# IuvenisSapiens/Qwen3-TTS-Rust

Hardware: AMD Instinct MI355X
Metric: audio-seconds generated per second (aggregate over GPUs) = concurrent real-time streams; RTF and first-chunk latency from the single-utterance leg (higher is better)
Workload: dtype i8

## Files before the change

### include/q3tts.h

```cpp
#ifndef Q3TTS_H
#define Q3TTS_H
#include <stdint.h>
#include <stddef.h>
#include "q3tts_spec.h"
#ifdef __cplusplus
extern "C" {
#endif

#define Q3TTS_OK 0
#define Q3TTS_ERR -1

const char* q3tts_last_error(void);
int q3tts_version(void);
int q3tts_device_count(void);

typedef struct q3tts_sampler_config {
    float temperature;
    int32_t top_k;
    float top_p;
    int32_t has_seed;
    uint64_t seed;
} q3tts_sampler_config;
void q3tts_sampler_config_default(q3tts_sampler_config* c);

// ... 81 lines not shown
int q3tts_submit_resume(q3tts_engine* e, const q3tts_request* r, int32_t want_pcm, const q3tts_gen_options* opts,
                        const int32_t* trail_ids, int32_t n_trail, int32_t open,
                        const int32_t* prefix_codes, int32_t n_prefix, int64_t* req_id);
#define Q3TTS_LOGPROB_COLS 17
#define Q3TTS_LOGPROB_NONE 1.0f
int q3tts_engine_set_logprobs(q3tts_engine* e, int32_t on);
int q3tts_fetch_logprobs(q3tts_engine* e, int64_t req_id, float* out, int32_t frame_off, int32_t max_frames, int32_t* got_frames);
int q3tts_engine_set_output_format(q3tts_engine* e, const q3tts_pcm_format* f);
int q3tts_request_format(q3tts_engine* e, int64_t req_id, q3tts_pcm_format* out);
int q3tts_fetch_pcm16(q3tts_engine* e, int64_t req_id, int16_t* out, int64_t off, int64_t cap, int64_t* got);
int q3tts_engine_pcm_out_stats(q3tts_engine* e, int64_t* chunks_converted, int64_t* samples_out);
int q3tts_engine_set_speech_rate(q3tts_engine* e, int32_t rate_pct);
int q3tts_request_speech_rate(q3tts_engine* e, int64_t req_id, int32_t* rate_pct);
int q3tts_engine_tsm_stats(q3tts_engine* e, int64_t* chunks, int64_t* frames_out, int64_t* flushes);
int q3tts_engine_set_pitch(q3tts_engine* e, int32_t pitch_pct);
int q3tts_request_pitch(q3tts_engine* e, int64_t req_id, int32_t* pitch_pct);
int q3tts_engine_pitch_stats(q3tts_engine* e, int64_t* chunks, int64_t* samples_out, int64_t* flushes, int64_t* table_bytes);
int q3tts_engine_set_volume(q3tts_engine* e, int32_t db10);
int q3tts_request_volume(q3tts_engine* e, int64_t req_id, int32_t* db10);
int q3tts_engine_volume_stats(q3tts_engine* e, int64_t* chunks, int64_t* samples);
typedef struct { double integrated_lufs, momentary_max_lufs, peak_dbfs; int32_t n_blocks, n_gated; } q3tts_loudness;
int q3tts_engine_set_loudness(q3tts_engine* e, int32_t on);
int q3tts_fetch_loudness(q3tts_engine* e, int64_t req_id, double* out , int64_t block_off, int64_t max_blocks, int64_t* got);
int q3tts_request_loudness(q3tts_engine* e, int64_t req_id, q3tts_loudness* out);
int q3tts_request_metered(q3tts_engine* e, int64_t req_id, int32_t* on);
int q3tts_engine_loudness_stats(q3tts_engine* e, int64_t* chunks, int64_t* blocks);
int q3tts_preamble_create(q3tts_engine* e, const int32_t* codes, int32_t n, int32_t* preamble_id);
int q3tts_preamble_poll(q3tts_engine* e, int32_t preamble_id, int32_t* state, int32_t* n_frames);
int q3tts_preamble_wait(q3tts_engine* e, int32_t preamble_id, double timeout_ms);
int q3tts_preamble_release(q3tts_engine* e, int32_t preamble_id);
int q3tts_voice_set_preamble(q3tts_engine* e, int32_t voice_id, int32_t preamble_id);
int q3tts_engine_set_preamble(q3tts_engine* e, int32_t preamble_id);
int q3tts_request_preamble(q3tts_engine* e, int64_t req_id, int32_t* preamble_id);
int q3tts_engine_preamble_stats(q3tts_engine* e, int64_t* built, int64_t* restores, int64_t* bytes_per_snapshot);
typedef struct q3tts_stem_stats { int64_t built, restores, rows_not_prefilled, pages_copied, mismatches, device_bytes; } q3tts_stem_stats;
int q3tts_stem_create(q3tts_engine* e, const float* rows, int32_t n_rows, int32_t* stem_id);
int q3tts_voice_stem_create(q3tts_engine* e, int32_t voice_id, int32_t lang_id, const int32_t* instr_ids, int32_t n_instr, int32_t* stem_id);
int q3tts_stem_poll(q3tts_engine* e, int32_t stem_id, int32_t* state, int32_t* n_rows);
int q3tts_stem_wait(q3tts_engine* e, int32_t stem_id, double timeout_ms);
int q3tts_stem_release(q3tts_engine* e, int32_t stem_id);
int q3tts_voice_set_stem(q3tts_engine* e, int32_t voice_id, int32_t stem_id);
int q3tts_engine_set_stem(q3tts_engine* e, int32_t stem_id);
int q3tts_request_stem(q3tts_engine* e, int64_t req_id, int32_t* stem_id, int32_t* rows_reused);
int q3tts_engine_stem_stats(q3tts_engine* e, q3tts_stem_stats* out);
int q3tts_submit_score(q3tts_engine* e, const float* prompt, int32_t n_prompt, const int32_t* trail_ids, int32_t n_trail,
                       const int32_t* codes, int32_t n, int64_t* req_id);
int32_t q3tts_engine_score_width(q3tts_engine* e);
int q3tts_submit_candidates(q3tts_engine* e, const q3tts_request* r, int32_t want_pcm, const q3tts_gen_options* opts,
                            const int32_t* trail_ids, int32_t n_trail, const uint64_t* seeds, int32_t n, int64_t* req_ids);
int q3tts_engine_candidate_stats(q3tts_engine* e, int64_t* sets, int64_t* prefill_rows_saved, int64_t* pages_copied);
int q3tts_submit_decode(q3tts_engine* e, const int32_t* codes, int32_t n, int64_t* req_id);
int32_t q3tts_engine_decode_width(q3tts_engine* e);
int q3tts_engine_decode_stats(q3tts_engine* e, int64_t* requests, int64_t* chunks, int64_t* chunks_shared);
int32_t q3tts_engine_prefill_width(q3tts_engine* e);
int q3tts_sched_start(q3tts_engine* e);
int q3tts_sched_stop(q3tts_engine* e);
int q3tts_sched_step(q3tts_engine* e, int32_t* busy);
int q3tts_voice_register(q3tts_engine* e, const float* spk_emb2048, const int32_t* ref_codes, int32_t n_ref_codes,
                         const int32_t* ref_text_ids, int32_t n_ref_text, int32_t* voice_id);
int q3tts_submit_text(q3tts_engine* e, int32_t voice_id, const int32_t* text_ids, int32_t n_text, int32_t lang_id,
                      const int32_t* instr_ids, int32_t n_instr, const q3tts_sampler_config* sampler, int32_t max_steps,
                      int32_t mask_eos, int32_t want_pcm, int64_t* req_id);
int q3tts_submit_text_ex(q3tts_engine* e, int32_t voice_id, const int32_t* text_ids, int32_t n_text, int32_t lang_id,
                         const int32_t* instr_ids, int32_t n_instr, const q3tts_sampler_config* sampler, int32_t max_steps,
                         int32_t mask_eos, int32_t want_pcm, const q3tts_gen_options* opts, int64_t* req_id);
int q3tts_submit_text_streaming(q3tts_engine* e, int32_t voice_id, const int32_t* text_ids, int32_t n_text, int32_t lang_id,
                                const int32_t* instr_ids, int32_t n_instr, const q3tts_sampler_config* sampler, int32_t max_steps,
                                int32_t mask_eos, int32_t want_pcm, const q3tts_gen_options* opts, int64_t* req_id);
int q3tts_submit_text_streaming_open(q3tts_engine* e, int32_t voice_id, const int32_t* text_ids, int32_t n_text, int32_t lang_id,
                                     const int32_t* instr_ids, int32_t n_instr, const q3tts_sampler_config* sampler, int32_t max_steps,
                                     int32_t mask_eos, int32_t want_pcm, const q3tts_gen_options* opts, int64_t* req_id);
int q3tts_text_append(q3tts_engine* e, int64_t req_id, const int32_t* text_ids, int32_t n, int32_t is_last);

typedef struct q3tts_group q3tts_group;
int q3tts_group_create(const q3tts_engine_params* p, const int32_t* device_ids, int32_t n_dev, q3tts_group** out);
void q3tts_group_destroy(q3tts_group* g);
int32_t q3tts_group_size(q3tts_group* g);
q3tts_engine* q3tts_group_engine(q3tts_group* g, int32_t i);
int32_t q3tts_group_uses_rccl(q3tts_group* g);
typedef struct q3tts_group_info_t {
    int32_t n_devices, rccl_loaded, rccl_ranks, distinct_devices;
    int64_t registrations_rccl, registrations_peer_copy;
} q3tts_group_info_t;
int q3tts_group_info(q3tts_group* g, q3tts_group_info_t* out);
int q3tts_group_voice_register(q3tts_group* g, const float* spk_emb2048, const int32_t* ref_codes, int32_t n_ref_codes,
                               const int32_t* ref_text_ids, int32_t n_ref_text, int32_t* voice_id);
int q3tts_group_submit(q3tts_group* g, const q3tts_request* r, int32_t want_pcm, int64_t* req_id);
int q3tts_group_submit_text(q3tts_group* g, int32_t voice_id, const int32_t* text_ids, int32_t n_text, int32_t lang_id,
                            const int32_t* instr_ids, int32_t n_instr, const q3tts_sampler_config* sampler, int32_t max_steps,
                            int32_t mask_eos, int32_t want_pcm, int64_t* req_id);
int q3tts_group_submit_ex(q3tts_group* g, const q3tts_request* r, int32_t want_pcm, const q3tts_gen_options* opts, int64_t* req_id);
int q3tts_group_submit_text_ex(q3tts_group* g, int32_t voice_id, const int32_t* text_ids, int32_t n_text, int32_t lang_id,
                               const int32_t* instr_ids, int32_t n_instr, const q3tts_sampler_config* sampler, int32_t max_steps,
                               int32_t mask_eos, int32_t want_pcm, const q3tts_gen_options* opts, int64_t* req_id);
int q3tts_group_submit_text_streaming(q3tts_group* g, int32_t voice_id, const int32_t* text_ids, int32_t n_text, int32_t lang_id,
                                      const int32_t* instr_ids, int32_t n_instr, const q3tts_sampler_config* sampler, int32_t max_steps,
                                      int32_t mask_eos, int32_t want_pcm, const q3tts_gen_options* opts, int64_t* req_id);
int q3tts_group_submit_text_streaming_open(q3tts_group* g, int32_t voice_id, const int32_t* text_ids, int32_t n_text, int32_t lang_id,
                                           const int32_t* instr_ids, int32_t n_instr, const q3tts_sampler_config* sampler,
                                           int32_t max_steps, int32_t mask_eos, int32_t want_pcm, const q3tts_gen_options* opts,
                                           int64_t* req_id);
int q3tts_group_text_append(q3tts_group* g, int64_t req_id, const int32_t* text_ids, int32_t n, int32_t is_last);
int q3tts_group_trail_append(q3tts_group* g, int64_t req_id, const int32_t* ids, int32_t n, int32_t close);
int q3tts_group_trail_progress(q3tts_group* g, int64_t req_id, int32_t* n_appended, int32_t* n_consumed, int32_t* closed);
int32_t q3tts_group_device_of(q3tts_group* g, int64_t req_id);
int q3tts_group_poll(q3tts_group* g, int64_t req_id, q3tts_req_status* out);
// ... 264 lines not shown
    uint64_t* keys; int64_t n_keys; int32_t key_stride; const int32_t* mask_per_tok; int32_t idx_add;
    float* out; int64_t out_floats, out_off; int32_t out_stride;
    int8_t* aq; uint16_t* ad;
    int32_t form_ran, lpr_ran, mt_ran, z_ran;
} q3tts_linear_desc;
int q3tts_op_linear(q3tts_linear_desc* d);
int q3tts_linear_plan(q3tts_linear_desc* d);
uint64_t q3tts_argmax_key(float v, int32_t idx);

enum { Q3TTS_SEL_SAMPLE = 0, Q3TTS_SEL_SAMPLE_PRED = 1, Q3TTS_SEL_ARGMAX = 2, Q3TTS_SEL_ARGMAX_KEYS = 3 };
#define Q3TTS_SELECT_SENTINEL 0xA5C3F00D5A3C0FF1ull
typedef struct q3tts_select_desc {
    int32_t kernel;
    int32_t B, n, stride, row_off;
    const float* logits;
    const float* temperature; const int32_t* top_k; const float* top_p;
    const int32_t* mask_idx;
    const uint64_t* seed;
    const uint32_t* draw0;
    int32_t n_draws;
    const float* penalty; const int32_t* hist; const int32_t* hist_len; int32_t hist_cap; const int32_t* cur_code;
    int32_t out_stride;
    int32_t start, end, add;
    int32_t* tokens;
    uint64_t* out_raw;
    uint32_t* draws_out;
} q3tts_select_desc;
int q3tts_op_select_rows(q3tts_select_desc* d);

enum { Q3TTS_GLUE_PROJECT_MT = 0, Q3TTS_GLUE_PROJECT_TABLE = 1, Q3TTS_GLUE_FEEDBACK_KEYS = 2, Q3TTS_GLUE_GATHER_ROWS_KEYS = 3,
       Q3TTS_GLUE_ADVANCE_KEYS = 4, Q3TTS_GLUE_STALL_SAVE = 5, Q3TTS_GLUE_ADVANCE_KEYS_GATED = 6 };
#define Q3TTS_GLUE_GUARD 64
typedef struct q3tts_guarded { void* p; int64_t n; } q3tts_guarded;
typedef struct q3tts_frame_glue_desc {
    int32_t kernel;
    int32_t ntok;
    int32_t n_in, n_out, x_stride, x_off, out_stride;
    const float* x; int64_t x_floats;
    const float* w; const float* b;
    const float* const* tables; const int64_t* table_rows;
    int32_t row_len, key_stride;
    const float* tts_pad;
    int32_t trail; const int32_t* trail_ids; int32_t ids_stride; const float* text_table; int64_t text_rows;
    const int32_t* n_trail; const int32_t* open; const int32_t* max_frames;
    int32_t hist_stride;
    q3tts_guarded out;
    q3tts_guarded keys, next_key0;
    q3tts_guarded finished, n_frames, t_slot, t_pos, hist;
    q3tts_guarded hidden, save_hidden;
    q3tts_guarded draws, pdraws, save_draws;
} q3tts_frame_glue_desc;
int q3tts_op_frame_glue(q3tts_frame_glue_desc* d);

enum { Q3TTS_GG_LOAD_ROWS = 0, Q3TTS_GG_ADD = 1, Q3TTS_GG_RMSNORM = 2, Q3TTS_GG_QUANT = 3, Q3TTS_GG_MATVEC = 4, Q3TTS_GG_LINEAR = 5,
       Q3TTS_GG_SWIGLU = 6 };
typedef struct q3tts_ggml_desc {
    int32_t op;
    int32_t ntok, k;
    int64_t n;
    const float* x; int64_t x_floats; int32_t x_stride; int32_t x_rows;
    const float* u; float eps;
    const int32_t* idx; const uint64_t* idx_keys; int32_t idx_stride; int64_t idx_n;
    const void* w; int32_t type, rows, row0, nrows, out_stride;
    q3tts_guarded out;
    q3tts_guarded q8, d8, qk, dk, bs;
} q3tts_ggml_desc;
int q3tts_op_ggml(q3tts_ggml_desc* d);

int q3tts_pcm_out_plan(int32_t rate, int32_t* L, int32_t* M, int32_t* n_taps, int32_t* taps_per_phase);
int64_t q3tts_pcm_out_filter(int32_t rate, float* h32, int64_t cap);
int64_t q3tts_pcm_out_samples(int32_t rate, int64_t n_native);
int q3tts_pcm_format_check(const q3tts_pcm_format* f);
int q3tts_op_pcm_convert(const float* in, int32_t G, const int32_t* chunk_samples, int32_t n_chunks, const int32_t* streams, int32_t n_streams,
                         const q3tts_pcm_format* fmt, const int32_t* reset_before, void* const* out, const int64_t* out_bytes, int64_t* n_out,
                         float* hist_store);

int64_t q3tts_tsm_samples(int32_t rate_pct, int64_t n_native, int32_t final);
int q3tts_tsm_windows(float* w, float* w2);
int q3tts_op_tsm(const float* in, int32_t G, const int32_t* chunk_samples, int32_t n_chunks, const int32_t* streams, int32_t n_streams,
                 const int32_t* rate_pct, const int32_t* encoding, const int32_t* reset_before, int32_t flush, void* const* out,
                 const int64_t* out_bytes, int64_t* n_out, int32_t* const* delta_trace, const int64_t* trace_len, float* hist_store);

int64_t q3tts_pitch_samples(int32_t rate_pct, int32_t pitch_pct, int64_t n_native, int32_t final);
int q3tts_pitch_plan(int32_t pitch_pct, int32_t* L, int32_t* M, int32_t* n_taps, int32_t* taps_per_output);
int64_t q3tts_pitch_filter(int32_t pitch_pct, float* h32, int64_t cap);
int q3tts_op_pitch(const float* in, int32_t G, const int32_t* chunk_samples, int32_t n_chunks, const int32_t* streams, int32_t n_streams,
                   const int32_t* rate_pct, const int32_t* pitch_pct, const int32_t* encoding, const int32_t* reset_before, int32_t flush,
                   void* const* out, const int64_t* out_bytes, int64_t* n_out, int32_t* const* delta_trace, const int64_t* trace_len,
                   float* hist_store, float* zhist_store);

float q3tts_volume_gain(int32_t db10);
int q3tts_op_volume(const float* in, int32_t G, const int32_t* chunk_samples, int32_t n_chunks, const int32_t* streams, int32_t n_streams,
                    const int32_t* vol_db10, const int32_t* reset_before, float* const* out, const int64_t* out_bytes, int64_t* n_out,
                    float* const* gain_trace, const int64_t* trace_len, float* hist_store);

int q3tts_loudness_tables(double* coef , double* m );
int q3tts_loudness_gate(const double* rows, int32_t n, q3tts_loudness* out);
int32_t q3tts_loudness_gain_db10(double measured_lufs, double target_lufs);
int q3tts_op_loudness(const float* in, int32_t G, const int32_t* chunk_samples, int32_t n_chunks, const int32_t* streams, int32_t n_streams,
                      const int32_t* metered, const int32_t* reset_before, double* const* rows, const int64_t* rows_bytes, int64_t* n_rows,
                      double* state_store);

int q3tts_intake_plan(int32_t rate, int32_t* L, int32_t* M, int32_t* n_taps, int32_t* taps_per_output);
int64_t q3tts_intake_filter(int32_t rate, float* h32, int64_t cap);
int64_t q3tts_intake_samples(int32_t rate, int64_t n_frames);
int32_t q3tts_intake_tile(int32_t rate);
// ... 10 lines not shown
```

### qwen3-tts-rust_amd/csrc/capi.cpp

```cpp
#include "../../include/q3tts.h"
#include "engine.h"
#include "tfctx.h"
#include <algorithm>

using namespace q3;

struct q3tts_assets { std::unique_ptr<HostAssets> owned; const HostAssets* a = nullptr; };
struct q3tts_engine { std::unique_ptr<Engine> e; q3tts_assets assets_view; };
struct q3tts_sampler { Sampler s; };
struct q3tts_chunker { std::unique_ptr<Chunker> c; };
struct q3tts_decoder { std::unique_ptr<CodecDecoder> d; hipStream_t st = nullptr; float* pinned = nullptr; size_t pinned_cap = 0; };
struct q3tts_tf { std::unique_ptr<TfContext> c; };

#define Q3_API_BEGIN try {
#define Q3_API_END(failval) } catch (const std::exception& ex) { set_last_error(ex.what()); return failval; } catch (...) { set_last_error("unknown error"); return failval; }

static void require_gpu() {
    int n = 0;
    if (hipGetDeviceCount(&n) != hipSuccess || n <= 0) throw Error("no HIP device available: the HIP path is the only compute path (no CPU fallback)");
}

extern "C" {

const char* q3tts_last_error(void) { return last_error(); }
// ... 85 lines not shown
    g.trail = trail_ids; g.n_trail = n_trail;
    *req_id = e->e->submit(g, want_pcm != 0, true);
    return Q3TTS_OK;
    Q3_API_END(Q3TTS_ERR)
}
int q3tts_submit_trailing_open(q3tts_engine* e, const q3tts_request* r, int32_t want_pcm, const q3tts_gen_options* opts,
                               const int32_t* trail_ids, int32_t n_trail, int64_t* req_id) {
    Q3_API_BEGIN
    Q3_CHECK(e && r && req_id, "null argument");
    GenRequest g = to_gen(*r);
    g.opts = to_opts(opts);
    g.trail = trail_ids; g.n_trail = n_trail; g.open = true;
    *req_id = e->e->submit(g, want_pcm != 0, true);
    return Q3TTS_OK;
    Q3_API_END(Q3TTS_ERR)
}
int q3tts_submit_resume(q3tts_engine* e, const q3tts_request* r, int32_t want_pcm, const q3tts_gen_options* opts, const int32_t* trail_ids,
                        int32_t n_trail, int32_t open, const int32_t* prefix_codes, int32_t n_prefix, int64_t* req_id) {
    Q3_API_BEGIN
    Q3_CHECK(e && r && req_id, "null argument");
    GenRequest g = to_gen(*r);
    g.opts = to_opts(opts);
    g.trail = trail_ids; g.n_trail = n_trail; g.open = open != 0;
    g.prefix = prefix_codes; g.n_prefix = n_prefix;
    *req_id = e->e->submit(g, want_pcm != 0, true);
    return Q3TTS_OK;
    Q3_API_END(Q3TTS_ERR)
}
int q3tts_submit_score(q3tts_engine* e, const float* prompt, int32_t n_prompt, const int32_t* trail_ids, int32_t n_trail, const int32_t* codes,
                       int32_t n, int64_t* req_id) {
    Q3_API_BEGIN
    Q3_CHECK(e && req_id, "null argument");
    *req_id = e->e->submit_score(prompt, n_prompt, trail_ids, n_trail, codes, n);
    return Q3TTS_OK;
    Q3_API_END(Q3TTS_ERR)
}
int32_t q3tts_engine_score_width(q3tts_engine* e) { return e ? e->e->score_width() : -1; }
int q3tts_submit_decode(q3tts_engine* e, const int32_t* codes, int32_t n, int64_t* req_id) {
    Q3_API_BEGIN
    Q3_CHECK(e && codes && req_id, "null argument");
    *req_id = e->e->submit_decode(codes, n);
    return Q3TTS_OK;
    Q3_API_END(Q3TTS_ERR)
}
int32_t q3tts_engine_decode_width(q3tts_engine* e) { return e ? e->e->decode_width() : -1; }
int q3tts_engine_decode_stats(q3tts_engine* e, int64_t* requests, int64_t* chunks, int64_t* chunks_shared) {
    Q3_API_BEGIN
    Q3_CHECK(e, "null argument");
    int64_t r = 0, c = 0, s = 0;
    e->e->decode_stats(&r, &c, &s);
    if (requests) *requests = r;
    if (chunks) *chunks = c;
    if (chunks_shared) *chunks_shared = s;
    return Q3TTS_OK;
    Q3_API_END(Q3TTS_ERR)
}
int q3tts_submit_candidates(q3tts_engine* e, const q3tts_request* r, int32_t want_pcm, const q3tts_gen_options* opts, const int32_t* trail_ids,
                            int32_t n_trail, const uint64_t* seeds, int32_t n, int64_t* req_ids) {
    Q3_API_BEGIN
    Q3_CHECK(e && r, "null argument");
    GenRequest g = to_gen(*r);
    g.opts = to_opts(opts);
    g.trail = trail_ids; g.n_trail = n_trail;
    std::vector<int64_t> ids((size_t)std::max(n, 1));
    e->e->submit_candidates(g, want_pcm != 0, seeds, n, req_ids ? ids.data() : nullptr);
    std::copy(ids.begin(), ids.begin() + n, req_ids);
    return Q3TTS_OK;
    Q3_API_END(Q3TTS_ERR)
}
int q3tts_engine_candidate_stats(q3tts_engine* e, int64_t* sets, int64_t* prefill_rows_saved, int64_t* pages_copied) {
    Q3_API_BEGIN
    Q3_CHECK(e, "null argument");
    int64_t s = 0, r = 0, p = 0;
    e->e->candidate_stats(&s, &r, &p);
    if (sets) *sets = s;
    if (prefill_rows_saved) *prefill_rows_saved = r;
    if (pages_copied) *pages_copied = p;
    return Q3TTS_OK;
    Q3_API_END(Q3TTS_ERR)
}
int q3tts_trail_append(q3tts_engine* e, int64_t req_id, const int32_t* ids, int32_t n, int32_t close) {
    Q3_API_BEGIN
    Q3_CHECK(e, "null argument");
    return e->e->append_trail(req_id, ids, n, close != 0);
    Q3_API_END(Q3TTS_ERR)
}
int q3tts_trail_progress(q3tts_engine* e, int64_t req_id, int32_t* n_appended, int32_t* n_consumed, int32_t* closed) {
    Q3_API_BEGIN
    Q3_CHECK(e && n_appended && n_consumed && closed, "null argument");
    int na = 0, nc = 0; bool cl = false;
    e->e->trail_progress(req_id, &na, &nc, &cl);
    *n_appended = na; *n_consumed = nc; *closed = cl ? 1 : 0;
    return Q3TTS_OK;
    Q3_API_END(Q3TTS_ERR)
}
int q3tts_text_append(q3tts_engine* e, int64_t req_id, const int32_t* text_ids, int32_t n, int32_t is_last) {
    Q3_API_BEGIN
    Q3_CHECK(e, "null argument");
    Q3_CHECK(n >= 0 && (n == 0 || text_ids), "bad arguments");
    std::vector<int32_t> ids(text_ids, text_ids + n);
    if (is_last) ids.push_back(Q3_TEXT_EOS);
    return e->e->append_trail(req_id, ids.data(), (int)ids.size(), is_last != 0);
    Q3_API_END(Q3TTS_ERR)
}
int q3tts_poll(q3tts_engine* e, int64_t id, q3tts_req_status* o) {
    Q3_API_BEGIN
// ... 580 lines not shown
```

### qwen3-tts-rust_amd/csrc/capi_ops.cpp

```cpp
#include "../../include/q3tts.h"
#include "transformer.h"
#include "host_logic.h"
#include "kdev.h"
#include "codec.h"
#include "kernels.h"
#include "pcm_out.h"
#include "tsm.h"
#include "pitch.h"
#include "volume.h"
#include "loudness.h"
#include "intake.h"
#include <memory>
#include "mel.h"

using namespace q3;
#define Q3_API_BEGIN try {
#define Q3_API_END(failval) } catch (const std::exception& ex) { set_last_error(ex.what()); return failval; } catch (...) { set_last_error("unknown error"); return failval; }
static void require_gpu() {
    int n = 0;
    if (hipGetDeviceCount(&n) != hipSuccess || n <= 0) throw Error("no HIP device available: the HIP path is the only compute path (no CPU fallback)");
}

static int attention_op_plan(const q3tts_attention_desc& d) {
    AttnPlanIn a;
// ... 1068 lines not shown
        } else {
            Q3_CHECK(d.tts_pad, "tts_pad missing");
            DevBuf<const float*> d_ptrs(16); DevBuf<int64_t> d_rows(16); DevBuf<float> d_pad(Q3_EMBD), d_text; DevBuf<int32_t> d_ntrail, d_ids;
            d_ptrs.upload(ptrs.data(), 16); d_rows.upload(d.table_rows, 16); d_pad.upload(d.tts_pad, Q3_EMBD);
            if (d.trail) {
                Q3_CHECK(d.n_trail && d.trail_ids && d.ids_stride >= 1 && d.text_table && d.text_rows >= 1, "the trail form needs n_trail / trail_ids / text_table");
                n_frames.up(d.n_frames, n, "n_frames");
                for (size_t t = 0; t < n; t++)
                    Q3_CHECK(n_frames.host[Q3TTS_GLUE_GUARD + t] >= 0 && d.n_trail[t] <= d.ids_stride, "n_frames < 0 or n_trail > ids_stride");
                d_ntrail.alloc(n); d_ntrail.upload(d.n_trail, n);
                d_ids.alloc(n * d.ids_stride); d_ids.upload(d.trail_ids, d_ids.n);
                d_text.alloc((size_t)d.text_rows * Q3_EMBD); d_text.upload(d.text_table, d_text.n);
                TextTrail tt; tt.n_frames = n_frames.p(); tt.n_trail = d_ntrail.p; tt.ids = d_ids.p; tt.ids_stride = d.ids_stride; tt.table = d_text.p; tt.rows = d.text_rows;
                launch_feedback_keys(0, d_ptrs.p, d_rows.p, keys.p(), d.key_stride, d_pad.p, out.p(), d.ntok, &tt);
            } else {
                launch_feedback_keys(0, d_ptrs.p, d_rows.p, keys.p(), d.key_stride, d_pad.p, out.p(), d.ntok);
            }
        }
        Q3_LAUNCH_CHECK();
        Q3_HIP(hipDeviceSynchronize());
        out.down(); keys.down(); n_frames.down();
        return Q3TTS_OK;
    }
    const bool gate = d.kernel != Q3TTS_GLUE_ADVANCE_KEYS;
    Q3_CHECK(d.max_frames && d.hist_stride >= 16, "max_frames / hist_stride missing");
    keys.up(d.keys, n * 16, "keys"); next_key0.up(d.next_key0, n, "next_key0");
    finished.up(d.finished, n, "finished"); n_frames.up(d.n_frames, n, "n_frames"); t_slot.up(d.t_slot, n, "t_slot");
    t_pos.up(d.t_pos, 4 * n, "t_pos"); hist.up(d.hist, n * d.hist_stride, "hist");
    for (size_t b = 0; b < n; b++)
        Q3_CHECK(n_frames.host[Q3TTS_GLUE_GUARD + b] >= 0 && d.max_frames[b] >= 0 && (int64_t)d.max_frames[b] * 16 <= d.hist_stride, "history row outside hist_stride");
    DevBuf<int32_t> d_max(n + 1), d_open, d_ntrail;
    d_max.zero(); d_max.upload(d.max_frames, n);
    AdvanceKeysArgs a{d.ntok, finished.p(), n_frames.p(), d_max.p, keys.p(), next_key0.p(), hist.p(), d.hist_stride, t_slot.p(), t_pos.p()};
    if (!gate) {
        launch_advance_keys(0, a);
    } else {
        Q3_CHECK(d.open && d.n_trail, "the gated kernels need open / n_trail");
        hidden.up(d.hidden, n * Q3_EMBD, "hidden"); save_hidden.up(d.save_hidden, n * Q3_EMBD, "save_hidden");
        draws.up(d.draws, n, "draws"); pdraws.up(d.pdraws, n, "pdraws"); save_draws.up(d.save_draws, 2 * n, "save_draws");
        d_open.alloc(n + 1); d_open.zero(); d_open.upload(d.open, n); d_ntrail.alloc(n + 1); d_ntrail.zero(); d_ntrail.upload(d.n_trail, n);
        StallArgs s; s.open = d_open.p; s.n_trail = d_ntrail.p; s.hidden = hidden.p(); s.draws = draws.p(); s.pdraws = pdraws.p();
        s.save_hidden = save_hidden.p(); s.save_draws = save_draws.p();
        if (d.kernel == Q3TTS_GLUE_STALL_SAVE) launch_stall_save(0, a, s);
        else launch_advance_keys_gated(0, a, s);
    }
    Q3_LAUNCH_CHECK();
    Q3_HIP(hipDeviceSynchronize());
    keys.down(); next_key0.down(); finished.down(); n_frames.down(); t_slot.down(); t_pos.down(); hist.down();
    hidden.down(); save_hidden.down(); draws.down(); pdraws.down(); save_draws.down();
    return Q3TTS_OK;
    Q3_API_END(Q3TTS_ERR)
}

int q3tts_op_ggml(q3tts_ggml_desc* dp) {
    Q3_API_BEGIN
    require_gpu();
    Q3_CHECK(dp, "null ggml-mode descriptor");
    const q3tts_ggml_desc& d = *dp;
    Q3_CHECK(d.op >= Q3TTS_GG_LOAD_ROWS && d.op <= Q3TTS_GG_SWIGLU, "unknown ggml-mode op");
    const bool flat = d.op == Q3TTS_GG_ADD || d.op == Q3TTS_GG_SWIGLU;
    const bool mat = d.op == Q3TTS_GG_MATVEC || d.op == Q3TTS_GG_LINEAR, quant = d.op == Q3TTS_GG_QUANT || mat;
    const auto holds = [](const q3tts_guarded& g, size_t core) { return g.p && g.n >= (int64_t)(core + 2 * Q3TTS_GLUE_GUARD); };
    GlueBuf<float> out, dk;
    GlueBuf<int8_t> q8, qk;
    GlueBuf<uint16_t> d8;
    GlueBuf<int16_t> bs;
    DevBuf<float> dx, du;
    if (flat) {
        Q3_CHECK(d.n >= 0 && d.n <= ((int64_t)1 << 31), "n out of [0, 2^31]");
        if (d.n == 0) return Q3TTS_OK;
        const size_t n = (size_t)d.n;
        Q3_CHECK(d.x && d.x_floats >= d.n && holds(d.out, n), "x / out do not hold n elements");
        Q3_CHECK(d.op == Q3TTS_GG_ADD || d.u, "u missing");
        out.up(d.out, n, "out");
        dx.alloc(n); dx.upload(d.x, n);
        if (d.op == Q3TTS_GG_ADD) gg_add(0, out.p(), dx.p, n);
        else { du.alloc(n); du.upload(d.u, n); gg_swiglu(0, dx.p, du.p, out.p(), n); }
        Q3_LAUNCH_CHECK();
        Q3_HIP(hipDeviceSynchronize());
        out.down();
        return Q3TTS_OK;
    }
    Q3_CHECK(d.ntok >= 0 && d.ntok <= 65535 && d.k >= 1, "ntok out of [0, 65535] or k < 1");
    const size_t nt = (size_t)d.ntok, k = (size_t)d.k;
    GgMat w;
    if (mat) {
        w.type = d.type; w.n = d.rows; w.k = d.k;
        Q3_CHECK(w.type == Q3_T_Q8_0 || w.type == Q3_T_Q5_K || w.type == Q3_T_Q6_K, "ggml mode serves Q8_0 / Q5_K / Q6_K matrices");
        Q3_CHECK(d.rows >= 0 && d.row0 >= 0 && d.nrows >= 0 && (int64_t)d.row0 + d.nrows <= d.rows, "ggml-mode matvec row range");
        if (d.nrows == 0) return Q3TTS_OK;
    }
    if (nt == 0) return Q3TTS_OK;
    if (quant) {
        Q3_CHECK(d.k % 256 == 0, "k % 256 != 0");
        Q3_CHECK(holds(d.q8, nt * k) && holds(d.d8, nt * k / 32) && holds(d.qk, nt * k) && holds(d.dk, nt * k / 256) && holds(d.bs, nt * k / 16),
                 "a quantised array does not hold ntok rows");
    }
    if (d.op == Q3TTS_GG_LOAD_ROWS) {
        Q3_CHECK(d.x && d.x_rows >= 1 && d.x_stride >= d.k && d.x_floats >= (int64_t)(d.x_rows - 1) * d.x_stride + d.k, "x does not hold x_rows rows");
        Q3_CHECK(!(d.idx && d.idx_keys) && holds(d.out, nt * k), "both index forms given, or out too small");
        if (d.idx || d.idx_keys) {
            Q3_CHECK(d.idx_stride >= 1 && d.idx_n >= (int64_t)(nt - 1) * d.idx_stride + 1, "idx / idx_keys do not hold ntok entries");
            for (size_t t = 0; t < nt; t++) {
                const int64_t row = d.idx_keys ? (int64_t)key_code(d.idx_keys[t * d.idx_stride]) : (int64_t)d.idx[t * d.idx_stride];
                Q3_CHECK(row >= 0 && row < d.x_rows, "a selected row lies outside x");
            }
// ... 608 lines not shown
```

### qwen3-tts-rust_amd/csrc/codec_worker.cpp

```cpp
#include "codec_worker.h"
#include <chrono>

namespace q3 {

CodecWorker::CodecWorker(CodecDecoder* codec, int dev, int n_lanes, int n_cs, size_t slot_cap) : codec_(codec), dev_(dev), st_(n_lanes), slot_cap_(slot_cap), n_cs_(n_cs) {
    for (auto& s : st_) Q3_HIP(hipStreamCreateWithFlags(&s, hipStreamNonBlocking));
    Q3_HIP(hipHostMalloc((void**)&pcm_pinned_, (size_t)n_cs * slot_cap_ * sizeof(float)));
}

CodecWorker::~CodecWorker() {
    if (started_) {
        { std::lock_guard<std::mutex> lk(mu_); stop_ = true; q_.hold = 0; }
        cv_.notify_all();
        thread_.join();
    }
    for (auto& c : comp_) (void)hipEventDestroy(c.ev);
    for (auto& kv : last_) (void)hipEventDestroy(kv.second.second);
    if (pcm_pinned_) (void)hipHostFree(pcm_pinned_);
    if (loud_pinned_.load()) (void)hipHostFree(loud_pinned_.load());
    for (auto s : st_) (void)hipStreamDestroy(s);
}

void CodecWorker::push(CodecJob* j, TaskKind kind, const int64_t* codes, int n_codes, bool is_final) {
    { std::lock_guard<std::mutex> lk(mu_); q_.push(j, kind, codes, n_codes, is_final); }
    cv_.notify_all();
}
void CodecWorker::purge(CodecJob* j) { std::lock_guard<std::mutex> lk(mu_); q_.purge(j); }
int CodecWorker::pending() { std::lock_guard<std::mutex> lk(mu_); return q_.pending; }

bool CodecWorker::poll_completion(bool block, Completion* out) {
    std::unique_lock<std::mutex> lk(mu_);
    if (!err_.empty()) throw Error("decoder thread: " + err_);
    if (comp_.empty()) {
        if (!block) return false;
        cv_.wait_for(lk, std::chrono::milliseconds(2));
        if (comp_.empty()) return false;
    }
    *out = comp_.front();
    if (!block && hipEventQuery(out->ev) != hipSuccess) return false;
    comp_.pop_front();
    q_.popped();
    lk.unlock();
    Q3_HIP(hipEventSynchronize(out->ev));
    return true;
}

unsigned char* CodecWorker::stage(const CodecJob& j, size_t add) const {
    const size_t at = j.pcm_enq * j.sample_bytes();
    Q3_CHECK(at + add <= slot_bytes(), "pcm staging overflow");
    return reinterpret_cast<unsigned char*>(pcm_pinned_ + (size_t)j.cs * slot_cap_) + at;
}

double* CodecWorker::loud_stage(const CodecJob& j, size_t add) {
    if (!loud_pinned_.load()) {
        std::lock_guard<std::mutex> cap(capture_mutex());
        double* p = nullptr;
        Q3_HIP(hipHostMalloc((void**)&p, (size_t)n_cs_ * loud_cap() * 2 * sizeof(double)));
        loud_pinned_.store(p);
    }
    Q3_CHECK(j.loud_enq + add <= loud_cap(), "loudness staging overflow");
    return loud_pinned_.load() + ((size_t)j.cs * loud_cap() + j.loud_enq) * 2;
}

int CodecWorker::pick_lane(const Step& s) {
    int lane = next_lane_;
    auto own = last_.find(s[0].job);
    if (s.size() == 1 && own != last_.end()) lane = own->second.first;
    else next_lane_ = (next_lane_ + 1) % (int)st_.size();
    for (const Task& t : s) {
        auto it = last_.find(t.job);
        if (it != last_.end() && it->second.first != lane) Q3_HIP(hipStreamWaitEvent(st_[lane], it->second.second, 0));
    }
    return lane;
}

void CodecWorker::start_stream(int lane, const Step& s) {
    CodecJob* j = s[0].job;
    if (j->pre_snap < 0) { codec_->reset_async(st_[lane], j->cs); return; }
    codec_->restore_async(st_[lane], j->pre_snap, j->cs, pcm_format_native(j->out.fmt) ? nullptr : j->pre_tail);
    pre_restores++;
}

void CodecWorker::decode_pass(int lane, const Step& s) {
    const int G = (int)s.size(), nf = (int)s[0].codes.size() / 16, spf = codec_->samples_per_frame();
    int n_low = 0;
    for (const Task& t : s) n_low += t.job->decode;
    dec_chunks += n_low;
    if (n_low < G) dec_shared += n_low;
    std::vector<int> streams(G); std::vector<float*> dst(G); std::vector<int64_t> codes((size_t)G * nf * 16);
    std::vector<OutSpec> out(G); std::vector<int64_t> n_out(G);
    std::vector<LoudDst> loud(G); std::vector<size_t> rows(G, 0);
    for (int g = 0; g < G; g++) {
        CodecJob* j = s[g].job;
        out[g] = j->out;
        const size_t add = j->bytes_due((int64_t)nf * spf, false);
        if (j->out.loud) {
            rows[g] = (size_t)loud_blocks(j->tsm_native, (int64_t)nf * spf);
            loud[g].pos = j->tsm_native; loud[g].rows = loud_stage(*j, rows[g]);
        }
        j->tsm_native += (int64_t)nf * spf;
        streams[g] = j->cs; dst[g] = reinterpret_cast<float*>(stage(*j, add));
        std::copy(s[g].codes.begin(), s[g].codes.end(), codes.begin() + (size_t)g * nf * 16);
    }
    codec_->decode_group_async(st_[lane], G, streams.data(), codes.data(), nf, dst.data(), lane, out.data(), n_out.data(), loud.data());
    for (int g = 0; g < G; g++) { s[g].job->pcm_enq += (size_t)n_out[g]; s[g].job->loud_enq += rows[g]; }
}

void CodecWorker::flush_rate(int lane, const Step& s) {
    CodecJob* j = s[0].job;
    if (!j->stretched() || j->cancel.load() || j->cs < 0) return;
    const size_t add = j->bytes_due(0, true);
    int64_t n = 0;
    codec_->tsm_flush_async(st_[lane], j->cs, stage(*j, add), &n, lane);
    j->pcm_enq += (size_t)n;
}
void CodecWorker::snapshot_build(int lane, const Step& s) {
    CodecJob* j = s[0].job;
    if (j->snapshot && !j->cancel.load()) j->snap = codec_->snapshot_async(st_[lane], j->cs);
}

void CodecWorker::record(int lane, const Step& s) {
    for (const Task& t : s) {
        hipEvent_t ev = nullptr;
        if (t.kind != TASK_RESET) {
            Q3_HIP(hipEventCreate(&ev));
            Q3_HIP(hipEventRecord(ev, st_[lane]));
        }
        auto it = last_.find(t.job);
        if (t.kind == TASK_FENCE) { if (it != last_.end()) { (void)hipEventDestroy(it->second.second); last_.erase(it); } }
        else {
            hipEvent_t ord;
            if (it == last_.end()) { Q3_HIP(hipEventCreateWithFlags(&ord, hipEventDisableTiming)); last_[t.job] = {lane, ord}; }
            else { ord = it->second.second; it->second.first = lane; }
            Q3_HIP(hipEventRecord(ord, st_[lane]));
        }
        if (t.kind == TASK_RESET) continue;
        std::lock_guard<std::mutex> lk(mu_);
        comp_.push_back(Completion{t.job, ev, t.job->pcm_enq, t.kind == TASK_FENCE, t.job->loud_enq});
        if (t.kind == TASK_CHUNK) codec_calls_++;
    }
    cv_.notify_all();
}

void CodecWorker::main() {
    try {
        Q3_HIP(hipSetDevice(dev_));
        const int gmax = codec_->max_group();
        for (;;) {
            Step s;
            {
                std::unique_lock<std::mutex> lk(mu_);
                cv_.wait(lk, [&] { return stop_ || q_.ready(); });
                s = q_.take(gmax);
                if (s.empty()) return;
            }
            const int lane = pick_lane(s);
            if (s[0].kind == TASK_RESET) start_stream(lane, s);
            else if (s[0].kind == TASK_CHUNK) decode_pass(lane, s);
            else { flush_rate(lane, s); snapshot_build(lane, s); }
            record(lane, s);
        }
    } catch (const std::exception& ex) {
        std::lock_guard<std::mutex> lk(mu_);
        err_ = ex.what();
        cv_.notify_all();
    }
}

}
```

### qwen3-tts-rust_amd/csrc/codec_worker.h

```cpp
#pragma once
#include "codec.h"
#include "loudness.h"
#include "sched_logic.h"
#include <atomic>
#include <condition_variable>
#include <mutex>
#include <thread>

namespace q3 {

struct CodecJob {
    int64_t id = 0;
    bool decode = false;
    int cs = -1;
    OutSpec out;
    int pre_snap = -1; const float* pre_tail = nullptr; bool snapshot = false;
    std::atomic<bool> cancel{false};
    int64_t tsm_native = 0;
    size_t pcm_enq = 0;
    size_t loud_enq = 0;
    int snap = -1;
    size_t sample_bytes() const { return out_sample_bytes(out); }
    bool stretched() const { return out_kind(out) >= OUT_RATED; }
    size_t bytes_due(int64_t n_more, bool final) const {
        return (size_t)(out_delivered(out, tsm_native + n_more, final) - out_delivered(out, tsm_native, false)) * sample_bytes();
    }
};

class CodecWorker {
public:
    struct Completion { CodecJob* job; hipEvent_t ev; size_t pcm_after; bool fence; size_t loud_after; };
    CodecWorker(CodecDecoder* codec, int dev, int n_lanes, int n_cs, size_t slot_cap);
    ~CodecWorker();
    void start() { if (!started_) { started_ = true; thread_ = std::thread([this] { main(); }); } }

    void push_reset(CodecJob* j) { push(j, TASK_RESET); }
    void push_chunk(CodecJob* j, const int64_t* codes, int n_codes, bool is_final) { push(j, TASK_CHUNK, codes, n_codes, is_final); }
    void push_fence(CodecJob* j) { push(j, TASK_FENCE); }
    void purge(CodecJob* j);
    struct Handover {
        CodecWorker* w;
        Handover(CodecWorker* w_, bool on) : w(on ? w_ : nullptr) { if (w) { std::lock_guard<std::mutex> lk(w->mu_); w->q_.open(); } }
        ~Handover() { if (w) { { std::lock_guard<std::mutex> lk(w->mu_); w->q_.close(); } w->cv_.notify_all(); } }
        Handover(const Handover&) = delete; Handover& operator=(const Handover&) = delete;
    };
    int pending();
    bool poll_completion(bool block, Completion* out);

    size_t slot_bytes() const { return slot_cap_ * sizeof(float); }
    const float* staging(int cs) const { return pcm_pinned_ + (size_t)cs * slot_cap_; }
    unsigned char* stage(const CodecJob& j, size_t add) const;
    size_t loud_cap() const { return slot_cap_ / Q3_LOUD_BLOCK + 1; }
    const double* loud_staging(int cs) const { return loud_pinned_.load() + (size_t)cs * loud_cap() * 2; }

    std::atomic<int64_t> dec_chunks{0}, dec_shared{0}, pre_restores{0};
    long take_codec_calls() { return (long)codec_calls_.exchange(0); }

private:
    typedef CodecQueue<CodecJob>::Task Task;
    typedef std::vector<Task> Step;
    void push(CodecJob* j, TaskKind kind, const int64_t* codes = nullptr, int n_codes = 0, bool is_final = false);
    void main();
    int pick_lane(const Step& s);
    void start_stream(int lane, const Step& s);
    void decode_pass(int lane, const Step& s);
    void flush_rate(int lane, const Step& s);
    void snapshot_build(int lane, const Step& s);
    void record(int lane, const Step& s);

    CodecDecoder* codec_; int dev_;
    std::vector<hipStream_t> st_;
    float* pcm_pinned_ = nullptr; size_t slot_cap_ = 0;
    std::atomic<double*> loud_pinned_{nullptr}; int n_cs_ = 0;
    double* loud_stage(const CodecJob& j, size_t add);
    std::thread thread_; bool started_ = false, stop_ = false;
    std::mutex mu_; std::condition_variable cv_;
    CodecQueue<CodecJob> q_; std::deque<Completion> comp_; std::string err_;
    std::map<CodecJob*, std::pair<int, hipEvent_t>> last_; int next_lane_ = 0;
    std::atomic<int64_t> codec_calls_{0};
};

}
```

### qwen3-tts-rust_amd/csrc/engine.cpp

```cpp
#include "engine.h"
#include "../../include/q3tts.h"
#include <algorithm>
#include <cmath>
#include <chrono>
#include "kdev.h"
#include <functional>

namespace q3 {

static std::string quant_dir(const std::string& q) {
    if (q == "q5_k_m") return "gguf_q5_k_m";
    if (q == "q8_0") return "gguf_q8_0";
    if (q == "bf16") return "gguf_bf16";
    if (q == "f16") return "gguf_f16";
    return "gguf";
}
static double now_ms() {
    return std::chrono::duration<double, std::milli>(std::chrono::steady_clock::now().time_since_epoch()).count();
}

Engine::Engine(const EngineParams& p) : p_(p) {
    Q3_CHECK(p.max_batch >= 1 && p.max_batch <= 512, "max_batch out of range");
    Q3_HIP(hipGetDevice(&dev_));
    Q3_HIP(hipStreamCreateWithFlags(&st_, hipStreamNonBlocking));
// ... 20 lines not shown
        const std::vector<float> wt = project_wt(assets_->proj_w, Q3_EMBD, dP_), wb = project_wblk(assets_->proj_w, Q3_EMBD, dP_);
        d_proj_wt_.alloc(wt.size()); d_proj_wt_.upload(wt.data(), wt.size());
        d_proj_wblk_.alloc(wb.size()); d_proj_wblk_.upload(wb.data(), wb.size());
    }
    d_proj_b_.alloc(dP_); d_proj_b_.upload(assets_->proj_b, dP_);
    d_tts_pad_.alloc(Q3_EMBD); d_tts_pad_.upload(assets_->tts_pad(), Q3_EMBD);
    std::vector<const float*> ptrs(16);
    std::vector<int64_t> rows(16);
    for (int q = 0; q < 16; q++) {
        const size_t n = (size_t)assets_->codec_rows[q] * Q3_EMBD;
        d_codec_tab_[q].alloc(n); d_codec_tab_[q].upload(assets_->codec[q], n);
        d_proj_tab_[q].alloc((size_t)assets_->codec_rows[q] * dP_);
        launch_project_table(st_, d_codec_tab_[q].p, assets_->codec_rows[q], d_proj_wt_.p, d_proj_b_.p, Q3_EMBD, dP_, d_proj_tab_[q].p);
        ptrs[q] = d_codec_tab_[q].p; rows[q] = assets_->codec_rows[q];
    }
    d_tab_ptrs_.alloc(16); d_tab_ptrs_.upload(ptrs.data(), 16);
    d_tab_rows_.alloc(16); d_tab_rows_.upload(rows.data(), 16);
    pred_l0_table_ = !predictor_->ggml_mode();
    if (const char* e = std::getenv("Q3_PRED_L0_TABLE")) if (e[0] == '0') pred_l0_table_ = false;
    if (pred_l0_table_) {
        const int qs = (predictor_->hp().n_head + 2 * predictor_->hp().n_kv) * 128;
        Transformer wide(*predictor_, 256);
        for (int q = 1; q < 15; q++) {
            d_qkv0_tab_[q].alloc((size_t)assets_->codec_rows[q] * qs);
            wide.build_layer0_qkv(st_, d_proj_tab_[q].p, dP_, assets_->codec_rows[q], d_qkv0_tab_[q].p);
            pred_table_bytes_ += d_qkv0_tab_[q].n * sizeof(float);
        }
        Q3_HIP(hipStreamSynchronize(st_));
    }
    const int pages_per_seq = (p.max_prompt + p.max_steps + 1 + 63) / 64;
    kv_rows_ = (int64_t)pages_per_seq * 64;
    kv_t_.reset(new KvPool(talker_->hp().n_layer, talker_->hp().n_kv, B * pages_per_seq + 1, B + 1, pages_per_seq));
    kv_p_.reset(new KvPool(predictor_->hp().n_layer, predictor_->hp().n_kv, B, B, 1));
    for (int b = 0; b < B; b++) kv_p_->ensure(b, 16);
    pred_identity_pages_ = true;
    for (int b = 0; b < B; b++) if (kv_p_->page(b, 0) != b) pred_identity_pages_ = false;
    if (const char* e = std::getenv("Q3_UNIFORM_META")) if (e[0] == '0') pred_identity_pages_ = false;
    kv_t_->ensure(B, 1);
    {
        const char* e = std::getenv("Q3_ASYNC_PREFILL");
        async_pf_ = B > 1 && !(e && e[0] == '0');
    }
    if (async_pf_) {
        talker_pf_.reset(new Transformer(*talker_, pf_chunk_));
        Q3_HIP(hipStreamCreateWithFlags(&st_pf_, hipStreamNonBlocking));
        Q3_HIP(hipEventCreate(&pf_done_)); Q3_HIP(hipEventCreate(&pf_e0_));
        lane_alloc(pf_, talker_pf_.get(), st_pf_, pf_chunk_, true,(size_t)4096 * (Q3_EMBD * 4 + 24 + 68 + 64) + ((size_t)1 << 16) + (size_t)B * 4 +
                   (size_t)B * 2 * (sizeof(StemJob) + 4) + 256);
    }
    hist_stride_ = p.max_steps * 16;
    tl_stride_ = (Q3_SAMPLE_END + 31) & ~31;
    slots_ = SlotTable(B); d_slots_.alloc(slots_.host.size()); slots_.dev = d_slots_.p;
    d_keys_.alloc(16 * B); d_next_key0_.alloc(B); d_hist_.alloc((size_t)B * hist_stride_);
    d_rngkey_.alloc((size_t)8 * B); d_draws_.alloc(B); d_prngkey_.alloc((size_t)8 * B); d_pdraws_.alloc(B);
    d_rngkey_.zero(); d_draws_.zero(); d_prngkey_.zero(); d_pdraws_.zero(); d_plogits_.alloc((size_t)B * Q3_CODEBOOK_SIZE);
    d_tlogits_.alloc((size_t)B * tl_stride_); d_thidden_.alloc((size_t)B * Q3_EMBD); d_pin_.alloc((size_t)2 * B * dP_);
    d_fb_.alloc((size_t)B * Q3_EMBD);
    d_hist_.zero(); d_tlogits_.zero(); d_thidden_.zero();
    std::vector<int32_t> seq(B), slot((size_t)16 * B), pos((size_t)16 * B * 4);
    for (int b = 0; b < B; b++) {
        seq[b] = b;
        for (int i = 0; i < 16; i++) { slot[(size_t)i * B + b] = i; for (int s = 0; s < 4; s++) pos[((size_t)i * B + b) * 4 + s] = i; }
    }
    d_pseq_.alloc(B); d_pseq_.upload(seq.data(), B);
    d_pslot_.alloc(slot.size()); d_pslot_.upload(slot.data(), slot.size());
    d_ppos_.alloc(pos.size()); d_ppos_.upload(pos.data(), pos.size());
    h_pend_.assign(B, std::vector<int32_t>()); h_pend_off_.assign(B, 0);
    slot_req_.assign(B, nullptr);
    if (const char* e = std::getenv("Q3_SCORE_WIDTH")) score_w_ = std::max(16, std::min(64, atoi(e)));
    if (async_pf_) { d_pf_logits_.alloc((size_t)B * tl_stride_); d_pf_hidden_.alloc((size_t)B * Q3_EMBD); }
    {
        std::vector<q3_u64> k0((size_t)16 * B, pack_key(-INFINITY, 0)), n0(B, pack_key(-INFINITY, 0));
        d_keys_.upload(k0.data(), k0.size()); d_next_key0_.upload(n0.data(), n0.size());
    }
    lane_alloc(ar_, talker_.get(), st_, talker_->max_tok(), false, (size_t)talker_->max_tok() * Q3_EMBD * 4 + (size_t)B * 4096 + ((size_t)1 << 20));
    Q3_HIP(hipDeviceSynchronize());
    upload_slot_state();
    if (p.load_codec) {
        Q3_CHECK(p.max_steps <= Q3TTS_CODEC_MAX_FRAMES, "max_steps above Q3TTS_CODEC_MAX_FRAMES: a request's codec stream could not be decoded to its end");
        static const int group_env = [] { const char* e = std::getenv("Q3_CODEC_GROUP"); return e ? atoi(e) : 0; }();
        const int group_cap = group_env > 0 ? group_env : (B >= 128 ? 32 : 16);
        const int n_cs = B + std::min(B, 16), gmax = std::max(1, std::min(B, group_cap));
        static const int lanes_env = [] { const char* e = std::getenv("Q3_CODEC_LANES"); return e ? atoi(e) : 0; }();
        const int n_lanes = B > 1 ? (lanes_env > 0 ? std::min(lanes_env, 8) : 2) : 1;
        codec_.reset(new CodecDecoder(p.model_dir + "/onnx/q3tts_codec.gguf", n_cs, 4, n_lanes, gmax));
        worker_.reset(new CodecWorker(codec_.get(), dev_, n_lanes, n_cs, (size_t)p.max_steps * codec_->samples_per_frame()));
        Q3_HIP(hipHostMalloc((void**)&pre_tails_, (size_t)Q3TTS_MAX_PREAMBLES * Q3_PCM_HIST * sizeof(float)));
        for (int i = Q3TTS_MAX_PREAMBLES - 1; i >= 0; i--) pre_tail_free_.push_back(i);
        for (int c = n_cs - 1; c >= 0; c--) cs_free_.push_back(c);
        decode_w_ = q3::decode_width(n_cs, B);
    }
    Q3_HIP(hipStreamSynchronize(st_));
    Q3_HIP(hipDeviceSynchronize());
    ar_.cur.reset();
}

void Engine::lane_alloc(PrefillLane& L, Transformer* talker, hipStream_t st, int chunk, bool async, size_t arena_bytes) {
    L.talker = talker; L.st = st; L.chunk = chunk; L.async = async;
    L.d_rows.alloc((size_t)chunk * Q3_EMBD); L.d_seq.alloc(chunk); L.d_slot.alloc(chunk); L.d_pos.alloc(4 * (size_t)chunk);
    L.d_codes.alloc((size_t)chunk * 16); L.d_ids.alloc(chunk); L.d_fork_dst.alloc(B_);
    L.d_stem_jobs.alloc((size_t)2 * B_); L.d_stem_slots.alloc((size_t)2 * B_);
    L.cur.cap = arena_bytes;
    Q3_HIP(hipHostMalloc((void**)&L.arena, arena_bytes));
}
void* Engine::stage_take(PrefillLane& L, size_t bytes) {
    size_t at = L.cur.take(bytes);
    if (at == StageCursor::NONE) {
        Q3_CHECK(!L.async, "prefill staging arena overflow");
        Q3_HIP(hipStreamSynchronize(L.st));
        L.cur.reset();
        at = L.cur.take(bytes);
        Q3_CHECK(at != StageCursor::NONE, "staging request larger than the arena");
    }
    return L.arena + at;
}
void Engine::h2d(void* dst, const void* src, size_t bytes) {
    void* p = stage_alloc(bytes);
    std::memcpy(p, src, bytes);
    Q3_HIP(hipMemcpyAsync(dst, p, bytes, hipMemcpyHostToDevice, st_));
}
void* Engine::d2h_begin(const void* src, size_t bytes) {
    void* p = stage_alloc(bytes);
    Q3_HIP(hipMemcpyAsync(p, src, bytes, hipMemcpyDeviceToHost, st_));
    return p;
}

struct CandSet { std::vector<float> prompt; std::vector<int32_t> trail; };
struct Engine::Req {
    CodecJob job;
    int64_t set = 0; std::shared_ptr<const CandSet> shared;
    const std::vector<int32_t>& trail_ids() const { return shared ? shared->trail : trail_own; }
    GenRequest r; std::vector<float> prompt_own; std::vector<int32_t> trail_own; bool want_pcm = false;
    std::vector<int32_t> prefix_own;
    bool closed = false;
    int state = REQ_QUEUED; int slot = -1; int fed = 0;
    std::vector<int32_t> codes; std::vector<float> pcm;
    int64_t pcm_n = 0;
    bool score = false;
    int pre = -1; bool pre_held = false; int build_pre = -1;
// ... 112 lines not shown
            if (v.lp) {
                LogprobArgs la;
                la.p.logits = d_plp_.p; la.p.stride = Q3_CODEBOOK_SIZE; la.p.head_stride = (size_t)B_ * Q3_CODEBOOK_SIZE; la.p.n = Q3_CODEBOOK_SIZE;
                la.p.key = d_keys_.p + 1; la.p.key_stride = 16; la.p.col = 1; la.n_first = 15;
                la.t.logits = d_tlogits_.p; la.t.stride = tl_stride_; la.t.n = Q3_SAMPLE_END; la.t.key = d_next_key0_.p; la.t.key_stride = 1;
                la.t.extra_idx = Q3_CODEC_EOS; la.t.col = 0; la.t.col_extra = Q3_LOGPROB_COLS - 1; la.t.row_ahead = 1;
                la.out = d_lp_.p; la.out_stride = Q3_LOGPROB_COLS; la.out_rows = lp_rows_;
                la.n_frames = di(SF_NFRAMES); la.finished = di(SF_FINISHED); la.max_frames = di(SF_MAXFRAMES); la.open = di(SF_OPEN);
                la.n_trail = di(SF_NTRAIL); la.record = d_lp_rec_.p;
                launch_logprob_rows(st_, la, B);
            }
        } else {
            ArgmaxEpi am{d_next_key0_.p, 1, di(SF_MASKEOS), 0};
            talker_->head(st_, 0, B, 0, tl_stride_, nullptr, 0, &am, Q3_SAMPLE_END, d_thidden_.p);
        }
    }
    if (v.gate) launch_advance_keys_gated(st_, a, sg);
    else launch_advance_keys(st_, a);
    Q3_LAUNCH_CHECK();
}

std::mutex& capture_mutex() { static std::mutex mu; return mu; }

Engine::FrameGraph& Engine::frame_graph(int width, FrameVariant v, bool capture) {
    std::unique_ptr<FrameGraph>& slot = graphs_[v.key(width)];
    std::unique_lock<std::mutex> build_lock(capture_mutex(), std::defer_lock);
    if (!slot || (capture && !slot->exec)) build_lock.lock();
    if (!slot) {
        slot.reset(new FrameGraph());
        FrameGraph& fg = *slot;
        fg.width = width;
        const int B = width;
        std::vector<int32_t> seqA(2 * B), slotA(2 * B), posA((size_t)2 * B * 4);
        for (int b = 0; b < B; b++) {
            seqA[b] = b; seqA[B + b] = b; slotA[b] = 0; slotA[B + b] = 1;
            for (int s = 0; s < 4; s++) { posA[(size_t)b * 4 + s] = 0; posA[((size_t)B + b) * 4 + s] = 1; }
        }
        fg.seqA.alloc(2 * B); fg.seqA.upload(seqA.data(), 2 * B);
        fg.slotA.alloc(2 * B); fg.slotA.upload(slotA.data(), 2 * B);
        fg.posA.alloc(posA.size()); fg.posA.upload(posA.data(), posA.size());
    }
    FrameGraph& fg = *slot;
    if (capture && !fg.exec) {
        (void)hipGetLastError();
        Q3_HIP(hipStreamBeginCapture(st_, hipStreamCaptureModeThreadLocal));
        try { record_frame(fg, v); }
        catch (...) { hipGraph_t dead = nullptr; (void)hipStreamEndCapture(st_, &dead); if (dead) (void)hipGraphDestroy(dead); throw; }
        Q3_HIP(hipStreamEndCapture(st_, &fg.graph));
        Q3_HIP(hipGraphInstantiate(&fg.exec, fg.graph, nullptr, nullptr, 0));
    }
    return fg;
}

void Engine::upload_slot_state() {
    slots_.route();
    h2d(slots_.dev, slots_.host.data(), slots_.host.size() * 4);
    slot_dirty_ = false;
}

void Engine::prefill_wave(PrefillLane& L, const std::vector<Req*>& wave, bool sampled) {
    size_t total = 0;
    std::vector<PromptRef> refs;
    std::vector<Req*> batch; std::vector<std::vector<Req*>> rest;
    split_sets(wave, batch, rest);
    for (Req* r : batch) {
        total += (size_t)admission_rows(r->r.n_prompt, r->n_skip, r->r.n_prefix);
        refs.push_back({r->r.prompt, r->r.n_prompt, r->slot, r->r.n_prefix, r->n_skip});
    }
    PrefillCursor cur; std::vector<std::pair<int, int>> lasts; std::vector<FbRun> fb;
    std::vector<char> is_score;
    for (Req* r : batch) is_score.push_back(r->score);
    restore_stems(L, batch);
    L.talker->set_same_seq_tokens(true);
    for (size_t done = 0; done < total;) {
        const size_t n_max = std::min<size_t>(total - done, (size_t)L.chunk);
        float* stage = (float*)stage_take(L, n_max * Q3_EMBD * 4);
        int32_t* hc = (int32_t*)stage_take(L, n_max * 68);
        int32_t* hs = (int32_t*)stage_take(L, n_max * 64);
        int32_t* seq = (int32_t*)stage_take(L, n_max * 4); int32_t* slot = (int32_t*)stage_take(L, n_max * 4); int32_t* pos = (int32_t*)stage_take(L, n_max * 16);
        const PrefillCursor before = cur;
        const int n = pack_prefill_chunk(refs, cur, (int)n_max, stage, seq, slot, pos, lasts, &fb);
        for (auto& run : staged_runs(n, fb))
            Q3_HIP(hipMemcpyAsync(L.d_rows.p + (size_t)run.first * Q3_EMBD, stage + (size_t)run.first * Q3_EMBD, (size_t)run.second * Q3_EMBD * 4, hipMemcpyHostToDevice, L.st));
        feedback_rows(L.st, batch, fb, hc, L.d_codes.p, L.d_ids.p, L.d_rows.p);
        Q3_HIP(hipMemcpyAsync(L.d_seq.p, seq, (size_t)n * 4, hipMemcpyHostToDevice, L.st));
        Q3_HIP(hipMemcpyAsync(L.d_slot.p, slot, (size_t)n * 4, hipMemcpyHostToDevice, L.st));
        Q3_HIP(hipMemcpyAsync(L.d_pos.p, pos, (size_t)n * 16, hipMemcpyHostToDevice, L.st));
        TokMeta tm{L.d_seq.p, L.d_slot.p, L.d_pos.p};
        Transformer::Input in; in.x = L.d_rows.p; in.x_stride = Q3_EMBD;
        L.talker->forward(L.st, in, n, tm, kv_t_->view(), nullptr);
        score_chunk(L.st, *L.talker, batch, score_head_runs(refs, is_score, before, n), hs);
        for (auto& lb : lasts) {
            if (batch[lb.first]->offline()) continue;
            if (L.async) head_staged(batch[lb.first], rest[lb.first], lb.second);
            else head_live(batch[lb.first], rest[lb.first], lb.second, sampled);
        }
        done += (size_t)n;
    }
    save_stems(L, batch);
    if (batch.size() < wave.size()) fork_sets(L.st, batch, rest, (int32_t*)stage_take(L, (size_t)B_ * 4), L.d_fork_dst.p);
}
SampleArgs Engine::first_head_args(const float* logits_row, int b) const {
    return SampleArgs{logits_row, tl_stride_, Q3_SAMPLE_END, df(SF_TEMP) + b, di(SF_TOPK) + b, df(SF_TOPP) + b,
                      di(SF_MASKEOS) + b, d_rngkey_.p + (size_t)b * 8, d_draws_.p + b, d_keys_.p + (size_t)b * 16, 16};
}
void Engine::head_live(Req* lead, const std::vector<Req*>& rest, int tok, bool sampled) {
    const bool hist = resumed_penalised(lead->r);
    const bool rec = lead->r.logprobs;
    for (size_t m = 0; m <= rest.size(); m++) {
// ... 427 lines not shown
            case CANCEL_PURGE: worker_->purge(&r->job); break;
            default: break;
            }
        }
    }
    for (Req* r : live) retire(r, false);
}

void Engine::admit(bool stalled) {
    if (async_pf_ && !pf_batch_.empty()) return;
    std::vector<Req*> batch;
    {
        std::lock_guard<std::mutex> lk(mu_);
        int reserved = 0;
        for (int b = 0; b < B_; b++) if (slot_req_[b]) reserved++;
        static const int quantum_div = [] { const char* e = std::getenv("Q3_ADMIT_DIV"); return e ? std::max(1, atoi(e)) : 8; }();
        const int free_slots = B_ - reserved, quantum = std::max(1, B_ / quantum_div);
        if (free_slots < quantum && n_active_ > 0 && free_slots < (int)pending_.size() && !stalled) return;
        std::vector<QueueEntry> q;
        for (Req* r : pending_) {
            if ((int)q.size() >= free_slots && (q.empty() || r->set == 0 || r->set != q.back().set)) break;
            q.push_back({admission_rows(r->r.n_prompt, r->n_skip, r->r.n_prefix), r->want_pcm, r->set});
        }
        for (int take = admission_take(q, free_slots, (int)cs_free_.size(), async_pf_ && n_active_ > 0); take > 0; take--) {
            Req* r = pending_.front();
            int slot = -1;
            for (int b = 0; b < B_; b++) if (!slot_req_[b]) { slot = b; break; }
            pending_.pop_front();
            r->slot = slot;
            if (r->want_pcm) { r->job.cs = cs_free_.back(); cs_free_.pop_back(); }
            r->state = REQ_RUNNING; r->t_admit = now_ms();
            slot_req_[slot] = r;
            batch.push_back(r);
        }
    }
    if (batch.empty()) return;
    alloc_stem_stores(batch);
    for (Req* r : batch) {
        if (r->want_pcm) worker_->push_reset(&r->job);
        r->chunker.reset(new Chunker([this, r](const int64_t* codes, int n_codes, bool is_final) { if (r->want_pcm) worker_->push_chunk(&r->job, codes, n_codes, is_final); }));
        Q3_HIP(hipEventCreate(&r->ev_admit));
    }
    if (async_pf_ && n_active_ > 0) { prefill_async(batch); return; }
    for (Req* r : batch) kv_t_->release(r->slot), kv_t_->ensure(r->slot, kv_positions(r->r, r->score), st_);
    bool sampled = live_variant(slots_).sampled;
    std::vector<Req*> live, scores, builds;
    for (Req* r : batch) {
        if (r->r.sampler.temperature > 0.0f) sampled = true;
        (r->build_stem >= 0 ? builds : r->score ? scores : live).push_back(r);
    }
    hipEvent_t e0, e1;
    Q3_HIP(hipEventCreate(&e0)); Q3_HIP(hipEventCreate(&e1));
    go_live(live);
    { std::lock_guard<std::mutex> lk(mu_); n_active_ += (int)live.size(); }
    Q3_HIP(hipEventRecord(e0, st_));
    for (Req* r : batch) Q3_HIP(hipEventRecord(r->ev_admit, st_));
    prefill_wave(ar_, batch, sampled);
    Q3_HIP(hipEventRecord(e1, st_));
    Q3_HIP(hipStreamSynchronize(st_));
    { float ms = 0; Q3_HIP(hipEventElapsedTime(&ms, e0, e1)); stats.prefill_ms += ms; }
    (void)hipEventDestroy(e0); (void)hipEventDestroy(e1);
    {
        const double t = now_ms();
        std::lock_guard<std::mutex> lk(mu_);
        for (Req* r : batch) r->prefill_ms = t - r->t_submit;
    }
    finish_scores(scores);
    finish_builds(builds);
}

int64_t Engine::submit_decode(const int32_t* codes, int n) {
    if (const char* why = decode_refusal(codes, n, p_.max_steps, codec_ != nullptr)) throw Error(why);
    std::unique_ptr<Req> r(new Req());
    r->job.decode = true; r->want_pcm = true;
    take_out(r.get(), n);
    r->r.max_steps = n; r->r.n_prompt = 0; r->r.sampler.temperature = 0.0f;
    r->codes.assign(codes, codes + (size_t)n * 16); r->fed = n;
    r->t_submit = now_ms();
    std::lock_guard<std::mutex> lk(mu_);
    if (pres_.setting >= 0) pre_attach(r.get(), pres_.setting);
    dec_reqs_++;
    return enqueue(std::move(r), decode_q_);
}

void Engine::admit_decodes() {
    std::lock_guard<std::mutex> lk(mu_);
    for (int take = decode_admit((int)decode_q_.size(), (int)cs_free_.size(), n_decoding_, decode_w_); take > 0; take--) {
        Req* r = decode_q_.front();
        decode_q_.pop_front();
        r->job.cs = cs_free_.back(); cs_free_.pop_back();
        r->state = REQ_DRAINING; r->t_admit = now_ms();
        n_draining_++; n_decoding_++;
        dec_admitted_.push_back(r);
    }
}

void Engine::enqueue_decodes() {
    std::vector<Req*> batch;
    batch.swap(dec_admitted_);
    for (Req* r : batch) {
        Q3_HIP(hipEventCreate(&r->ev_admit));
        Q3_HIP(hipEventRecord(r->ev_admit, st_));
        CodecWorker::Handover piece(worker_.get(), true);
        worker_->push_reset(&r->job);
        Chunker cut([&](const int64_t* codes, int n_codes, bool is_final) { worker_->push_chunk(&r->job, codes, n_codes, is_final); });
        push_frames(cut, r->codes.data(), r->fed);
        cut.push(nullptr, 0, true);
        worker_->push_fence(&r->job);
    }
}

void Engine::prefill_async(const std::vector<Req*>& wave) {
    for (Req* r : wave) {
        kv_t_->release(r->slot);
        kv_t_->ensure(r->slot, kv_positions(r->r, r->score), st_pf_);
    }
    pf_.cur.reset();
    Q3_HIP(hipEventRecord(pf_e0_, st_pf_));
    for (Req* r : wave) Q3_HIP(hipEventRecord(r->ev_admit, st_pf_));
    prefill_wave(pf_, wave, false);
    Q3_HIP(hipEventRecord(pf_done_, st_pf_));
    pf_batch_ = wave;
    n_prefilling_ = (int)wave.size();
}

void Engine::go_live(const std::vector<Req*>& batch) {
    ar_.cur.reset();
    q3_u64 armed[17]; std::fill_n(armed, 17, pack_key(-INFINITY, 0));
    bool prefix_pcm = false;
    for (Req* r : batch) prefix_pcm = prefix_pcm || (r->want_pcm && r->r.n_prefix >= 4);
    {
        CodecWorker::Handover hold(worker_.get(), worker_ && prefix_pcm);
        for (Req* r : batch) {
            const int b = r->slot;
            slots_.load(b, r->r);
            const int k = r->r.n_prefix;
            const uint32_t draws = r->r.sampler.temperature > 0.0f ? (uint32_t)k : 0u, pdraws = 15u * (uint32_t)k;
            if (k > 0) {
                h2d(d_hist_.p + (size_t)b * hist_stride_, r->prefix_own.data(), (size_t)k * 64);
                push_frames(*r->chunker, r->prefix_own.data(), k);
            }
            StdRng rng(r->seed);
            h2d(d_rngkey_.p + (size_t)b * 8, rng.key(), 32);
            h2d(d_draws_.p + b, &draws, 4);
            if (r->r.opts.pred_sampled()) {
                StdRng prng(r->seed ^ (uint64_t)Q3_PRED_SEED_XOR);
                h2d(d_prngkey_.p + (size_t)b * 8, prng.key(), 32);
                h2d(d_pdraws_.p + b, &pdraws, 4);
            }
            h_pend_[b].clear();
            std::vector<int32_t> ids;
            { std::lock_guard<std::mutex> lk(mu_); ids = r->trail_ids(); slots_.hi(SF_OPEN)[b] = r->r.open && !r->closed; }
            slots_.hi(SF_NTRAIL)[b] = (int)ids.size();
            if (!ids.empty()) h2d(d_trail_.p + (size_t)b * p_.max_prompt, ids.data(), ids.size() * 4);
            h2d(d_keys_.p + (size_t)b * 16, armed, 16 * 8);
            h2d(d_next_key0_.p + b, armed, 8);
            if (lp_ready_.load()) {
                const int32_t rec = r->r.logprobs ? 1 : 0;
                h2d(d_lp_rec_.p + b, &rec, 4);
                if (rec) Q3_HIP(hipMemsetD32Async((hipDeviceptr_t)(d_lp_.p + (size_t)b * lp_rows_ * Q3_LOGPROB_COLS), (int)q3_f32_bits(Q3_LOGPROB_NONE),
                                                  (size_t)lp_rows_ * Q3_LOGPROB_COLS, st_));
            }
            slots_.live[b] = 1;
        }
    }
    upload_slot_state();
}

void Engine::activate() {
    std::vector<Req*> batch, dropped, scores, builds;
    batch.swap(pf_batch_);
    for (Req* r : batch) if (r->build_stem >= 0) builds.push_back(r);
    batch.erase(std::remove_if(batch.begin(), batch.end(), [](Req* r) { return r->build_stem >= 0; }), batch.end());
    {
        std::lock_guard<std::mutex> lk(mu_);
        const double t = now_ms();
        for (Req* r : batch) if (r->job.cancel) { r->prefill_ms = t - r->t_submit; dropped.push_back(r); }
        batch.erase(std::remove_if(batch.begin(), batch.end(), [](Req* r) { return r->job.cancel.load(); }), batch.end());
    }
    for (Req* r : dropped) retire(r, false);
    for (Req* r : batch) if (r->score) scores.push_back(r);
    batch.erase(std::remove_if(batch.begin(), batch.end(), [](Req* r) { return r->score; }), batch.end());
    go_live(batch);
    for (Req* r : batch) {
        const int b = r->slot;
        Q3_HIP(hipMemcpyAsync(d_thidden_.p + (size_t)b * Q3_EMBD, d_pf_hidden_.p + (size_t)b * Q3_EMBD, (size_t)Q3_EMBD * 4, hipMemcpyDeviceToDevice, st_));
        SampleArgs sa = first_head_args(d_pf_logits_.p + (size_t)b * tl_stride_, b);
        if (resumed_penalised(r->r)) head_history(sa, b);
        launch_sample(st_, sa, 1);
        if (r->r.logprobs) first_head_logprobs(st_, d_pf_logits_.p + (size_t)b * tl_stride_, b, r->r.n_prefix);
    }
    Q3_HIP(hipStreamSynchronize(st_));
    { float ms = 0; Q3_HIP(hipEventElapsedTime(&ms, pf_e0_, pf_done_)); stats.prefill_ms += ms; }
    n_prefilling_ = 0;
    {
        const double t = now_ms();
        std::lock_guard<std::mutex> lk(mu_);
        for (Req* r : batch) r->prefill_ms = t - r->t_submit;
        for (Req* r : scores) r->prefill_ms = t - r->t_submit;
        n_active_ += (int)batch.size();
    }
    finish_scores(scores);
    finish_builds(builds);
}

void Engine::ensure_score() {
    std::lock_guard<std::mutex> lk(sc_mu_);
    if (sc_ready_.load()) return;
    std::lock_guard<std::mutex> cap(capture_mutex());
    int prev = 0;
    Q3_HIP(hipGetDevice(&prev));
    Q3_HIP(hipSetDevice(dev_));
    try {
        const int W = score_w_, rows = std::max(talker_->max_tok(), pf_chunk_);
        pred_sc_.reset(new Transformer(*predictor_, 16 * W));
        kv_sc_.reset(new KvPool(predictor_->hp().n_layer, predictor_->hp().n_kv, W, W, 1));
        for (int w = 0; w < W; w++) kv_sc_->ensure(w, 16);
        std::vector<int32_t> seq, slot, pos;
        for (int F = 1; F <= W; F++)
            for (int p = 0; p < 16; p++)
                for (int f = 0; f < F; f++) { seq.push_back(f); slot.push_back(p); for (int s4 = 0; s4 < 4; s4++) pos.push_back(p); }
        d_sc_seq_.alloc(seq.size()); d_sc_seq_.upload(seq.data(), seq.size());
        d_sc_slot_.alloc(slot.size()); d_sc_slot_.upload(slot.data(), slot.size());
        d_sc_pos_.alloc(pos.size()); d_sc_pos_.upload(pos.data(), pos.size());
        std::vector<const float*> tabs(15); std::vector<int64_t> tab_rows(15);
        for (int q = 0; q < 15; q++) { tabs[q] = d_proj_tab_[q].p; tab_rows[q] = assets_->codec_rows[q]; }
        d_sc_tabs_.alloc(15); d_sc_tabs_.upload(tabs.data(), 15);
        d_sc_tab_rows_.alloc(15); d_sc_tab_rows_.upload(tab_rows.data(), 15);
        d_sc_codes_.alloc((size_t)rows * 16); d_sc_tlogits_.alloc((size_t)rows * tl_stride_); d_sc_hidden_.alloc((size_t)rows * Q3_EMBD);
        d_sc_hproj_.alloc((size_t)W * dP_); d_sc_in_.alloc((size_t)16 * W * dP_); d_sc_plogits_.alloc((size_t)15 * W * Q3_CODEBOOK_SIZE);
        d_sc_out_.alloc((size_t)B_ * p_.max_steps * Q3_LOGPROB_COLS);
        Q3_HIP(hipStreamSynchronize(nullptr));
    } catch (...) { (void)hipSetDevice(prev); throw; }
    Q3_HIP(hipSetDevice(prev));
    sc_ready_ = true;
}

int64_t Engine::submit_score(const float* prompt, int n_prompt, const int32_t* trail, int n_trail, const int32_t* codes, int n) {
    if (const char* why = score_refusal(prompt, n_prompt, p_.max_prompt, trail, n_trail, codes, n, p_.max_steps, kv_rows_, talker_->ggml_mode()))
        throw Error(why);
    ensure_score();
    if (n_trail > 0) ensure_text_stream();
    std::unique_ptr<Req> r(new Req());
    r->score = true;
    GenRequest& g = r->r;
    g.n_prompt = n_prompt; g.max_steps = n; g.sampler.temperature = 0.0f; g.n_trail = n_trail;
    g.n_prefix = n - 1;
    r->prompt_own.assign(prompt, prompt + (size_t)n_prompt * Q3_EMBD); g.prompt = r->prompt_own.data();
    r->trail_own.assign(trail, trail + n_trail); g.trail = r->trail_own.data();
    r->prefix_own.assign(codes, codes + (size_t)n * 16); g.prefix = r->prefix_own.data();
    r->t_submit = now_ms();
    std::lock_guard<std::mutex> lk(mu_);
    return enqueue(std::move(r), pending_);
// ... 16 lines not shown
            launch_score_inputs(st, d_sc_hproj_.p, d_sc_tabs_.p, d_sc_tab_rows_.p, dP_, codes, F, d_sc_in_.p);
            const size_t m0 = (size_t)16 * F * (F - 1) / 2;
            TokMeta tm{d_sc_seq_.p + m0, d_sc_slot_.p + m0, d_sc_pos_.p + m0 * 4};
            Transformer::Input in; in.x = d_sc_in_.p; in.x_stride = dP_;
            pred_sc_->set_same_seq_tokens(true);
            pred_sc_->forward(st, in, 16 * F, tm, kv_sc_->view(), nullptr);
            for (int q = 0; q < 15; q++)
                pred_sc_->head(st, (q + 1) * F, F, q * Q3_CODEBOOK_SIZE, Q3_CODEBOOK_SIZE, d_sc_plogits_.p + (size_t)q * W * Q3_CODEBOOK_SIZE, Q3_CODEBOOK_SIZE);
            ScoreRowsArgs sa;
            sa.tlogits = d_sc_tlogits_.p + (size_t)(at + f0) * tl_stride_; sa.t_stride = tl_stride_;
            sa.plogits = d_sc_plogits_.p; sa.p_head_stride = (size_t)W * Q3_CODEBOOK_SIZE; sa.codes = codes;
            sa.out = d_sc_out_.p + ((size_t)r->slot * p_.max_steps + run.frame + f0) * Q3_LOGPROB_COLS;
            launch_score_rows(st, sa, F);
        }
        at += run.n;
    }
    Q3_LAUNCH_CHECK();
}

void Engine::finish_scores(const std::vector<Req*>& scores) {
    for (Req* r : scores) {
        const int b = r->slot, n = r->r.max_steps;
        bool cancelled;
        { std::lock_guard<std::mutex> lk(mu_); cancelled = r->job.cancel; }
        const float* rows = nullptr;
        if (!cancelled) {
            ar_.cur.reset();
            rows = (const float*)d2h_begin(d_sc_out_.p + (size_t)b * p_.max_steps * Q3_LOGPROB_COLS, (size_t)n * Q3_LOGPROB_COLS * 4);
            Q3_HIP(hipStreamSynchronize(st_));
        }
        {
            std::lock_guard<std::mutex> lk(mu_);
            if (r->job.cancel) r->state = REQ_CANCELLED;
            else {
                r->codes = r->prefix_own;
                r->lp.assign(rows, rows + (size_t)n * Q3_LOGPROB_COLS);
                r->fed = n;
                r->state = REQ_DONE;
            }
            slot_req_[b] = nullptr; r->slot = -1;
            r->t_done = now_ms();
            cv_.notify_all();
        }
        kv_t_->release(b);
    }
}

void Engine::retire(Req* r, bool flush_tail) {
    if (flush_tail) r->chunker->push(nullptr, 0, true);
    const int b = r->slot;
    {
        std::lock_guard<std::mutex> lk(mu_);
        slot_req_[b] = nullptr;
        if (slots_.live[b]) { slots_.live[b] = 0; n_active_--; }
        r->slot = -1;
        r->state = retired_state(r->want_pcm, r->job.cancel);
        if (r->want_pcm) n_draining_++;
        else { r->t_done = now_ms(); drop_held(r); cv_.notify_all(); }
    }
    if (r->want_pcm) {
        if (!flush_tail) worker_->purge(&r->job);
        worker_->push_fence(&r->job);
    }
    slots_.reset(b); h_pend_[b].clear();
    kv_t_->release(b);
    slot_dirty_ = true;
}

static int pick_width(int hi, int W) {
    int w = 1;
    while (w < hi) w <<= 1;
    return std::min(w, W);
}

void Engine::run_group() {
    int hi = 0, remaining = 0;
    int32_t* h_nfr = slots_.hi(SF_NFRAMES); int32_t* h_fin = slots_.hi(SF_FINISHED);
    for (int b = 0; b < B_; b++)
        if (slots_.live[b]) { hi = b + 1; remaining = std::max(remaining, slot_req_[b]->r.max_steps - h_nfr[b]); }
    const FrameVariant v = live_variant(slots_);
    ar_.cur.reset();
    for (int b = 0; b < B_; b++)
        if (!h_pend_[b].empty()) {
            h2d(d_trail_.p + (size_t)b * p_.max_prompt + h_pend_off_[b], h_pend_[b].data(), h_pend_[b].size() * 4);
            h_pend_[b].clear();
        }
    if (slot_dirty_) upload_slot_state();
    const int width = pick_width(hi, B_);
    const int group = std::max(1, std::min(4, remaining));
    const bool eager = instrument_ || !p_.use_graph;
    FrameGraph& fg = frame_graph(width, v, !eager);
    if (instrument_) { talker_->timer = &timer_; predictor_->timer = &timer_; talker_->timer_gu = &timer_gu_; }
    hipEvent_t e0, e1;
    Q3_HIP(hipEventCreate(&e0)); Q3_HIP(hipEventCreate(&e1));
    Q3_HIP(hipEventRecord(e0, st_));
    for (int g = 0; g < group; g++) {
        if (eager) record_frame(fg, v);
        else Q3_HIP(hipGraphLaunch(fg.exec, st_));
    }
    Q3_HIP(hipEventRecord(e1, st_));
    const int32_t* p_nfr = (const int32_t*)d2h_begin(di(SF_NFRAMES), (size_t)width * 4);
    const int32_t* p_fin = (const int32_t*)d2h_begin(di(SF_FINISHED), (size_t)width * 4);
    std::vector<const int32_t*> p_hist(width, nullptr);
    std::vector<const float*> p_lp(width, nullptr);
    for (int b = 0; b < width; b++)
        if (slots_.live[b]) {
            Req* r = slot_req_[b];
            const int rows = std::min(group, r->r.max_steps - r->fed);
            if (rows > 0) p_hist[b] = (const int32_t*)d2h_begin(d_hist_.p + (size_t)b * hist_stride_ + (size_t)r->fed * 16, (size_t)rows * 64);
            if (rows > 0 && r->r.logprobs)
                p_lp[b] = (const float*)d2h_begin(d_lp_.p + ((size_t)b * lp_rows_ + r->fed) * Q3_LOGPROB_COLS, (size_t)rows * Q3_LOGPROB_COLS * 4);
        }
    Q3_HIP(hipStreamSynchronize(st_));
    { float ms = 0; Q3_HIP(hipEventElapsedTime(&ms, e0, e1)); stats.frame_loop_ms += ms; }
    (void)hipEventDestroy(e0); (void)hipEventDestroy(e1);
    stats.steps++; stats.slot_frames += (double)width * group; stats.graph_frames += group;
    talker_->timer = nullptr; predictor_->timer = nullptr; talker_->timer_gu = nullptr;
    if (instrument_) {
        stats.gemv_ms += timer_.collect_ms(); stats.gemv_bytes += timer_.bytes; stats.gemv_launches += timer_.launches; timer_.bytes = 0; timer_.launches = 0;
        stats.gu_ms += timer_gu_.collect_ms(); stats.gu_bytes += timer_gu_.bytes; stats.gu_launches += timer_gu_.launches; timer_gu_.bytes = 0; timer_gu_.launches = 0;
    }
    std::memcpy(h_nfr, p_nfr, (size_t)width * 4); std::memcpy(h_fin, p_fin, (size_t)width * 4);
    CodecWorker::Handover hold(worker_.get(), worker_ != nullptr);
    for (int b = 0; b < width; b++) {
        if (!slots_.live[b]) continue;
        Req* r = slot_req_[b];
        if (h_nfr[b] > r->fed) {
            const int nnew = h_nfr[b] - r->fed;
            const int32_t* hbuf = p_hist[b];
            {
                std::lock_guard<std::mutex> lk(mu_);
                r->codes.insert(r->codes.end(), hbuf, hbuf + (size_t)nnew * 16);
                if (p_lp[b]) r->lp.insert(r->lp.end(), p_lp[b], p_lp[b] + (size_t)nnew * Q3_LOGPROB_COLS);
                r->fed = h_nfr[b];
            }
            push_frames(*r->chunker, hbuf, nnew);
            stats.frames += nnew;
        }
        if (h_fin[b] || h_nfr[b] >= r->r.max_steps) retire(r, true);
    }
    enqueue_decodes();
}

static double g_t_harvest = 0, g_t_admit = 0, g_t_group = 0, g_t_idle = 0;
static const bool g_trace = std::getenv("Q3_SCHED_TRACE") != nullptr;
bool Engine::step() {
    std::lock_guard<std::mutex> step_lock(step_mu_);
    Q3_HIP(hipSetDevice(dev_));
    if (worker_) worker_->start();
    const double t0 = now_ms();
    harvest(false);
    const double t1 = now_ms();
    if (async_pf_ && n_prefilling_ > 0) {
        if (n_active_ == 0) Q3_HIP(hipEventSynchronize(pf_done_));
        if (hipEventQuery(pf_done_) == hipSuccess) activate();
    }
    free_stem_stores();
    collect_appends();
    collect_cancels();
    admit(n_active_ > 0 && slots_.all_live_stalled());
    if (codec_) admit_decodes();
    if (!(n_active_ > 0 && !slots_.all_live_stalled())) enqueue_decodes();
    const double t2 = now_ms();
    const bool stalled = n_active_ > 0 && slots_.all_live_stalled();
    const int dec_pending = stalled && worker_ ? worker_->pending() : 0;
    if (n_active_ > 0 && !stalled) run_group();
    else if (n_prefilling_ > 0) { Q3_HIP(hipEventSynchronize(pf_done_)); activate(); }
    else if (n_draining_ > 0 || dec_pending > 0) harvest(true);
    const double t3 = now_ms();
    if (g_trace) {
        g_t_harvest += t1 - t0; g_t_admit += t2 - t1; (n_active_ > 0 ? g_t_group : g_t_idle) += t3 - t2;
        fprintf(stderr, "[sched] harvest %.1f admit %.1f group %.1f drain-wait %.1f ms (frame_loop %.1f prefill %.1f)\n", g_t_harvest, g_t_admit, g_t_group, g_t_idle,
                stats.frame_loop_ms, stats.prefill_ms);
    }
    std::lock_guard<std::mutex> lk(mu_);
    stalled_idle_ = stalled && n_prefilling_ == 0 && dec_pending == 0;
    return n_active_ > 0 || n_prefilling_ > 0 || n_draining_ > 0 || !pending_.empty() || !decode_q_.empty();
}

ReqStatus Engine::poll(int64_t id) {
    std::lock_guard<std::mutex> lk(mu_);
    const Req& r = req(id);
    ReqStatus s;
    const bool ended = r.state == REQ_DONE || r.state == REQ_CANCELLED;
    s.state = r.state; s.n_frames = r.fed; s.n_pcm = ended ? r.pcm_n : (int64_t)r.pcm_ready;
    s.queue_ms = (r.t_admit > 0 ? r.t_admit : ended ? r.t_done : now_ms()) - r.t_submit;
// ... 369 lines not shown
```

### qwen3-tts-rust_amd/csrc/engine.h

```cpp
#pragma once
#include "transformer.h"
#include "host_logic.h"
#include "sched_logic.h"
#include "codec.h"
#include "codec_worker.h"
#include <atomic>
#include <condition_variable>
#include <deque>
#include <map>
#include <memory>
#include <mutex>
#include <thread>

namespace q3 {

struct EngineParams {
    std::string model_dir;
    std::string quant = "q8_0";
    int max_batch = 1;
    int max_prompt = 1024;
    int max_steps = Q3_DEFAULT_MAX_STEPS;
    bool load_codec = true;
    bool use_graph = true;
};

struct GenResult {
    std::vector<int32_t> codes; int n_frames = 0;
    std::vector<float> pcm;
    double prefill_ms = 0, first_chunk_ms = 0, total_ms = 0;
};

struct EngineStats {
    double frame_loop_ms = 0; long frames = 0;
    double gemv_ms = 0; long gemv_launches = 0; double gemv_bytes = 0;
    double gu_ms = 0; long gu_launches = 0; double gu_bytes = 0;
    double codec_ms = 0; long codec_calls = 0;
    double prefill_ms = 0;
    long steps = 0; double slot_frames = 0;
    long graph_frames = 0;
};

struct ReqStatus {
    int state = REQ_QUEUED; int n_frames = 0; int64_t n_pcm = 0;
    double queue_ms = 0, prefill_ms = 0, first_chunk_ms = 0, total_ms = 0;
    std::string error;
};

struct Voice {
    std::vector<float> spk_emb; std::vector<int32_t> ref_codes, ref_text_ids;
    int preamble = -1;
    int stem = -1;
};


class Engine {
public:
    explicit Engine(const EngineParams& p);
    ~Engine();
    void generate_batch(const std::vector<GenRequest>& reqs, std::vector<GenResult>& out, bool want_pcm);

    int64_t submit(const GenRequest& r, bool want_pcm, bool copy_prompt = true, bool may_record = true);
    void set_logprobs(bool on);
    void fetch_logprobs(int64_t id, float* out, int frame_off, int max_frames, int* got_frames);
    int append_trail(int64_t id, const int32_t* ids, int n, bool close);
    void trail_progress(int64_t id, int* n_appended, int* n_consumed, bool* closed);
    int cancel(int64_t id);
    int64_t submit_score(const float* prompt, int n_prompt, const int32_t* trail, int n_trail, const int32_t* codes, int n);
    int score_width() const { return score_w_; }
    void submit_candidates(const GenRequest& g, bool want_pcm, const uint64_t* seeds, int n, int64_t* req_ids);
    void candidate_stats(int64_t* sets, int64_t* rows_saved, int64_t* pages_copied) const {
        *sets = cand_sets_.load(); *rows_saved = cand_rows_saved_.load(); *pages_copied = cand_pages_.load();
    }
    int64_t submit_decode(const int32_t* codes, int n);
    int decode_width() const { return decode_w_; }
    void decode_stats(int64_t* requests, int64_t* chunks, int64_t* chunks_shared) const {
        *requests = dec_reqs_.load(); *chunks = worker_ ? worker_->dec_chunks.load() : 0; *chunks_shared = worker_ ? worker_->dec_shared.load() : 0;
    }
    void set_output_format(const q3tts_pcm_format* f);
    q3tts_pcm_format request_format(int64_t id);
    void fetch_pcm16(int64_t id, int16_t* out, int64_t off, int64_t cap, int64_t* got);
    OutputStageStats output_stats() const;
    void set_speech_rate(int pct);
    int request_speech_rate(int64_t id);
    void set_pitch(int pct);
    int request_pitch(int64_t id);
    void set_volume(int db10);
    int request_volume(int64_t id);
    void set_loudness(bool on);
    bool request_metered(int64_t id);
    void fetch_loudness(int64_t id, double* out, int64_t block_off, int64_t max_blocks, int64_t* got);
    int preamble_create(const int32_t* codes, int n);
    void preamble_poll(int id, int* state, int* n_frames);
    bool preamble_wait(int id, double timeout_ms);
    void preamble_release(int id);
    void set_voice_preamble(int voice_id, int preamble_id);
    int voice_preamble(int voice_id);
    void set_preamble(int preamble_id);
    int request_preamble(int64_t id);
    void preamble_stats(int64_t* built, int64_t* restores, int64_t* bytes_per_snapshot) const;
    int stem_create(const float* rows, int n);
    void stem_poll(int id, int* state, int* n_rows);
    bool stem_wait(int id, double timeout_ms);
    void stem_release(int id);
    void set_voice_stem(int voice_id, int stem_id);
    int voice_stem(int voice_id);
    void set_stem(int stem_id);
    void request_stem(int64_t id, int* stem_id, int* rows_reused);
    struct StemStats { int64_t built = 0, restores = 0, rows_skipped = 0, pages_copied = 0, mismatches = 0, bytes_held = 0; };
    StemStats stem_stats() const;
    bool step();
    ReqStatus poll(int64_t id);
    void fetch(int64_t id, int32_t* codes, int frame_off, int max_frames, float* pcm, int64_t pcm_off, int64_t pcm_cap,
               int* got_frames, int64_t* got_pcm);
    bool wait(int64_t id, double timeout_ms);
    void release(int64_t id);
    void start_driver();
    void stop_driver();
    int register_voice(const Voice& v);
    const Voice& voice(int id) const;

    const HostAssets& assets() const { return *assets_; }
    Transformer& talker() { return *talker_; }
    Transformer& predictor() { return *predictor_; }
    CodecDecoder* codec() { return codec_.get(); }
    EngineStats stats; void reset_stats() { read_stats(); stats = EngineStats(); }
    const EngineStats& read_stats() { if (worker_) stats.codec_calls += worker_->take_codec_calls(); return stats; }
    void set_instrument(bool on) { instrument_ = on; }
// ... 8 lines not shown
    struct FrameGraph {
        int width = 0; hipGraph_t graph = nullptr; hipGraphExec_t exec = nullptr;
        DevBuf<int32_t> seqA, slotA, posA;
    };
    void record_frame(FrameGraph& fg, FrameVariant v);
    FrameGraph& frame_graph(int width, FrameVariant v, bool capture);
    void validate(const GenRequest& g) const;
    void ensure_text_stream();
    Req& req(int64_t id);
    int64_t enqueue(std::unique_ptr<Req> r, std::deque<Req*>& queue);
    struct PrefillLane {
        Transformer* talker = nullptr; hipStream_t st = nullptr; int chunk = 0; bool async = false;
        DevBuf<float> d_rows; DevBuf<int32_t> d_seq, d_slot, d_pos;
        DevBuf<int32_t> d_codes, d_ids, d_fork_dst;
        DevBuf<StemJob> d_stem_jobs; DevBuf<int32_t> d_stem_slots;
        unsigned char* arena = nullptr; StageCursor cur;
    };
    void lane_alloc(PrefillLane& L, Transformer* talker, hipStream_t st, int chunk, bool async, size_t arena_bytes);
    void* stage_take(PrefillLane& L, size_t bytes);
    void prefill_wave(PrefillLane& L, const std::vector<Req*>& wave, bool sampled);
    void head_live(Req* lead, const std::vector<Req*>& rest, int tok, bool sampled);
    void head_staged(Req* lead, const std::vector<Req*>& rest, int tok);
    SampleArgs first_head_args(const float* logits_row, int b) const;
    void feedback_rows(hipStream_t st, const std::vector<Req*>& batch, const std::vector<FbRun>& fb, int32_t* hc, int32_t* d_codes, int32_t* d_ids, float* d_rows);
    void head_history(SampleArgs& sa, int b) const;
    static bool resumed_penalised(const GenRequest& g) { return g.n_prefix > 0 && g.opts.penalised(); }
    void first_head_logprobs(hipStream_t st, const float* logits_row, int b, int row);
    void ensure_score();
    void score_chunk(hipStream_t st, Transformer& talker, const std::vector<Req*>& batch, const std::vector<ScoreRun>& runs, int32_t* h_codes);
    void finish_scores(const std::vector<Req*>& scores);
    static void split_sets(const std::vector<Req*>& batch, std::vector<Req*>& lead, std::vector<std::vector<Req*>>& rest);
    void fork_sets(hipStream_t st, const std::vector<Req*>& lead, const std::vector<std::vector<Req*>>& rest, int32_t* h_dst, int32_t* d_dst);
    static int kv_positions(const GenRequest& g, bool score) { return score ? g.n_prompt + g.n_prefix + 1 : g.n_prompt + g.max_steps + 1; }
    void restore_stems(PrefillLane& L, const std::vector<Req*>& lead);
    void save_stems(PrefillLane& L, const std::vector<Req*>& lead);
    void alloc_stem_stores(const std::vector<Req*>& wave);
    void finish_builds(const std::vector<Req*>& builds);
    void free_stem_stores();
    void prefill_async(const std::vector<Req*>& wave);
    void go_live(const std::vector<Req*>& batch);
    void activate();
    void admit_decodes();
    void enqueue_decodes();
    void admit(bool stalled);
    void run_group();
    void collect_appends();
    void collect_cancels();
    void harvest(bool block);
    void retire(Req* r, bool flush_tail);
    int64_t copy_pcm(const Req& r, void* out, int64_t off, int64_t cap) const;
    OutSpec out_; mutable std::mutex out_mu_;
    void take_out(Req* r, int max_steps, const OutSpec* given = nullptr) const;
    void upload_slot_state();
    void* stage_alloc(size_t bytes) { return stage_take(ar_, bytes); }
    void h2d(void* dst, const void* src, size_t bytes);
    void* d2h_begin(const void* src, size_t bytes);

    EngineParams p_;
    hipStream_t st_ = nullptr; int dev_ = 0;
    std::unique_ptr<HostAssets> assets_;
    std::unique_ptr<Transformer> talker_, predictor_, talker_pf_;
    hipStream_t st_pf_ = nullptr; PrefillLane ar_, pf_;
    DevBuf<float> d_pf_logits_, d_pf_hidden_;
    std::vector<Req*> pf_batch_; hipEvent_t pf_done_ = nullptr, pf_e0_ = nullptr; bool async_pf_ = false; int n_prefilling_ = 0;
    int pf_chunk_ = 256;
    std::unique_ptr<KvPool> kv_t_, kv_p_;
    std::unique_ptr<CodecDecoder> codec_;
    std::unique_ptr<CodecWorker> worker_;
    DevBuf<float> d_codec_tab_[16]; DevBuf<float> d_proj_tab_[16];
    DevBuf<float> d_qkv0_tab_[16]; bool pred_l0_table_ = false; size_t pred_table_bytes_ = 0;
    DevBuf<float> d_proj_wt_, d_proj_wblk_, d_proj_b_, d_tts_pad_;
    DevBuf<const float*> d_tab_ptrs_; DevBuf<int64_t> d_tab_rows_;
    int dP_ = 0;
    int B_ = 0; SlotTable slots_; DevBuf<uint32_t> d_slots_; bool slot_dirty_ = false;
    int32_t* di(SlotField f) const { return slots_.di(f); } float* df(SlotField f) const { return slots_.df(f); }
    DevBuf<int32_t> d_hist_; DevBuf<q3_u64> d_keys_, d_next_key0_;
    DevBuf<uint32_t> d_rngkey_, d_draws_, d_prngkey_, d_pdraws_; DevBuf<float> d_plogits_;
    DevBuf<int32_t> d_pseq_, d_pslot_, d_ppos_;
    DevBuf<float> d_tlogits_, d_thidden_, d_pin_, d_fb_;
    int64_t kv_rows_ = 0;
    int hist_stride_ = 0, tl_stride_ = 0;
    DevBuf<float> d_text_; DevBuf<int32_t> d_trail_; int64_t text_rows_ = 0;
    std::mutex text_mu_; bool text_ready_ = false;
    DevBuf<float> d_stall_hidden_; DevBuf<uint32_t> d_stall_draws_;
    DevBuf<float> d_lp_, d_plp_; DevBuf<int32_t> d_lp_rec_; int lp_rows_ = 0;
    std::mutex lp_mu_; std::atomic<bool> lp_on_{false}, lp_ready_{false};
    std::unique_ptr<Transformer> pred_sc_; std::unique_ptr<KvPool> kv_sc_; int score_w_ = 32;
    DevBuf<int32_t> d_sc_seq_, d_sc_slot_, d_sc_pos_, d_sc_codes_; DevBuf<const float*> d_sc_tabs_; DevBuf<int64_t> d_sc_tab_rows_;
    DevBuf<float> d_sc_tlogits_, d_sc_hidden_, d_sc_hproj_, d_sc_in_, d_sc_plogits_, d_sc_out_;
    std::mutex sc_mu_; std::atomic<bool> sc_ready_{false};
    int64_t next_set_ = 1;
    std::atomic<int64_t> cand_sets_{0}, cand_rows_saved_{0}, cand_pages_{0};
    std::map<int, std::unique_ptr<FrameGraph>> graphs_;
    bool instrument_ = false; bool pred_identity_pages_ = false;
    std::vector<std::vector<int32_t>> h_pend_; std::vector<int> h_pend_off_;
    std::mutex mu_; std::condition_variable cv_;
    std::mutex step_mu_;
    std::map<int64_t, std::unique_ptr<Req>> reqs_;
    std::deque<Req*> pending_;
    std::vector<Req*> slot_req_;
    std::vector<int> cs_free_;
    int64_t next_id_ = 1;
    int n_active_ = 0, n_draining_ = 0;
    std::deque<Req*> decode_q_; int n_decoding_ = 0, decode_w_ = 0;
    std::vector<Req*> dec_admitted_;
    std::atomic<int64_t> dec_reqs_{0};
    struct PreHeld { int snap = -1, tail = -1; };
    struct StemHeld { std::shared_ptr<const std::vector<float>> rows; uint16_t* store = nullptr; int64_t bytes = 0; };
    HeldTable<PreHeld> pres_{"preamble"}; HeldTable<StemHeld> stems_{"stem"};
    float* pre_tails_ = nullptr; std::vector<int> pre_tail_free_;
    std::vector<std::pair<uint16_t*, int64_t>> stem_garbage_;
    std::atomic<int64_t> pre_built_{0};
    std::atomic<int64_t> stem_built_{0}, stem_restores_{0}, stem_rows_{0}, stem_pages_{0}, stem_miss_{0}, stem_bytes_{0};
    void recycled(const std::optional<PreHeld>& p);
    void recycled(const std::optional<StemHeld>& s);
    void pre_attach(Req* r, int pid);
    void stem_match(Req* const* rs, int n_reqs, int asked);
    void drop_held(Req* r);
    void end_build(Req* r);
    template <class T> void held_poll(T& tab, int id, int* state, int* n);
    template <class T> bool held_wait(T& tab, int id, double timeout_ms);
    template <class T> void held_release(T& tab, int id);
    template <class T> void held_set(T& tab, int Voice::*field, int voice_id, int id);
    int voice_setting(int Voice::*field, int voice_id);
    bool trail_dirty_ = false;
    std::vector<int64_t> cancel_ids_;
    uint64_t wake_ = 0;
    bool stalled_idle_ = false;
    std::vector<Voice> voices_;
    std::thread driver_; bool driver_on_ = false, driver_stop_ = false;
    LaunchTimer timer_, timer_gu_;
};
// ... 3 lines not shown
```

### qwen3-tts-rust_amd/csrc/kernels.h

```cpp
#pragma once
#include <hip/hip_runtime.h>
#include <cstdint>
#include <map>
#include <mutex>
#include <vector>
#include "wlayout.h"
#include "q3_common.h"

namespace q3 {

struct Q8Mat {
    const uint8_t* qs = nullptr;
    const uint16_t* sc = nullptr;
    int N = 0;
    int Npad = 0;
    int K = 0;
    const uint8_t* rg_type = nullptr;
    const uint32_t* rg_off = nullptr;
    const uint8_t* meta = nullptr;
    size_t qbytes = 0;
    int nparts = 0; int p1_rg0 = 0x7fffffff, p2_rg0 = 0x7fffffff; int p0_type = 0, p1_type = 0, p2_type = 0; uint32_t p0_off = 0, p1_off = 0, p2_off = 0;
    size_t bytes() const { return (qbytes ? qbytes : (size_t)Npad * K) + (size_t)Npad * (K / 32) * 2 + (meta ? (size_t)Npad * (K / 256) * 16 : 0); }
};

// ... 124 lines not shown
                  LIN_GEMM_KQ_MFMA = 6, LIN_GU_Q8_TILE1 = 7, LIN_GU_Q8_MFMA = 8, LIN_GU_KQ_MFMA = 9, LIN_GU_UNFUSED = 10, LIN_NORM = 11,
                  LIN_NORM_WG = 12, LIN_GEMV_NORM = 13, LIN_GEMV_NORM_ARGMAX = 14, LIN_GU_SWIGLU_NORM = 15, LIN_F_GEMV = 16, LIN_F_MFMA16 = 17,
                  LIN_F_MFMA = 18, LIN_F_GU_MFMA16 = 19, LIN_F_GU_UNFUSED = 20, LIN_GEMM_Q8_WIDE = 21, LIN_GU_Q8_WIDE = 22 };
bool prefill_wide();
struct LinearPlanIn {
    int op = LOP_GEMV;
    int K = 0, row0 = 0, nrows = 0, ntok = 0, ff = 0;
    int wts = 0;
    bool kq = false;
    int kq_parts = 0;
    bool has_wt = false;
    int out_stride = 0; uintptr_t out_addr = 0;
    int x_stride = 0; uintptr_t x_addr = 0;
    uintptr_t aq_addr = 0;
    int lpr_hint = 0;
    bool fused = true;
};
struct LinearPlan { int form = LIN_AUTO, lpr = 0, mt = 0, z = 0, nseg = 0; };
LinearPlan plan_linear(const LinearPlanIn& in);
void run_gemv_q8(hipStream_t st, const LinearPlan& p, const Q8Mat& w, int row0, int nrows, const int8_t* xq, const uint16_t* xd, float* out,
                 int out_stride, int ntok);
void run_gateup_q8(hipStream_t st, const LinearPlan& p, const Q8Mat& wgu, int ff, const int8_t* xq, const uint16_t* xd, int8_t* aq, uint16_t* ad,
                   int ntok);
void run_gemv_q8_norm(hipStream_t st, const LinearPlan& p, const Q8Mat& w, int row0, int nrows, const NormPro& a, float* out, int out_stride,
                      int ntok, const ArgmaxEpi* am);
void run_gateup_swiglu(hipStream_t st, const LinearPlan& p, const Q8Mat& wgu, int ff, const NormPro& a, int8_t* aq, uint16_t* ad, int ntok);
void run_gemv_float(hipStream_t st, const LinearPlan& p, const FMat& w, int row0, int nrows, const float* x, int x_stride, float* out,
                    int out_stride, int ntok);
void run_gateup_float(hipStream_t st, const LinearPlan& p, const FMat& wgu, int ff, const float* x, int x_stride, float* act, int ntok);
LinearPlanIn linear_plan_in(int op, const Q8Mat& w, int row0, int nrows, int ntok);
struct TextTrail {
    const int32_t* n_frames = nullptr; const int32_t* n_trail = nullptr; const int32_t* ids = nullptr; int ids_stride = 0;
    const float* table = nullptr; int64_t rows = 0;
};
void launch_feedback_keys(hipStream_t st, const float* const* tables, const int64_t* table_rows, const q3_u64* keys, int key_stride,
                          const float* tts_pad, float* out, int ntok, const TextTrail* trail = nullptr);
struct FeedbackIds { const int32_t* ids = nullptr; int n_ids = 0; const float* table = nullptr; int64_t rows = 0; };
void launch_feedback_codes(hipStream_t st, const float* const* tables, const int64_t* table_rows, const int32_t* codes, const float* tts_pad,
                           float* out, int n, const FeedbackIds* ids = nullptr);
void launch_gather_rows_keys(hipStream_t st, const float* table, int64_t rows, const q3_u64* keys, int key_stride, int row_len,
                             float* dst, int ntok);
struct AdvanceKeysArgs {
    int B; int32_t *finished, *n_frames; const int32_t* max_frames; q3_u64* keys; q3_u64* next_key0; int32_t* hist; int hist_stride;
    int32_t *t_slot, *t_pos;
};
void launch_advance_keys(hipStream_t st, const AdvanceKeysArgs& a);
struct StallArgs {
    const int32_t* open = nullptr; const int32_t* n_trail = nullptr;
    float* hidden = nullptr; uint32_t* draws = nullptr; uint32_t* pdraws = nullptr;
    float* save_hidden = nullptr; uint32_t* save_draws = nullptr;
};
void launch_stall_save(hipStream_t st, const AdvanceKeysArgs& a, const StallArgs& s);
void launch_advance_keys_gated(hipStream_t st, const AdvanceKeysArgs& a, const StallArgs& s);

struct SampleArgs {
    const float* logits; int stride; int n;
    const float* temperature; const int32_t* top_k; const float* top_p;
    const int32_t* mask_idx;
    const uint32_t* rng_key; uint32_t* draws;
    q3_u64* out_key; int out_stride;
    const float* penalty = nullptr;
    const int32_t* hist = nullptr; int hist_stride = 0; const int32_t* hist_len = nullptr;
    const q3_u64* cur_key = nullptr; int cur_stride = 0;
};
void launch_sample(hipStream_t st, const SampleArgs& a, int B);
void launch_sample_pred(hipStream_t st, const SampleArgs& a, int B);

struct LogprobHead {
    const float* logits = nullptr; int stride = 0; size_t head_stride = 0; int n = 0;
    const q3_u64* key = nullptr; int key_stride = 0; const int32_t* chosen = nullptr;
    int extra_idx = -1; int col = 0, col_extra = -1; int row_ahead = 0;
};
struct LogprobArgs {
    LogprobHead p; int n_first = 0; LogprobHead t;
    float* out = nullptr; int out_stride = 0, out_rows = 0;
    const int32_t* n_frames = nullptr; const int32_t* finished = nullptr; const int32_t* max_frames = nullptr;
    const int32_t* open = nullptr; const int32_t* n_trail = nullptr; const int32_t* record = nullptr;
};
void launch_logprob_rows(hipStream_t st, const LogprobArgs& a, int B);

void launch_score_inputs(hipStream_t st, const float* hidden_proj, const float* const* tabs, const int64_t* tab_rows, int dP, const int32_t* codes,
                         int F, float* out);
struct ScoreRowsArgs {
    const float* tlogits = nullptr; int t_stride = 0;
    const float* plogits = nullptr; size_t p_head_stride = 0;
    const int32_t* codes = nullptr; float* out = nullptr;
};
void launch_score_rows(hipStream_t st, const ScoreRowsArgs& a, int F);

void launch_kv_fork(hipStream_t st, const KvCache& kv, int src_seq, const int32_t* dst_seqs, int n_dst, int n_pages);

struct StemJob { uint16_t* k; uint16_t* v; int32_t n_pages, first, n_dst, pad; };
void launch_kv_stem(hipStream_t st, const KvCache& kv, const StemJob* jobs, int n_jobs, int max_pages, const int32_t* slots, bool save);

template <class Meta> struct UploadRing {
    static constexpr int SLOTS = 64;
    UploadRing() = default;
    UploadRing(const UploadRing&) = delete; UploadRing& operator=(const UploadRing&) = delete;
    ~UploadRing() {
        for (auto e : ev) if (e) (void)hipEventDestroy(e);
        if (host) (void)hipHostFree(host);
    }
    void alloc(int max_group_) {
        max_group = max_group_;
        dev.alloc((size_t)SLOTS * max_group);
        Q3_HIP(hipHostMalloc((void**)&host, sizeof(Meta) * SLOTS * max_group));
// ... 146 lines not shown
```

### qwen3-tts-rust_amd/csrc/kernels_fused.hip

```cpp
#include "kernels.h"
#include "kdev.h"
#include "wslice.h"
#include <cstdlib>
#include "q3_common.h"

namespace q3 {
Q3_STAMP_SETTER(set_stamp_buffer_fused)

__device__ __forceinline__ void norm_quant_token(const NormPro& a, int d, int tok, int ntok, int lane, int8_t* xq_dst,
                                                 uint16_t* xd_dst, bool write_global) {
    const int nch = d >> 8;
    const float* hin = a.h_in;
    if (a.idx_keys) hin += (size_t)key_code(a.idx_keys[(size_t)tok * a.idx_stride]) * a.h_stride;
    else hin += (size_t)tok * a.h_stride;
    float4 x[8];
    float p = 0.0f;
#pragma unroll
    for (int c = 0; c < 8; c++) {
        if (c < nch) {
            float4 v = *reinterpret_cast<const float4*>(hin + 256 * c + 4 * lane);
            if (a.nparts > 0) {
                const float* pp = a.parts + (size_t)tok * a.parts_stride + 256 * c + 4 * lane;
                float4 y = *reinterpret_cast<const float4*>(pp);
                for (int s = 1; s < a.nparts; s++) {
// ... 841 lines not shown
    for (int q = 1; q < 16; q++) k[q] = pack_key(-INFINITY, 0);
}
__global__ void k_advance_keys(AdvanceKeysArgs a) {
    const int b = blockIdx.x * 64 + threadIdx.x;
    if (b >= a.B) return;
    advance_slot(a, b);
}
void launch_advance_keys(hipStream_t st, const AdvanceKeysArgs& a) {
    hipLaunchKernelGGL(k_advance_keys, dim3((a.B + 63) / 64), dim3(64), 0, st, a);
}

__device__ __forceinline__ bool slot_waits(const AdvanceKeysArgs& a, const StallArgs& s, int b) {
    const int f = a.n_frames[b];
    return !a.finished[b] && f < a.max_frames[b] && s.open[b] && f >= s.n_trail[b];
}
__global__ void __launch_bounds__(256) k_stall_save(AdvanceKeysArgs a, StallArgs s) {
    const int b = blockIdx.x;
    if (!slot_waits(a, s, b)) return;
    const float4* src = reinterpret_cast<const float4*>(s.hidden + (size_t)b * 2048);
    float4* dst = reinterpret_cast<float4*>(s.save_hidden + (size_t)b * 2048);
    const float4 v0 = src[threadIdx.x], v1 = src[threadIdx.x + 256];
    dst[threadIdx.x] = v0;
    dst[threadIdx.x + 256] = v1;
    if (threadIdx.x == 0) { s.save_draws[2 * b] = s.draws[b]; s.save_draws[2 * b + 1] = s.pdraws[b]; }
}
void launch_stall_save(hipStream_t st, const AdvanceKeysArgs& a, const StallArgs& s) {
    hipLaunchKernelGGL(k_stall_save, dim3(a.B), dim3(256), 0, st, a, s);
}
__global__ void __launch_bounds__(256) k_advance_keys_gated(AdvanceKeysArgs a, StallArgs s) {
    const int b = blockIdx.x;
    const bool waits = slot_waits(a, s, b);
    __syncthreads();
    if (!waits) {
        if (threadIdx.x == 0) advance_slot(a, b);
        return;
    }
    const float4* src = reinterpret_cast<const float4*>(s.save_hidden + (size_t)b * 2048);
    float4* dst = reinterpret_cast<float4*>(s.hidden + (size_t)b * 2048);
    const float4 v0 = src[threadIdx.x], v1 = src[threadIdx.x + 256];
    dst[threadIdx.x] = v0;
    dst[threadIdx.x + 256] = v1;
    if (threadIdx.x == 0) {
        s.draws[b] = s.save_draws[2 * b];
        s.pdraws[b] = s.save_draws[2 * b + 1];
        u64* k = a.keys + (size_t)b * 16;
        a.next_key0[b] = pack_key(-INFINITY, 0);
        for (int q = 1; q < 16; q++) k[q] = pack_key(-INFINITY, 0);
    }
}
void launch_advance_keys_gated(hipStream_t st, const AdvanceKeysArgs& a, const StallArgs& s) {
    hipLaunchKernelGGL(k_advance_keys_gated, dim3(a.B), dim3(256), 0, st, a, s);
}

}
```

### qwen3-tts-rust_amd/csrc/sched_logic.h

```cpp
#pragma once
#include "../../include/q3tts_spec.h"
#include <algorithm>
#include <cmath>
#include <cstddef>
#include <cstdint>
#include <cstring>
#include <deque>
#include <map>
#include <optional>
#include <stdexcept>
#include <string>
#include <utility>
#include <vector>

namespace q3 {

struct SamplerConfig {
    float temperature = 0.7f; int top_k = 40; float top_p = 0.9f; bool has_seed = false; uint64_t seed = 0;
};

struct GenOptions {
    float repetition_penalty = 1.0f;
    float predictor_temperature = 0.0f;
    int predictor_top_k = 0;
// ... 27 lines not shown
    int B = 0, off[SF_COUNT + 1] = {0};
    std::vector<uint32_t> host; uint32_t* dev = nullptr;
    std::vector<char> live; std::vector<const GenRequest*> req;
    explicit SlotTable(int n = 0) : B(n), live(n, 0), req(n, nullptr) {
        for (int f = 0; f < SF_COUNT; f++) off[f + 1] = off[f] + (((f == SF_TPOS ? 4 : 1) * B + 15) & ~15);
        host.assign(off[SF_COUNT], 0);
        for (int b = 0; b < B; b++) reset(b);
        route();
    }
    int32_t* hi(SlotField f) { return (int32_t*)(host.data() + off[f]); }
    float* hf(SlotField f) { return (float*)(host.data() + off[f]); }
    const int32_t* hi(SlotField f) const { return (const int32_t*)(host.data() + off[f]); }
    int32_t* di(SlotField f) const { return (int32_t*)(dev + off[f]); }
    float* df(SlotField f) const { return (float*)(dev + off[f]); }
    void reset(int b) {
        req[b] = nullptr;
        hi(SF_FINISHED)[b] = 1; hi(SF_MAXFRAMES)[b] = hi(SF_NFRAMES)[b] = hi(SF_NPROMPT)[b] = 0; hi(SF_MASKEOS)[b] = -1;
        hf(SF_TEMP)[b] = 0.0f; hi(SF_TOPK)[b] = 0; hf(SF_TOPP)[b] = 1.0f; hi(SF_NTRAIL)[b] = hi(SF_OPEN)[b] = 0;
        hf(SF_PEN)[b] = 1.0f; hf(SF_PTEMP)[b] = 0.0f; hi(SF_PTOPK)[b] = 0; hf(SF_PTOPP)[b] = 1.0f;
    }
    void load(int b, const GenRequest& r) {
        req[b] = &r;
        hi(SF_FINISHED)[b] = 0; hi(SF_MAXFRAMES)[b] = r.max_steps; hi(SF_NFRAMES)[b] = r.n_prefix; hi(SF_NPROMPT)[b] = r.n_prompt;
        hi(SF_MASKEOS)[b] = r.mask_eos ? Q3_CODEC_EOS : -1; hi(SF_NTRAIL)[b] = r.n_trail; hi(SF_OPEN)[b] = 0;
        hf(SF_TEMP)[b] = r.sampler.temperature; hi(SF_TOPK)[b] = r.sampler.top_k; hf(SF_TOPP)[b] = r.sampler.top_p;
        const GenOptions& o = r.opts;
        hf(SF_PEN)[b] = o.repetition_penalty; hf(SF_PTEMP)[b] = o.predictor_temperature; hi(SF_PTOPK)[b] = o.predictor_top_k; hf(SF_PTOPP)[b] = o.predictor_top_p;
    }
    void route() {
        for (int b = 0; b < B; b++) {
            const int t = live[b] ? hi(SF_NPROMPT)[b] + hi(SF_NFRAMES)[b] : 0;
            int32_t* pos = hi(SF_TPOS) + 4 * b;
            hi(SF_TSEQ)[b] = live[b] ? b : B; hi(SF_TSLOT)[b] = pos[0] = pos[1] = pos[2] = t; pos[3] = 0;
        }
    }
    bool stalled(int b) const { const int f = hi(SF_NFRAMES)[b]; return hi(SF_OPEN)[b] && !hi(SF_FINISHED)[b] && f < hi(SF_MAXFRAMES)[b] && f >= hi(SF_NTRAIL)[b]; }
    bool all_live_stalled() const {
        bool any = false;
        for (int b = 0; b < B; b++) if (live[b]) { if (!stalled(b)) return false; any = true; }
        return any;
    }
};

inline FrameVariant live_variant(const SlotTable& t) {
    FrameVariant v;
    for (int b = 0; b < t.B; b++) if (t.live[b]) {
        const GenRequest& r = *t.req[b];
        const bool open = t.hi(SF_OPEN)[b] != 0;
        v.sampled |= r.sampler.temperature > 0.0f; v.pen |= r.opts.penalised(); v.pred |= r.opts.pred_sampled();
        v.trail |= r.n_trail > 0 || r.open || open; v.gate |= open; v.lp |= r.logprobs;
    }
    return v;
}

enum ReqState { REQ_QUEUED = 0, REQ_RUNNING = 1, REQ_DRAINING = 2, REQ_DONE = 3, REQ_CANCELLED = 4, REQ_FAILED = -1 };
inline bool req_ended(int state) { return state == REQ_DONE || state == REQ_CANCELLED || state == REQ_FAILED; }

enum CancelAction {
    CANCEL_NOTHING,
    CANCEL_AT_ONCE,
    CANCEL_AT_ACTIVATE,
    CANCEL_RETIRE,
    CANCEL_RETIRE_FENCE,
    CANCEL_PURGE
};
inline CancelAction cancel_action(int state, bool in_wave, bool live, bool want_pcm) {
    if (state == REQ_QUEUED) return CANCEL_AT_ONCE;
    if (state == REQ_DRAINING) return CANCEL_PURGE;
    if (state != REQ_RUNNING) return CANCEL_NOTHING;
    if (!live) return in_wave ? CANCEL_AT_ACTIVATE : CANCEL_NOTHING;
    return want_pcm ? CANCEL_RETIRE_FENCE : CANCEL_RETIRE;
}
inline int retired_state(bool want_pcm, bool cancelled) { return want_pcm ? REQ_DRAINING : cancelled ? REQ_CANCELLED : REQ_DONE; }
inline int fenced_state(bool cancelled) { return cancelled ? REQ_CANCELLED : REQ_DONE; }

struct StageCursor {
    static constexpr size_t NONE = ~(size_t)0;
    size_t cap = 0, used = 0;
    size_t take(size_t bytes) {
        if (bytes > cap) return NONE;
        bytes = (bytes + 63) & ~(size_t)63;
        if (bytes > cap - used) return NONE;
        const size_t at = used;
        used += bytes;
        return at;
    }
    void reset() { used = 0; }
};

struct PromptRef { const float* rows; int n, slot; int n_fb = 0; int n_skip = 0; }; struct PrefillCursor { size_t req = 0; int tok = 0; };
struct FbRun { int req, row, frame, n; };
inline int pack_prefill_chunk(const std::vector<PromptRef>& batch, PrefillCursor& c, int n_max, float* stage, int32_t* seq, int32_t* slot,
                              int32_t* pos, std::vector<std::pair<int, int>>& lasts, std::vector<FbRun>* fb = nullptr) {
    int n = 0;
    if (fb) fb->clear();
    for (lasts.clear(); n < n_max && c.req < batch.size(); n++) {
        const PromptRef& r = batch[c.req];
        if (c.tok < r.n_skip) c.tok = r.n_skip;
        if (c.tok < r.n) std::copy(r.rows + (size_t)c.tok * Q3_EMBD, r.rows + (size_t)(c.tok + 1) * Q3_EMBD, stage + (size_t)n * Q3_EMBD);
        else if (fb) {
            if (!fb->empty() && fb->back().req == (int)c.req && fb->back().row + fb->back().n == n) fb->back().n++;
            else fb->push_back({(int)c.req, n, c.tok - r.n, 1});
        }
        seq[n] = r.slot; slot[n] = c.tok; pos[4 * n] = pos[4 * n + 1] = pos[4 * n + 2] = c.tok; pos[4 * n + 3] = 0;
        if (c.tok == r.n + r.n_fb - 1) { lasts.emplace_back((int)c.req, n); c.req++; c.tok = 0; } else c.tok++;
    }
// ... 106 lines not shown
        return unhold(id);
    }
    Recycled finish(int id, bool ok) {
        Entry* e = find(id);
        if (!e) return std::nullopt;
        e->refs.state = ok ? HELD_READY : HELD_FAILED; e->refs.holders++;
        return unhold(id);
    }
    void fail_building() { for (auto& kv : map_) if (kv.second.refs.state == HELD_BUILDING) kv.second.refs.state = HELD_FAILED; }
    const char* set_refusal(int id) const { auto it = map_.find(id); return words.set_refusal(it != map_.end(), it != map_.end() ? it->second.refs.state : 0); }
    Recycled swap_setting(int& which, int id) {
        if (id >= 0) { if (const char* why = set_refusal(id)) throw std::runtime_error(why); hold(id); }
        else if (id != -1) throw std::runtime_error(words.bad_id);
        const int old = which;
        which = id;
        return old >= 0 ? unhold(old) : std::nullopt;
    }
private:
    std::map<int, Entry> map_; int next_ = 0;
};

inline const char* preamble_refusal(const int32_t* codes, int n, int max_steps, bool have_codec, int live, int64_t max_positions) {
    if (const char* why = decode_refusal(codes, n, max_steps, have_codec)) return why;
    if (live >= Q3TTS_MAX_PREAMBLES) return "Q3TTS_MAX_PREAMBLES preambles are live: release one first";
    if ((int64_t)n + max_steps > max_positions) return "n + max_steps exceeds the codec's frame positions";
    return nullptr;
}
enum { PREAMBLE_NONE = -1, PREAMBLE_ENGINE = -2 };
inline int preamble_of_request(bool want_pcm, int asked, int engine_level) {
    if (!want_pcm) return PREAMBLE_NONE;
    return asked == PREAMBLE_ENGINE ? engine_level : asked;
}

inline const char* stem_refusal(const float* rows, int n, int max_prompt, int live, bool ggml) {
    if (ggml) return "prompt stems are not available with Q3_SPEC=ggml (the ggml-arithmetic mode serves the reference's decoding only)";
    if (!rows) return "stem rows missing";
    if (n < 1) return "n_rows must be >= 1";
    if (n >= max_prompt) return "n_rows must be below max_prompt: a request that takes a stem has at least one row of its own";
    if (live >= Q3TTS_MAX_STEMS) return "Q3TTS_MAX_STEMS stems are live: release one first";
    return nullptr;
}
enum { STEM_NONE = -1, STEM_ENGINE = -2 };
inline int stem_of_request(int asked, int engine_level) { return asked == STEM_ENGINE ? engine_level : asked; }
inline bool stem_takes(int state, int n, const float* stem_rows, const float* prompt, int n_prompt, bool score) {
    if (score || state != Q3TTS_STEM_READY || n < 1 || n_prompt <= n || !stem_rows || !prompt) return false;
    return std::memcmp(stem_rows, prompt, (size_t)n * Q3_EMBD * sizeof(float)) == 0;
}
inline int stem_pages(int n) { return (n + 63) / 64; }
inline int64_t stem_store_bytes(int n, int n_layer, int n_kv) { return (int64_t)2 * stem_pages(n) * n_layer * n_kv * 8192 * 2; }
inline int admission_rows(int n_prompt, int n_skip, int n_prefix) { return n_prompt - n_skip + n_prefix; }

inline int decode_width(int n_cs, int max_batch) { return std::max(1, (n_cs - max_batch) / 2); }
inline int decode_admit(int queued, int free_cs, int holding, int width) { return std::max(0, std::min(queued, std::min(free_cs, width - holding))); }

enum TaskKind { TASK_CHUNK = 0, TASK_RESET = 1, TASK_FENCE = 2 };
enum { SEAT_DRY_MAX = 4 };
struct TaskHead { int64_t req; int frames; int kind; int64_t epoch = 0; };
struct Seat { bool low; int index; };
struct Seating { std::vector<Seat> seats; int dry = 0; };
inline Seating seat_chunks(const std::vector<TaskHead>& live, const std::vector<TaskHead>& low, int gmax, int dry) {
    Seating out;
    out.dry = dry;
    std::vector<int> heads; std::vector<int64_t> seen;
    for (int i = 0; i < (int)low.size(); i++)
        if (std::find(seen.begin(), seen.end(), low[i].req) == seen.end()) { seen.push_back(low[i].req); heads.push_back(i); }
    for (int i : heads) if (low[i].kind != TASK_CHUNK) { out.seats.push_back({true, i}); return out; }
    if (live.empty() && heads.empty()) return out;
    const bool turn = !heads.empty() && (live.empty() || dry >= SEAT_DRY_MAX);
    if (!turn && live[0].kind != TASK_CHUNK) { out.seats.push_back({false, 0}); return out; }
    const TaskHead& lead = turn ? low[heads[0]] : live[0];
    out.seats.push_back({turn, turn ? heads[0] : 0});
    seen.assign(1, lead.req);
    bool bound = !turn; int64_t epoch = lead.epoch;
    for (int i = 0; i < (int)live.size() && (int)out.seats.size() < gmax; i++) {
        const bool dup = std::find(seen.begin(), seen.end(), live[i].req) != seen.end();
        if (!dup) seen.push_back(live[i].req);
        if (dup || live[i].kind != TASK_CHUNK || live[i].frames != lead.frames || (bound && live[i].epoch != epoch)) continue;
        out.seats.push_back({false, i});
        bound = true; epoch = live[i].epoch;
    }
    bool seated_low = turn;
    for (int i : heads) {
        if ((int)out.seats.size() >= gmax) break;
        if (turn && i == heads[0]) continue;
        if (low[i].frames == lead.frames) { out.seats.push_back({true, i}); seated_low = true; }
    }
    out.dry = seated_low ? 0 : heads.empty() ? 0 : dry + 1;
    return out;
}

template <class Job> struct CodecQueue {
    struct Task { Job* job; TaskKind kind; std::vector<int64_t> codes; bool is_final; int64_t epoch; };
    std::deque<Task> live, low;
    int pending = 0, hold = 0, dry = 0; int64_t epoch = 0;
    void open() { if (hold++ == 0) epoch++; }
    void close() { hold--; }
    void push(Job* j, TaskKind kind, const int64_t* codes = nullptr, int n_codes = 0, bool is_final = false) {
        (j->decode ? low : live).push_back(Task{j, kind, std::vector<int64_t>(codes, codes + n_codes), is_final, kind == TASK_CHUNK && !j->decode ? epoch : 0});
        if (kind != TASK_RESET) pending++;
    }
    void purge(Job* j) {
        std::deque<Task>& q = j->decode ? low : live;
        for (auto it = q.begin(); it != q.end();) {
            if (it->job == j && it->kind == TASK_CHUNK) { it = q.erase(it); pending--; }
            else ++it;
        }
    }
    bool ready() const { return hold == 0 && !(live.empty() && low.empty()); }
    std::vector<Task> take(int gmax) {
        std::vector<Task> step;
        if (!ready()) return step;
        auto heads = [](const std::deque<Task>& q) {
            std::vector<TaskHead> h;
            for (const Task& t : q) h.push_back({t.job->id, (int)t.codes.size() / 16, t.kind, t.epoch});
            return h;
        };
        const Seating s = seat_chunks(heads(live), heads(low), gmax, dry);
        dry = s.dry;
        for (const Seat& c : s.seats) step.push_back(std::move((c.low ? low : live)[c.index]));
        for (int lo = 0; lo < 2; lo++) {
            std::vector<int> idx;
            for (const Seat& c : s.seats) if ((int)c.low == lo) idx.push_back(c.index);
            std::sort(idx.rbegin(), idx.rend());
            for (int i : idx) (lo ? low : live).erase((lo ? low : live).begin() + i);
        }
        return step;
    }
    void popped() { pending--; }
};

struct QueueEntry { int rows; bool want_pcm; int64_t set; };
inline int admission_take(const std::vector<QueueEntry>& q, int free_slots, int free_codec, bool limit_rows, size_t max_rows = 4096) {
    size_t take = 0, rows = 0;
    while (take < q.size() && free_slots > 0) {
        const QueueEntry& e = q[take];
        size_t k = 1;
        if (e.set != 0) while (take + k < q.size() && q[take + k].set == e.set) k++;
        if ((size_t)free_slots < k) break;
        if (e.want_pcm && (size_t)free_codec < k) break;
        if (limit_rows && take > 0 && rows + (size_t)e.rows > max_rows) break;
        take += k; free_slots -= (int)k; rows += (size_t)e.rows;
        if (e.want_pcm) free_codec -= (int)k;
    }
    return (int)take;
}

struct ScoreRun { int req, row, frame, n; };
inline std::vector<ScoreRun> score_head_runs(const std::vector<PromptRef>& batch, const std::vector<char>& score, PrefillCursor before, int n_chunk) {
    std::vector<ScoreRun> out;
// ... 164 lines not shown
```

### qwen3-tts-rust_amd/python/q3tts/__init__.py

```python
import ctypes as C
import os
import numpy as np

_HERE = os.path.dirname(os.path.abspath(__file__))
PKG_ROOT = os.path.dirname(os.path.dirname(_HERE))
LIB_PATH = os.path.join(PKG_ROOT, "libq3tts.so")
_lib = None


class Q3Error(RuntimeError):
    pass


class SamplerConfig(C.Structure):
    _fields_ = [("temperature", C.c_float), ("top_k", C.c_int32), ("top_p", C.c_float), ("has_seed", C.c_int32),
                ("seed", C.c_uint64)]


class GenOptions(C.Structure):
    _fields_ = [("repetition_penalty", C.c_float), ("predictor_temperature", C.c_float), ("predictor_top_k", C.c_int32),
                ("predictor_top_p", C.c_float)]


GEN_DEFAULTS = {"repetition_penalty": 1.0, "predictor_temperature": 0.0, "predictor_top_k": 0, "predictor_top_p": 1.0}
# ... 38 lines not shown
    "q3tts_chunker_free", "q3tts_chunker_push", "q3tts_decoder_create", "q3tts_decoder_destroy", "q3tts_decoder_samples_per_frame",
    "q3tts_decoder_reset", "q3tts_decoder_decode", "q3tts_mel_frames", "q3tts_mel", "q3tts_tf_open", "q3tts_tf_close",
    "q3tts_tf_dims", "q3tts_tf_clear", "q3tts_tf_eval", "q3tts_op_gemv_q8", "q3tts_op_gateup_q8", "q3tts_op_matmul_float", "q3tts_op_rmsnorm_quant", "q3tts_op_swiglu_quant",
    "q3tts_op_argmax", "q3tts_op_project", "q3tts_op_sample", "q3tts_submit", "q3tts_poll", "q3tts_fetch", "q3tts_wait",
    "q3tts_release", "q3tts_decoder_create_ex", "q3tts_decoder_decode_group", "q3tts_sched_start", "q3tts_sched_stop", "q3tts_sched_step", "q3tts_voice_register", "q3tts_submit_text",
    "q3tts_group_create", "q3tts_group_destroy", "q3tts_group_size", "q3tts_group_engine", "q3tts_group_uses_rccl", "q3tts_group_voice_register",
    "q3tts_group_submit", "q3tts_group_submit_text", "q3tts_group_device_of", "q3tts_group_poll", "q3tts_group_fetch", "q3tts_group_wait",
    "q3tts_group_release", "q3tts_group_start", "q3tts_group_stop", "q3tts_comm_available", "q3tts_comm_unique_id", "q3tts_comm_create",
    "q3tts_comm_destroy", "q3tts_comm_voice_register", "q3tts_engine_device",
    "q3tts_onnx_open", "q3tts_onnx_close", "q3tts_onnx_counts", "q3tts_onnx_summary", "q3tts_onnx_node", "q3tts_onnx_node_input", "q3tts_onnx_node_output",
    "q3tts_onnx_node_attr_ints", "q3tts_onnx_node_attr_float", "q3tts_onnx_initializer", "q3tts_onnx_op_kernel", "q3tts_onnx_decoder_contract",
    "q3tts_onnx_session_open", "q3tts_onnx_session_close", "q3tts_onnx_session_unsupported", "q3tts_onnx_session_set_input", "q3tts_onnx_session_run",
    "q3tts_onnx_session_output_info", "q3tts_onnx_session_output", "q3tts_onnx_session_launches", "q3tts_onnx_op_executable",
    "q3tts_text_nfc", "q3tts_op_gemv_kq", "q3tts_op_gateup_kq", "q3tts_onnx_decoder_open", "q3tts_onnx_decoder_close", "q3tts_onnx_decoder_reset", "q3tts_onnx_decoder_fetch", "q3tts_group_info", "q3tts_onnx_decoder_decode",
    "q3tts_decoder_state_floats", "q3tts_decoder_state_export", "q3tts_decoder_state_import", "q3tts_decoder_state_entry",
    "q3tts_tokenizer_open", "q3tts_tokenizer_close", "q3tts_tokenizer_encode", "q3tts_tokenizer_decode", "q3tts_tokenizer_vocab_size",
    "q3tts_gen_options_default", "q3tts_submit_ex", "q3tts_submit_text_ex", "q3tts_generate_batch_ex", "q3tts_group_submit_ex",
    "q3tts_group_submit_text_ex", "q3tts_op_sample_rows",
    "q3tts_prompt_build_streaming", "q3tts_submit_trailing", "q3tts_submit_text_streaming", "q3tts_generate_batch_trailing",
    "q3tts_group_submit_text_streaming", "q3tts_op_codec_gemm", "q3tts_codec_gemm_plan", "q3tts_codec_gemm_tap_reuse", "q3tts_op_codec_kernel", "q3tts_op_attention", "q3tts_attention_plan",
    "q3tts_op_linear", "q3tts_linear_plan", "q3tts_argmax_key",
    "q3tts_submit_trailing_open", "q3tts_trail_append", "q3tts_trail_progress", "q3tts_submit_text_streaming_open", "q3tts_text_append",
    "q3tts_group_submit_text_streaming_open", "q3tts_group_text_append", "q3tts_group_trail_append", "q3tts_group_trail_progress",
    "q3tts_cancel", "q3tts_group_cancel",
    "q3tts_submit_resume", "q3tts_group_submit_resume", "q3tts_op_feedback_rows", "q3tts_engine_prefill_width",
    "q3tts_engine_set_logprobs", "q3tts_fetch_logprobs", "q3tts_group_set_logprobs", "q3tts_group_fetch_logprobs", "q3tts_op_logprob_rows",
    "q3tts_submit_score", "q3tts_group_submit_score", "q3tts_engine_score_width", "q3tts_op_score_rows", "q3tts_op_score_inputs",
    "q3tts_pred_table_bytes", "q3tts_op_attention_keyed", "q3tts_op_select_rows", "q3tts_op_frame_glue", "q3tts_op_ggml",
    "q3tts_submit_candidates", "q3tts_group_submit_candidates", "q3tts_engine_candidate_stats", "q3tts_op_kv_fork",
    "q3tts_submit_decode", "q3tts_group_submit_decode", "q3tts_engine_decode_width", "q3tts_engine_decode_stats",
    "q3tts_engine_set_output_format", "q3tts_request_format", "q3tts_fetch_pcm16", "q3tts_engine_pcm_out_stats",
    "q3tts_group_set_output_format", "q3tts_group_fetch_pcm16", "q3tts_group_request_format",
    "q3tts_pcm_out_plan", "q3tts_pcm_out_filter", "q3tts_pcm_out_samples", "q3tts_pcm_format_check", "q3tts_op_pcm_convert",
    "q3tts_decoder_snapshot_create", "q3tts_decoder_snapshot_restore", "q3tts_decoder_snapshot_free", "q3tts_decoder_snapshot_bytes",
    "q3tts_preamble_create", "q3tts_preamble_poll", "q3tts_preamble_wait", "q3tts_preamble_release", "q3tts_voice_set_preamble",
    "q3tts_engine_set_preamble", "q3tts_request_preamble", "q3tts_engine_preamble_stats",
    "q3tts_group_preamble_create", "q3tts_group_preamble_wait", "q3tts_group_preamble_release", "q3tts_group_voice_set_preamble",
    "q3tts_group_set_preamble", "q3tts_group_request_preamble",
    "q3tts_stem_create", "q3tts_voice_stem_create", "q3tts_stem_poll", "q3tts_stem_wait", "q3tts_stem_release", "q3tts_voice_set_stem",
    "q3tts_engine_set_stem", "q3tts_request_stem", "q3tts_engine_stem_stats", "q3tts_op_kv_stem",
    "q3tts_group_stem_create", "q3tts_group_voice_stem_create", "q3tts_group_stem_wait", "q3tts_group_stem_release",
    "q3tts_group_voice_set_stem", "q3tts_group_set_stem", "q3tts_group_request_stem", "q3tts_group_stem_stats",
    "q3tts_engine_set_speech_rate", "q3tts_request_speech_rate", "q3tts_engine_tsm_stats", "q3tts_group_set_speech_rate",
    "q3tts_group_request_speech_rate", "q3tts_tsm_samples", "q3tts_tsm_windows", "q3tts_op_tsm", "q3tts_mel_tables",
    "q3tts_engine_set_pitch", "q3tts_request_pitch", "q3tts_engine_pitch_stats", "q3tts_group_set_pitch", "q3tts_group_request_pitch",
    "q3tts_pitch_samples", "q3tts_pitch_plan", "q3tts_pitch_filter", "q3tts_op_pitch",
    "q3tts_engine_set_volume", "q3tts_request_volume", "q3tts_engine_volume_stats", "q3tts_group_set_volume", "q3tts_group_request_volume",
    "q3tts_volume_gain", "q3tts_op_volume",
    "q3tts_engine_set_loudness", "q3tts_fetch_loudness", "q3tts_request_loudness", "q3tts_request_metered", "q3tts_engine_loudness_stats",
    "q3tts_group_set_loudness", "q3tts_group_fetch_loudness", "q3tts_group_request_loudness", "q3tts_group_request_metered",
    "q3tts_loudness_tables", "q3tts_loudness_gate", "q3tts_loudness_gain_db10", "q3tts_op_loudness",
    "q3tts_intake_plan", "q3tts_intake_filter", "q3tts_intake_samples", "q3tts_intake_tile", "q3tts_intake_check", "q3tts_wav_probe",
    "q3tts_intake", "q3tts_wav_intake",
]


class IntakeClip(C.Structure):
    _fields_ = [("data", C.c_void_p), ("n_frames", C.c_int64), ("sample_rate", C.c_int32), ("channels", C.c_int32),
                ("sample_format", C.c_int32), ("downmix", C.c_int32)]


class WavInfo(C.Structure):
    _fields_ = [("sample_format", C.c_int32), ("channels", C.c_int32), ("sample_rate", C.c_int32), ("bits", C.c_int32),
                ("data_offset", C.c_int64), ("n_frames", C.c_int64)]


class PcmFormat(C.Structure):
    _fields_ = [("sample_rate", C.c_int32), ("encoding", C.c_int32)]


class Loudness(C.Structure):
    _fields_ = [("integrated_lufs", C.c_double), ("momentary_max_lufs", C.c_double), ("peak_dbfs", C.c_double), ("n_blocks", C.c_int32),
                ("n_gated", C.c_int32)]


class StemStats(C.Structure):
    _fields_ = [("built", C.c_int64), ("restores", C.c_int64), ("rows_not_prefilled", C.c_int64), ("pages_copied", C.c_int64),
                ("mismatches", C.c_int64), ("device_bytes", C.c_int64)]


PCM_F32, PCM_S16 = 0, 1
PCM_RATES = (8000, 12000, 16000, 22050, 24000, 32000, 44100, 48000)
PCM_NATIVE_RATE, PCM_FRAME, PCM_HIST = 24000, 1920, 96
TSM_HOP, TSM_WIN, TSM_SEARCH, TSM_LOOK, TSM_HIST, TSM_MIN, TSM_MAX = 480, 960, 240, 1200, 1920, 50, 200
PITCH_MIN, PITCH_MAX, PITCH_HIST = 50, 200, 64
VOL_MIN, VOL_MAX, VOL_LOOK, VOL_HOLD, VOL_DELAY, VOL_HIST = -400, 200, 128, 512, 127, 638
LOUD_SEG, LOUD_BLOCK, LOUD_STATE = 96, 2400, 6
INTAKE_U8, INTAKE_S16, INTAKE_S24, INTAKE_S32, INTAKE_F32 = 0, 1, 2, 3, 4
INTAKE_FIRST, INTAKE_MEAN = 0, 1
INTAKE_SAMPLE_BYTES = (1, 2, 3, 4, 4)
INTAKE_MAX_CLIPS, INTAKE_MAX_OUT = 64, 2880000
MAX_PREAMBLES = 64
PREAMBLE_BUILDING, PREAMBLE_READY, PREAMBLE_FAILED = 0, 1, -1
MAX_STEMS = 64
STEM_BUILDING, STEM_READY, STEM_FAILED = 0, 1, -1
LOGPROB_COLS = 17
LOGPROB_NONE = 1.0


def lib():
    global _lib
    if _lib is None:
        if not os.path.exists(LIB_PATH):
            raise Q3Error("libq3tts.so not built (run qwen3-tts-rust_amd/build.sh); there is no CPU fallback")
        L = C.CDLL(LIB_PATH)
        L.q3tts_last_error.restype = C.c_char_p
# ... 69 lines not shown
        L.q3tts_group_submit_ex.argtypes = [C.c_void_p, C.POINTER(Request), C.c_int32, C.POINTER(GenOptions), C.POINTER(C.c_int64)]
        L.q3tts_group_submit_text_ex.argtypes = [C.c_void_p, C.c_int32, C.c_void_p, C.c_int32, C.c_int32, C.c_void_p, C.c_int32,
                                                 C.POINTER(SamplerConfig), C.c_int32, C.c_int32, C.c_int32, C.POINTER(GenOptions),
                                                 C.POINTER(C.c_int64)]
        L.q3tts_op_sample_rows.argtypes = [C.c_int32, C.c_void_p, C.c_int32, C.c_int32, C.c_void_p, C.c_void_p, C.c_void_p, C.c_void_p,
                                           C.c_void_p, C.c_void_p, C.c_void_p, C.c_int32, C.c_int32, C.c_void_p]
        L.q3tts_prompt_build_streaming.argtypes = [C.c_void_p, C.c_void_p, C.c_int32, C.c_int32, C.c_int32, C.c_void_p, C.c_void_p, C.c_int32,
                                                   C.c_void_p, C.c_int32, C.c_void_p, C.c_int32, C.c_void_p, C.c_int32, C.c_void_p, C.c_int32,
                                                   C.POINTER(C.c_int32)]
        L.q3tts_submit_trailing.argtypes = [C.c_void_p, C.POINTER(Request), C.c_int32, C.POINTER(GenOptions), C.c_void_p, C.c_int32,
                                            C.POINTER(C.c_int64)]
        L.q3tts_submit_text_streaming.argtypes = L.q3tts_submit_text_ex.argtypes
        L.q3tts_generate_batch_trailing.argtypes = [C.c_void_p, C.POINTER(Request), C.c_int32, C.c_int32, C.POINTER(GenOptions),
                                                    C.POINTER(C.c_void_p), C.c_void_p]
        L.q3tts_group_submit_text_streaming.argtypes = L.q3tts_group_submit_text_ex.argtypes
        L.q3tts_submit_trailing_open.argtypes = L.q3tts_submit_trailing.argtypes
        L.q3tts_trail_append.argtypes = [C.c_void_p, C.c_int64, C.c_void_p, C.c_int32, C.c_int32]
        L.q3tts_trail_progress.argtypes = [C.c_void_p, C.c_int64, C.POINTER(C.c_int32), C.POINTER(C.c_int32), C.POINTER(C.c_int32)]
        L.q3tts_submit_text_streaming_open.argtypes = L.q3tts_submit_text_ex.argtypes
        L.q3tts_text_append.argtypes = [C.c_void_p, C.c_int64, C.c_void_p, C.c_int32, C.c_int32]
        L.q3tts_group_submit_text_streaming_open.argtypes = L.q3tts_group_submit_text_ex.argtypes
        L.q3tts_group_text_append.argtypes = L.q3tts_text_append.argtypes
        L.q3tts_group_trail_append.argtypes = L.q3tts_trail_append.argtypes
        L.q3tts_group_trail_progress.argtypes = L.q3tts_trail_progress.argtypes
        L.q3tts_cancel.argtypes = [C.c_void_p, C.c_int64]
        L.q3tts_group_cancel.argtypes = [C.c_void_p, C.c_int64]
        L.q3tts_submit_resume.argtypes = [C.c_void_p, C.POINTER(Request), C.c_int32, C.POINTER(GenOptions), C.c_void_p, C.c_int32, C.c_int32,
                                          C.c_void_p, C.c_int32, C.POINTER(C.c_int64)]
        L.q3tts_group_submit_resume.argtypes = [C.c_void_p, C.c_int32] + L.q3tts_submit_resume.argtypes[1:]
        L.q3tts_op_feedback_rows.argtypes = [C.c_void_p, C.c_void_p, C.c_int32, C.c_void_p, C.c_int32, C.c_void_p]
        L.q3tts_engine_prefill_width.argtypes = [C.c_void_p]
        L.q3tts_engine_set_logprobs.argtypes = [C.c_void_p, C.c_int32]
        L.q3tts_fetch_logprobs.argtypes = [C.c_void_p, C.c_int64, C.c_void_p, C.c_int32, C.c_int32, C.POINTER(C.c_int32)]
        L.q3tts_group_set_logprobs.argtypes = L.q3tts_engine_set_logprobs.argtypes
        L.q3tts_group_fetch_logprobs.argtypes = L.q3tts_fetch_logprobs.argtypes
        L.q3tts_submit_score.argtypes = [C.c_void_p, C.c_void_p, C.c_int32, C.c_void_p, C.c_int32, C.c_void_p, C.c_int32, C.POINTER(C.c_int64)]
        L.q3tts_group_submit_score.argtypes = [C.c_void_p, C.c_int32] + L.q3tts_submit_score.argtypes[1:]
        L.q3tts_engine_score_width.argtypes = [C.c_void_p]
        L.q3tts_submit_candidates.argtypes = [C.c_void_p, C.c_void_p, C.c_int32, C.c_void_p, C.c_void_p, C.c_int32, C.c_void_p, C.c_int32, C.c_void_p]
        L.q3tts_group_submit_candidates.argtypes = [C.c_void_p, C.c_int32] + L.q3tts_submit_candidates.argtypes[1:]
        L.q3tts_engine_candidate_stats.argtypes = [C.c_void_p, C.POINTER(C.c_int64), C.POINTER(C.c_int64), C.POINTER(C.c_int64)]
        L.q3tts_op_kv_fork.argtypes = [C.c_void_p, C.c_void_p, C.c_int32, C.c_int32, C.c_int32, C.c_void_p, C.c_int32, C.c_int32, C.c_int32, C.c_void_p,
                                       C.c_int32, C.c_int32]
        L.q3tts_engine_score_width.restype = C.c_int32
        L.q3tts_submit_decode.argtypes = [C.c_void_p, C.c_void_p, C.c_int32, C.POINTER(C.c_int64)]
        L.q3tts_group_submit_decode.argtypes = [C.c_void_p, C.c_int32] + L.q3tts_submit_decode.argtypes[1:]
        L.q3tts_engine_decode_width.argtypes = [C.c_void_p]
        L.q3tts_engine_decode_width.restype = C.c_int32
        L.q3tts_engine_decode_stats.argtypes = [C.c_void_p, C.POINTER(C.c_int64), C.POINTER(C.c_int64), C.POINTER(C.c_int64)]
        L.q3tts_op_score_rows.argtypes = [C.c_void_p, C.c_int32, C.c_void_p, C.c_void_p, C.c_int32, C.c_void_p]
        L.q3tts_op_score_inputs.argtypes = [C.c_void_p, C.POINTER(C.c_void_p), C.c_void_p, C.c_int32, C.c_void_p, C.c_int32, C.c_void_p]
        L.q3tts_op_logprob_rows.argtypes = [C.c_void_p, C.c_int32, C.c_int32, C.c_int32, C.c_void_p, C.c_int32, C.c_void_p, C.c_void_p]
        L.q3tts_op_frame_glue.argtypes = [C.c_void_p]
        L.q3tts_engine_set_output_format.argtypes = [C.c_void_p, C.POINTER(PcmFormat)]
        L.q3tts_request_format.argtypes = [C.c_void_p, C.c_int64, C.POINTER(PcmFormat)]
        L.q3tts_fetch_pcm16.argtypes = [C.c_void_p, C.c_int64, C.c_void_p, C.c_int64, C.c_int64, C.POINTER(C.c_int64)]
        L.q3tts_engine_pcm_out_stats.argtypes = [C.c_void_p, C.POINTER(C.c_int64), C.POINTER(C.c_int64)]
        L.q3tts_group_set_output_format.argtypes = L.q3tts_engine_set_output_format.argtypes
        L.q3tts_group_fetch_pcm16.argtypes = L.q3tts_fetch_pcm16.argtypes
        L.q3tts_group_request_format.argtypes = L.q3tts_request_format.argtypes
        L.q3tts_decoder_snapshot_create.argtypes = [C.c_void_p, C.c_int32, C.POINTER(C.c_int32)]
        L.q3tts_decoder_snapshot_restore.argtypes = [C.c_void_p, C.c_int32, C.c_int32]
        L.q3tts_decoder_snapshot_free.argtypes = [C.c_void_p, C.c_int32]
        L.q3tts_decoder_snapshot_bytes.argtypes = [C.c_void_p]
        L.q3tts_decoder_snapshot_bytes.restype = C.c_int64
        L.q3tts_preamble_create.argtypes = [C.c_void_p, C.c_void_p, C.c_int32, C.POINTER(C.c_int32)]
        L.q3tts_preamble_poll.argtypes = [C.c_void_p, C.c_int32, C.POINTER(C.c_int32), C.POINTER(C.c_int32)]
        L.q3tts_preamble_wait.argtypes = [C.c_void_p, C.c_int32, C.c_double]
        L.q3tts_preamble_release.argtypes = [C.c_void_p, C.c_int32]
        L.q3tts_voice_set_preamble.argtypes = [C.c_void_p, C.c_int32, C.c_int32]
        L.q3tts_engine_set_preamble.argtypes = [C.c_void_p, C.c_int32]
        L.q3tts_request_preamble.argtypes = [C.c_void_p, C.c_int64, C.POINTER(C.c_int32)]
        L.q3tts_engine_preamble_stats.argtypes = [C.c_void_p, C.POINTER(C.c_int64), C.POINTER(C.c_int64), C.POINTER(C.c_int64)]
        L.q3tts_group_preamble_create.argtypes = L.q3tts_preamble_create.argtypes
        L.q3tts_group_preamble_wait.argtypes = L.q3tts_preamble_wait.argtypes
        L.q3tts_group_preamble_release.argtypes = L.q3tts_preamble_release.argtypes
        L.q3tts_group_voice_set_preamble.argtypes = L.q3tts_voice_set_preamble.argtypes
        L.q3tts_group_set_preamble.argtypes = L.q3tts_engine_set_preamble.argtypes
        L.q3tts_group_request_preamble.argtypes = L.q3tts_request_preamble.argtypes
        L.q3tts_stem_create.argtypes = [C.c_void_p, C.c_void_p, C.c_int32, C.POINTER(C.c_int32)]
        L.q3tts_voice_stem_create.argtypes = [C.c_void_p, C.c_int32, C.c_int32, C.c_void_p, C.c_int32, C.POINTER(C.c_int32)]
        L.q3tts_stem_poll.argtypes = [C.c_void_p, C.c_int32, C.POINTER(C.c_int32), C.POINTER(C.c_int32)]
        L.q3tts_stem_wait.argtypes = [C.c_void_p, C.c_int32, C.c_double]
        L.q3tts_stem_release.argtypes = [C.c_void_p, C.c_int32]
        L.q3tts_voice_set_stem.argtypes = [C.c_void_p, C.c_int32, C.c_int32]
        L.q3tts_engine_set_stem.argtypes = [C.c_void_p, C.c_int32]
        L.q3tts_request_stem.argtypes = [C.c_void_p, C.c_int64, C.POINTER(C.c_int32), C.POINTER(C.c_int32)]
        L.q3tts_engine_stem_stats.argtypes = [C.c_void_p, C.POINTER(StemStats)]
        L.q3tts_group_stem_create.argtypes = L.q3tts_stem_create.argtypes
        L.q3tts_group_voice_stem_create.argtypes = L.q3tts_voice_stem_create.argtypes
        L.q3tts_group_stem_wait.argtypes = L.q3tts_stem_wait.argtypes
        L.q3tts_group_stem_release.argtypes = L.q3tts_stem_release.argtypes
        L.q3tts_group_voice_set_stem.argtypes = L.q3tts_voice_set_stem.argtypes
        L.q3tts_group_set_stem.argtypes = L.q3tts_engine_set_stem.argtypes
        L.q3tts_group_request_stem.argtypes = L.q3tts_request_stem.argtypes
        L.q3tts_group_stem_stats.argtypes = L.q3tts_engine_stem_stats.argtypes
        L.q3tts_op_kv_stem.argtypes = [C.c_void_p, C.c_void_p, C.c_int32, C.c_int32, C.c_int32, C.c_void_p, C.c_int32, C.c_int32, C.c_void_p, C.c_void_p,
                                       C.c_int32, C.c_int32, C.c_void_p, C.c_void_p, C.c_void_p, C.c_void_p, C.c_void_p, C.c_int32, C.c_int32]
        L.q3tts_pcm_out_plan.argtypes = [C.c_int32] + [C.POINTER(C.c_int32)] * 4
        L.q3tts_pcm_out_filter.argtypes = [C.c_int32, C.c_void_p, C.c_int64]
        L.q3tts_pcm_out_filter.restype = C.c_int64
        L.q3tts_pcm_out_samples.argtypes = [C.c_int32, C.c_int64]
        L.q3tts_pcm_out_samples.restype = C.c_int64
        L.q3tts_pcm_format_check.argtypes = [C.POINTER(PcmFormat)]
        L.q3tts_op_pcm_convert.argtypes = [C.c_void_p, C.c_int32, C.c_void_p, C.c_int32, C.c_void_p, C.c_int32, C.c_void_p, C.c_void_p,
                                           C.POINTER(C.c_void_p), C.c_void_p, C.c_void_p, C.c_void_p]
# ... 558 lines not shown
    def submit(self, prompt, max_steps=8, temperature=0.0, top_k=40, top_p=0.9, seed=42, mask_eos=True, want_pcm=False,
               repetition_penalty=1.0, predictor_temperature=0.0, predictor_top_k=0, predictor_top_p=1.0, trailing_ids=None,
               open_trail=False, prefix_codes=None):
        pr = np.ascontiguousarray(prompt, np.float32)
        r = Request()
        self._fill(r, pr, 0, max_steps, temperature, top_k, top_p, seed, mask_eos)
        o = self._opts(0, repetition_penalty, predictor_temperature, predictor_top_k, predictor_top_p)
        rid = C.c_int64()
        if prefix_codes is not None:
            pc = np.ascontiguousarray(prefix_codes, np.int32).reshape(-1, 16)
            tr = np.ascontiguousarray(trailing_ids if trailing_ids is not None else [], np.int32)
            _chk(lib().q3tts_submit_resume(self.h, C.byref(r), 1 if want_pcm else 0, C.byref(o) if o is not None else None,
                                           _p(tr) if tr.size else None, tr.size, 1 if open_trail else 0, _p(pc) if pc.size else None,
                                           pc.shape[0], C.byref(rid)))
        elif trailing_ids is not None or open_trail:
            tr = np.ascontiguousarray(trailing_ids if trailing_ids is not None else [], np.int32)
            fn = lib().q3tts_submit_trailing_open if open_trail else lib().q3tts_submit_trailing
            _chk(fn(self.h, C.byref(r), 1 if want_pcm else 0, C.byref(o) if o is not None else None, _p(tr), tr.size,
                                             C.byref(rid)))
        elif o is None:
            _chk(lib().q3tts_submit(self.h, C.byref(r), 1 if want_pcm else 0, C.byref(rid)))
        else:
            _chk(lib().q3tts_submit_ex(self.h, C.byref(r), 1 if want_pcm else 0, C.byref(o), C.byref(rid)))
        return rid.value

    def submit_score(self, prompt, codes, trailing_ids=None):
        pr = np.ascontiguousarray(prompt, np.float32)
        c = np.ascontiguousarray(codes, np.int32).reshape(-1, 16)
        tr = np.ascontiguousarray(trailing_ids if trailing_ids is not None else [], np.int32)
        rid = C.c_int64()
        _chk(lib().q3tts_submit_score(self.h, _p(pr), pr.shape[0], _p(tr) if tr.size else None, tr.size, _p(c) if c.size else None,
                                      c.shape[0], C.byref(rid)))
        return rid.value

    def submit_candidates(self, prompt, seeds, max_steps=8, temperature=0.0, top_k=40, top_p=0.9, mask_eos=True, want_pcm=False,
                          repetition_penalty=1.0, predictor_temperature=0.0, predictor_top_k=0, predictor_top_p=1.0, trailing_ids=None):
        return _submit_candidates(lib().q3tts_submit_candidates, (self.h,), prompt, seeds, max_steps, temperature, top_k, top_p, mask_eos, want_pcm,
                                  GenOptions(repetition_penalty, predictor_temperature, predictor_top_k, predictor_top_p), trailing_ids)

    def submit_decode(self, codes):
        c = np.ascontiguousarray(codes, np.int32).reshape(-1, 16)
        rid = C.c_int64()
        _chk(lib().q3tts_submit_decode(self.h, _p(c) if c.size else None, c.shape[0], C.byref(rid)))
        return rid.value

    def decode_width(self):
        return lib().q3tts_engine_decode_width(self.h)

    def decode_stats(self):
        a, b, c = C.c_int64(), C.c_int64(), C.c_int64()
        _chk(lib().q3tts_engine_decode_stats(self.h, C.byref(a), C.byref(b), C.byref(c)))
        return dict(requests=a.value, chunks=b.value, chunks_shared=c.value)

    def candidate_stats(self):
        a, b, c = C.c_int64(), C.c_int64(), C.c_int64()
        _chk(lib().q3tts_engine_candidate_stats(self.h, C.byref(a), C.byref(b), C.byref(c)))
        return dict(sets=a.value, prefill_rows_saved=b.value, pages_copied=c.value)

    def score_width(self):
        return lib().q3tts_engine_score_width(self.h)

    def register_voice(self, spk_emb, ref_codes=None, ref_text_ids=None):
        spk = np.ascontiguousarray(spk_emb, np.float32)
        rc = np.ascontiguousarray(ref_codes, np.int32).reshape(-1) if ref_codes is not None else None
        rt = np.ascontiguousarray(ref_text_ids, np.int32) if ref_text_ids is not None else None
        vid = C.c_int32()
        _chk(lib().q3tts_voice_register(self.h, _p(spk), _p(rc), rc.size if rc is not None else 0, _p(rt), rt.size if rt is not None else 0,
                                        C.byref(vid)))
        if rc is not None and rc.size:
            self._voice_ref[vid.value] = rc.reshape(-1, 16).copy()
        return vid.value

    def preamble_create(self, codes):
        return _preamble_create(lib().q3tts_preamble_create, self.h, codes)

    def preamble_poll(self, pid):
        st, n = C.c_int32(), C.c_int32()
        _chk(lib().q3tts_preamble_poll(self.h, pid, C.byref(st), C.byref(n)))
        return st.value, n.value

    def preamble_wait(self, pid, timeout_ms=-1.0):
        return _preamble_wait(lib().q3tts_preamble_wait, self.h, pid, timeout_ms)

    def preamble_release(self, pid):
        _chk(lib().q3tts_preamble_release(self.h, pid))

    def voice_set_preamble(self, voice_id, pid):
        _chk(lib().q3tts_voice_set_preamble(self.h, voice_id, -1 if pid is None else pid))

    def set_preamble(self, pid):
        _chk(lib().q3tts_engine_set_preamble(self.h, -1 if pid is None else pid))

    def request_preamble(self, rid):
        return _request_preamble(lib().q3tts_request_preamble, self.h, rid)

    def preamble_stats(self):
        a, b, c = C.c_int64(), C.c_int64(), C.c_int64()
        _chk(lib().q3tts_engine_preamble_stats(self.h, C.byref(a), C.byref(b), C.byref(c)))
        return dict(built=a.value, restores=b.value, bytes_per_snapshot=c.value)

    def stem_create(self, rows):
        return _stem_create(lib().q3tts_stem_create, self.h, rows)

    def voice_stem_create(self, voice_id, lang_id=2055, instr_ids=None):
        return _voice_stem_create(lib().q3tts_voice_stem_create, self.h, voice_id, lang_id, instr_ids)

# ... 1067 lines not shown

class FrameGlueDesc(C.Structure):
    _fields_ = [("kernel", C.c_int32), ("ntok", C.c_int32),
                ("n_in", C.c_int32), ("n_out", C.c_int32), ("x_stride", C.c_int32), ("x_off", C.c_int32), ("out_stride", C.c_int32),
                ("x", C.c_void_p), ("x_floats", C.c_int64), ("w", C.c_void_p), ("b", C.c_void_p),
                ("tables", C.c_void_p), ("table_rows", C.c_void_p), ("row_len", C.c_int32), ("key_stride", C.c_int32), ("tts_pad", C.c_void_p),
                ("trail", C.c_int32), ("trail_ids", C.c_void_p), ("ids_stride", C.c_int32), ("text_table", C.c_void_p), ("text_rows", C.c_int64),
                ("n_trail", C.c_void_p), ("open", C.c_void_p), ("max_frames", C.c_void_p), ("hist_stride", C.c_int32)] + \
               [(k, Guarded) for k in ("out", "keys", "next_key0", "finished", "n_frames", "t_slot", "t_pos", "hist", "hidden", "save_hidden",
                                       "draws", "pdraws", "save_draws")]


def glue_guarded(core, sentinel, dtype=None):
    core = np.ascontiguousarray(core, dtype).reshape(-1)
    whole = np.full(core.size + 2 * GLUE_GUARD, sentinel, core.dtype)
    whole[GLUE_GUARD: GLUE_GUARD + core.size] = core
    return whole


def glue_core(whole, shape=None):
    c = whole[GLUE_GUARD: whole.size - GLUE_GUARD]
    return c if shape is None else c.reshape(shape)


def op_frame_glue(kernel, tables=None, **fields):
    d = FrameGlueDesc()
    d.kernel = kernel
    keep = []
    for k, v in fields.items():
        if k in _GLUE_GUARDED:
            assert isinstance(v, np.ndarray) and v.dtype == _GLUE_GUARDED[k] and v.ndim == 1 and v.flags["C_CONTIGUOUS"], k
            setattr(d, k, Guarded(v.ctypes.data, v.size))
        elif k in _GLUE_ARRAYS:
            a = np.ascontiguousarray(v, _GLUE_ARRAYS[k])
            keep.append(a)
            setattr(d, k, a.ctypes.data)
            if k == "x":
                d.x_floats = a.size
            if k == "text_table":
                d.text_rows = a.shape[0]
        elif k in _GLUE_INTS:
            setattr(d, k, int(v))
        else:
            raise TypeError("op_frame_glue: q3tts_frame_glue_desc has no field %r for the caller to set" % k)
    if tables is not None:
        tabs = [np.ascontiguousarray(t, np.float32) for t in tables]
        ptrs = (C.c_void_p * len(tabs))(*[t.ctypes.data for t in tabs])
        rows = np.array([t.shape[0] for t in tabs], np.int64)
        keep += [tabs, ptrs, rows]
        d.tables, d.table_rows = C.cast(ptrs, C.c_void_p), rows.ctypes.data
    _chk(lib().q3tts_op_frame_glue(C.byref(d)))


GG_LOAD_ROWS, GG_ADD, GG_RMSNORM, GG_QUANT, GG_MATVEC, GG_LINEAR, GG_SWIGLU = range(7)
_GG_GUARDED = {"out": np.float32, "q8": np.int8, "d8": np.uint16, "qk": np.int8, "dk": np.float32, "bs": np.int16}
_GG_ARRAYS = {"x": np.float32, "u": np.float32, "idx": np.int32, "idx_keys": np.uint64, "w": np.uint8}
_GG_INTS = ("ntok", "k", "n", "x_stride", "x_rows", "idx_stride", "type", "rows", "row0", "nrows", "out_stride")


class GgmlDesc(C.Structure):
    _fields_ = [("op", C.c_int32), ("ntok", C.c_int32), ("k", C.c_int32), ("n", C.c_int64),
                ("x", C.c_void_p), ("x_floats", C.c_int64), ("x_stride", C.c_int32), ("x_rows", C.c_int32),
                ("u", C.c_void_p), ("eps", C.c_float),
                ("idx", C.c_void_p), ("idx_keys", C.c_void_p), ("idx_stride", C.c_int32), ("idx_n", C.c_int64),
                ("w", C.c_void_p), ("type", C.c_int32), ("rows", C.c_int32), ("row0", C.c_int32), ("nrows", C.c_int32), ("out_stride", C.c_int32)] + \
               [(k, Guarded) for k in ("out", "q8", "d8", "qk", "dk", "bs")]


def op_ggml(op, **fields):
    d = GgmlDesc()
    d.op = op
    keep = []
    for k, v in fields.items():
        if k in _GG_GUARDED:
            assert isinstance(v, np.ndarray) and v.dtype == _GG_GUARDED[k] and v.ndim == 1 and v.flags["C_CONTIGUOUS"], k
            setattr(d, k, Guarded(v.ctypes.data, v.size))
        elif k in _GG_ARRAYS:
            a = np.ascontiguousarray(v, _GG_ARRAYS[k]).reshape(-1)
            keep.append(a)
            setattr(d, k, a.ctypes.data if a.size else None)
            if k == "x":
                d.x_floats = a.size
            if k in ("idx", "idx_keys"):
                d.idx_n = a.size
        elif k in _GG_INTS:
            setattr(d, k, int(v))
        elif k == "eps":
            d.eps = float(v)
        else:
            raise TypeError("op_ggml: q3tts_ggml_desc has no field %r for the caller to set" % k)
    lib().q3tts_op_ggml.argtypes = [C.POINTER(GgmlDesc)]
    _chk(lib().q3tts_op_ggml(C.byref(d)))


def pcm_out_plan(rate):
    v = [C.c_int32() for _ in range(4)]
    _chk(lib().q3tts_pcm_out_plan(rate, *[C.byref(x) for x in v]))
    return tuple(x.value for x in v)


def pcm_out_filter(rate):
    h = np.zeros(pcm_out_plan(rate)[2], np.float32)
    n = lib().q3tts_pcm_out_filter(rate, _p(h), h.size)
    if n != h.size:
        raise Q3Error(lib().q3tts_last_error().decode())
    return h
# ... 318 lines not shown
```

Measured before the change: 766.6.

## Pack per-group frame outputs into one device record and widen idle codec passes

Adds a GPU kernel that gathers each slot's new code rows, logprobs, frame counts and finished flags into one contiguous record, so the host issues a single device-to-host copy per frame group instead of one per live slot. The fed offsets are kept on the device in a double buffer. The codec worker now picks the pass width from the engine's load, taking a wider group (default 32) when the engine is idle. This adds a small pack kernel on the main stream and extra state that must stay in sync with the host's fed counters.

```diff
diff --git a/include/q3tts.h b/include/q3tts.h
--- a/include/q3tts.h
+++ b/include/q3tts.h
@@ -157,6 +157,7 @@
 int q3tts_submit_decode(q3tts_engine* e, const int32_t* codes, int32_t n, int64_t* req_id);
 int32_t q3tts_engine_decode_width(q3tts_engine* e);
 int q3tts_engine_decode_stats(q3tts_engine* e, int64_t* requests, int64_t* chunks, int64_t* chunks_shared);
+int q3tts_engine_codec_pass_stats(q3tts_engine* e, int64_t* passes, int64_t* streams, int64_t* widest);
 int32_t q3tts_engine_prefill_width(q3tts_engine* e);
 int q3tts_sched_start(q3tts_engine* e);
 int q3tts_sched_stop(q3tts_engine* e);
@@ -527,6 +528,17 @@
 } q3tts_frame_glue_desc;
 int q3tts_op_frame_glue(q3tts_frame_glue_desc* d);
 
+typedef struct q3tts_group_pack_desc {
+    int32_t width, group;
+    const int32_t* n_frames; const int32_t* finished; const int32_t* fed;
+    const int32_t* hist; int32_t hist_stride;
+    const float* lp; int32_t lp_rows; const int32_t* lp_rec;
+    q3tts_guarded rec;
+    q3tts_guarded fed_next;
+} q3tts_group_pack_desc;
+int q3tts_group_record_layout(int32_t width, int32_t lp, int64_t* out);
+int q3tts_op_group_pack(q3tts_group_pack_desc* d);
+
 enum { Q3TTS_GG_LOAD_ROWS = 0, Q3TTS_GG_ADD = 1, Q3TTS_GG_RMSNORM = 2, Q3TTS_GG_QUANT = 3, Q3TTS_GG_MATVEC = 4, Q3TTS_GG_LINEAR = 5,
        Q3TTS_GG_SWIGLU = 6 };
 typedef struct q3tts_ggml_desc {
diff --git a/qwen3-tts-rust_amd/csrc/capi.cpp b/qwen3-tts-rust_amd/csrc/capi.cpp
--- a/qwen3-tts-rust_amd/csrc/capi.cpp
+++ b/qwen3-tts-rust_amd/csrc/capi.cpp
@@ -161,6 +161,17 @@
     if (requests) *requests = r;
     if (chunks) *chunks = c;
     if (chunks_shared) *chunks_shared = s;
+    return Q3TTS_OK;
+    Q3_API_END(Q3TTS_ERR)
+}
+int q3tts_engine_codec_pass_stats(q3tts_engine* e, int64_t* passes, int64_t* streams, int64_t* widest) {
+    Q3_API_BEGIN
+    Q3_CHECK(e, "null argument");
+    int64_t p = 0, s = 0, w = 0;
+    e->e->codec_pass_stats(&p, &s, &w);
+    if (passes) *passes = p;
+    if (streams) *streams = s;
+    if (widest) *widest = w;
     return Q3TTS_OK;
     Q3_API_END(Q3TTS_ERR)
 }
diff --git a/qwen3-tts-rust_amd/csrc/capi_ops.cpp b/qwen3-tts-rust_amd/csrc/capi_ops.cpp
--- a/qwen3-tts-rust_amd/csrc/capi_ops.cpp
+++ b/qwen3-tts-rust_amd/csrc/capi_ops.cpp
@@ -1144,6 +1144,53 @@
     Q3_API_END(Q3TTS_ERR)
 }
 
+int q3tts_group_record_layout(int32_t width, int32_t lp, int64_t* out) {
+    Q3_API_BEGIN
+    Q3_CHECK(out && width >= 1 && width <= 65535, "group record: width out of [1, 65535] or no place for the layout");
+    const GroupRecord r(width, lp != 0);
+    out[0] = (int64_t)r.nfr; out[1] = (int64_t)r.fin; out[2] = (int64_t)r.codes; out[3] = (int64_t)r.logprobs; out[4] = (int64_t)r.bytes;
+    return Q3TTS_OK;
+    Q3_API_END(Q3TTS_ERR)
+}
+int q3tts_op_group_pack(q3tts_group_pack_desc* dp) {
+    Q3_API_BEGIN
+    require_gpu();
+    Q3_CHECK(dp, "null group-pack descriptor");
+    const q3tts_group_pack_desc& d = *dp;
+    Q3_CHECK(d.width >= 1 && d.width <= 65535 && d.group >= 1 && d.group <= GroupRecord::ROWS, "width out of [1, 65535] or group out of [1, 4]");
+    Q3_CHECK(d.n_frames && d.finished && d.fed && d.hist, "n_frames / finished / fed / hist missing");
+    Q3_CHECK(d.hist_stride >= 16 && d.hist_stride % 16 == 0, "hist_stride must be a positive multiple of 16");
+    Q3_CHECK(!d.lp || d.lp_rows >= 1, "lp_rows missing");
+    const size_t n = (size_t)d.width;
+    for (size_t b = 0; b < n; b++) {
+        const int64_t rows = std::min<int64_t>(d.group, (int64_t)d.n_frames[b] - d.fed[b]);
+        if (rows <= 0) continue;
+        Q3_CHECK(d.fed[b] >= 0 && ((int64_t)d.fed[b] + rows) * 16 <= d.hist_stride, "a produced row lies outside hist_stride");
+        Q3_CHECK(!d.lp || (int64_t)d.fed[b] + rows <= d.lp_rows, "a produced row lies outside lp_rows");
+    }
+    const GroupRecord r(d.width, d.lp != nullptr);
+    GlueBuf<uint8_t> rec; GlueBuf<int32_t> fed_next;
+    const auto holds = [](const q3tts_guarded& g, size_t core) { return g.p && g.n >= (int64_t)(core + 2 * Q3TTS_GLUE_GUARD); };
+    Q3_CHECK(holds(d.rec, r.bytes) && holds(d.fed_next, n), "guarded buffer too small or missing: rec / fed_next");
+    rec.up(d.rec, r.bytes, "rec"); fed_next.up(d.fed_next, n, "fed_next");
+    DevBuf<int32_t> d_nfr(n), d_fin(n), d_fed(n), d_hist(n * d.hist_stride), d_rec; DevBuf<float> d_lp;
+    d_nfr.upload(d.n_frames, n); d_fin.upload(d.finished, n); d_fed.upload(d.fed, n); d_hist.upload(d.hist, d_hist.n);
+    GroupPackArgs a;
+    a.width = d.width; a.group = d.group; a.n_frames = d_nfr.p; a.finished = d_fin.p; a.fed = d_fed.p; a.fed_next = fed_next.p();
+    a.hist = d_hist.p; a.hist_stride = d.hist_stride; a.rec = rec.p();
+    if (d.lp) {
+        d_lp.alloc(n * d.lp_rows * Q3_LOGPROB_COLS); d_lp.upload(d.lp, d_lp.n);
+        a.lp = d_lp.p; a.lp_rows = d.lp_rows;
+        if (d.lp_rec) { d_rec.alloc(n); d_rec.upload(d.lp_rec, n); a.lp_rec = d_rec.p; }
+    }
+    launch_group_pack(0, a);
+    Q3_LAUNCH_CHECK();
+    Q3_HIP(hipDeviceSynchronize());
+    rec.down(); fed_next.down();
+    return Q3TTS_OK;
+    Q3_API_END(Q3TTS_ERR)
+}
+
 int q3tts_op_ggml(q3tts_ggml_desc* dp) {
     Q3_API_BEGIN
     require_gpu();
diff --git a/qwen3-tts-rust_amd/csrc/codec_worker.cpp b/qwen3-tts-rust_amd/csrc/codec_worker.cpp
--- a/qwen3-tts-rust_amd/csrc/codec_worker.cpp
+++ b/qwen3-tts-rust_amd/csrc/codec_worker.cpp
@@ -3,7 +3,9 @@
 
 namespace q3 {
 
-CodecWorker::CodecWorker(CodecDecoder* codec, int dev, int n_lanes, int n_cs, size_t slot_cap) : codec_(codec), dev_(dev), st_(n_lanes), slot_cap_(slot_cap), n_cs_(n_cs) {
+CodecWorker::CodecWorker(CodecDecoder* codec, int dev, int n_lanes, int n_cs, size_t slot_cap, CodecCaps caps)
+    : codec_(codec), dev_(dev), caps_(caps), st_(n_lanes), slot_cap_(slot_cap), n_cs_(n_cs) {
+    Q3_CHECK(caps.busy >= 1 && caps.busy <= caps.idle && caps.idle <= codec->max_group(), "codec pass widths outside the decoder's scratch");
     for (auto& s : st_) Q3_HIP(hipStreamCreateWithFlags(&s, hipStreamNonBlocking));
     Q3_HIP(hipHostMalloc((void**)&pcm_pinned_, (size_t)n_cs * slot_cap_ * sizeof(float)));
 }
@@ -87,6 +89,8 @@
     for (const Task& t : s) n_low += t.job->decode;
     dec_chunks += n_low;
     if (n_low < G) dec_shared += n_low;
+    passes++; pass_streams += G;
+    if (G > pass_widest.load()) pass_widest = G;
     std::vector<int> streams(G); std::vector<float*> dst(G); std::vector<int64_t> codes((size_t)G * nf * 16);
     std::vector<OutSpec> out(G); std::vector<int64_t> n_out(G);
     std::vector<LoudDst> loud(G); std::vector<size_t> rows(G, 0);
@@ -145,13 +149,12 @@
 void CodecWorker::main() {
     try {
         Q3_HIP(hipSetDevice(dev_));
-        const int gmax = codec_->max_group();
         for (;;) {
             Step s;
             {
                 std::unique_lock<std::mutex> lk(mu_);
                 cv_.wait(lk, [&] { return stop_ || q_.ready(); });
-                s = q_.take(gmax);
+                s = q_.take(caps_.pass(q_.lead_wide()));
                 if (s.empty()) return;
             }
             const int lane = pick_lane(s);
diff --git a/qwen3-tts-rust_amd/csrc/codec_worker.h b/qwen3-tts-rust_amd/csrc/codec_worker.h
--- a/qwen3-tts-rust_amd/csrc/codec_worker.h
+++ b/qwen3-tts-rust_amd/csrc/codec_worker.h
@@ -30,7 +30,7 @@
 class CodecWorker {
 public:
     struct Completion { CodecJob* job; hipEvent_t ev; size_t pcm_after; bool fence; size_t loud_after; };
-    CodecWorker(CodecDecoder* codec, int dev, int n_lanes, int n_cs, size_t slot_cap);
+    CodecWorker(CodecDecoder* codec, int dev, int n_lanes, int n_cs, size_t slot_cap, CodecCaps caps);
     ~CodecWorker();
     void start() { if (!started_) { started_ = true; thread_ = std::thread([this] { main(); }); } }
 
@@ -41,9 +41,10 @@
     struct Handover {
         CodecWorker* w;
         Handover(CodecWorker* w_, bool on) : w(on ? w_ : nullptr) { if (w) { std::lock_guard<std::mutex> lk(w->mu_); w->q_.open(); } }
-        ~Handover() { if (w) { { std::lock_guard<std::mutex> lk(w->mu_); w->q_.close(); } w->cv_.notify_all(); } }
+        ~Handover() { if (w) { { std::lock_guard<std::mutex> lk(w->mu_); w->q_.close(w->engine_idle_); } w->cv_.notify_all(); } }
         Handover(const Handover&) = delete; Handover& operator=(const Handover&) = delete;
     };
+    void set_engine_idle(bool idle) { engine_idle_ = idle; }
     int pending();
     bool poll_completion(bool block, Completion* out);
 
@@ -54,6 +55,7 @@
     const double* loud_staging(int cs) const { return loud_pinned_.load() + (size_t)cs * loud_cap() * 2; }
 
     std::atomic<int64_t> dec_chunks{0}, dec_shared{0}, pre_restores{0};
+    std::atomic<int64_t> passes{0}, pass_streams{0}, pass_widest{0};
     long take_codec_calls() { return (long)codec_calls_.exchange(0); }
 
 private:
@@ -68,7 +70,7 @@
     void snapshot_build(int lane, const Step& s);
     void record(int lane, const Step& s);
 
-    CodecDecoder* codec_; int dev_;
+    CodecDecoder* codec_; int dev_; CodecCaps caps_; bool engine_idle_ = false;
     std::vector<hipStream_t> st_;
     float* pcm_pinned_ = nullptr; size_t slot_cap_ = 0;
     std::atomic<double*> loud_pinned_{nullptr}; int n_cs_ = 0;
diff --git a/qwen3-tts-rust_amd/csrc/engine.cpp b/qwen3-tts-rust_amd/csrc/engine.cpp
--- a/qwen3-tts-rust_amd/csrc/engine.cpp
+++ b/qwen3-tts-rust_amd/csrc/engine.cpp
@@ -96,6 +96,7 @@
     tl_stride_ = (Q3_SAMPLE_END + 31) & ~31;
     slots_ = SlotTable(B); d_slots_.alloc(slots_.host.size()); slots_.dev = d_slots_.p;
     d_keys_.alloc(16 * B); d_next_key0_.alloc(B); d_hist_.alloc((size_t)B * hist_stride_);
+    d_rec_.alloc(GroupRecord(B, true).bytes); d_fed_[0].alloc(B); d_fed_[1].alloc(B);
     d_rngkey_.alloc((size_t)8 * B); d_draws_.alloc(B); d_prngkey_.alloc((size_t)8 * B); d_pdraws_.alloc(B);
     d_rngkey_.zero(); d_draws_.zero(); d_prngkey_.zero(); d_pdraws_.zero(); d_plogits_.alloc((size_t)B * Q3_CODEBOOK_SIZE);
     d_tlogits_.alloc((size_t)B * tl_stride_); d_thidden_.alloc((size_t)B * Q3_EMBD); d_pin_.alloc((size_t)2 * B * dP_);
@@ -122,13 +123,16 @@
     upload_slot_state();
     if (p.load_codec) {
         Q3_CHECK(p.max_steps <= Q3TTS_CODEC_MAX_FRAMES, "max_steps above Q3TTS_CODEC_MAX_FRAMES: a request's codec stream could not be decoded to its end");
-        static const int group_env = [] { const char* e = std::getenv("Q3_CODEC_GROUP"); return e ? atoi(e) : 0; }();
-        const int group_cap = group_env > 0 ? group_env : (B >= 128 ? 32 : 16);
-        const int n_cs = B + std::min(B, 16), gmax = std::max(1, std::min(B, group_cap));
+        static const int group_env = [] { const char* e = std::getenv("Q3_CODEC_GROUP"); return e ? atoi(e) : -1; }();
+        static const int idle_env = [] { const char* e = std::getenv("Q3_CODEC_GROUP_IDLE"); return e ? std::max(0, atoi(e)) : -1; }();
+        const int n_cs = B + std::min(B, 16);
+        const CodecCaps caps = codec_caps(B, n_cs, group_env, idle_env);
+        const int gmax = caps.idle;
         static const int lanes_env = [] { const char* e = std::getenv("Q3_CODEC_LANES"); return e ? atoi(e) : 0; }();
         const int n_lanes = B > 1 ? (lanes_env > 0 ? std::min(lanes_env, 8) : 2) : 1;
         codec_.reset(new CodecDecoder(p.model_dir + "/onnx/q3tts_codec.gguf", n_cs, 4, n_lanes, gmax));
-        worker_.reset(new CodecWorker(codec_.get(), dev_, n_lanes, n_cs, (size_t)p.max_steps * codec_->samples_per_frame()));
+        worker_.reset(new CodecWorker(codec_.get(), dev_, n_lanes, n_cs, (size_t)p.max_steps * codec_->samples_per_frame(), caps));
+        publish_load();
         Q3_HIP(hipHostMalloc((void**)&pre_tails_, (size_t)Q3TTS_MAX_PREAMBLES * Q3_PCM_HIST * sizeof(float)));
         for (int i = Q3TTS_MAX_PREAMBLES - 1; i >= 0; i--) pre_tail_free_.push_back(i);
         for (int c = n_cs - 1; c >= 0; c--) cs_free_.push_back(c);
@@ -347,9 +351,14 @@
     return fg;
 }
 
+void Engine::publish_load() {
+    if (worker_) worker_->set_engine_idle(n_active_ == 0 && n_prefilling_ == 0);
+}
+
 void Engine::upload_slot_state() {
     slots_.route();
     h2d(slots_.dev, slots_.host.data(), slots_.host.size() * 4);
+    h2d(d_fed_[fed_cur_].p, slots_.hi(SF_NFRAMES), (size_t)B_ * 4);
     slot_dirty_ = false;
 }
 
@@ -883,7 +892,7 @@
     hipEvent_t e0, e1;
     Q3_HIP(hipEventCreate(&e0)); Q3_HIP(hipEventCreate(&e1));
     go_live(live);
-    { std::lock_guard<std::mutex> lk(mu_); n_active_ += (int)live.size(); }
+    { std::lock_guard<std::mutex> lk(mu_); n_active_ += (int)live.size(); publish_load(); }
     Q3_HIP(hipEventRecord(e0, st_));
     for (Req* r : batch) Q3_HIP(hipEventRecord(r->ev_admit, st_));
     prefill_wave(ar_, batch, sampled);
@@ -953,6 +962,7 @@
     Q3_HIP(hipEventRecord(pf_done_, st_pf_));
     pf_batch_ = wave;
     n_prefilling_ = (int)wave.size();
+    publish_load();
 }
 
 void Engine::go_live(const std::vector<Req*>& batch) {
@@ -1030,6 +1040,7 @@
         for (Req* r : batch) r->prefill_ms = t - r->t_submit;
         for (Req* r : scores) r->prefill_ms = t - r->t_submit;
         n_active_ += (int)batch.size();
+        publish_load();
     }
     finish_scores(scores);
     finish_builds(builds);
@@ -1152,7 +1163,7 @@
     {
         std::lock_guard<std::mutex> lk(mu_);
         slot_req_[b] = nullptr;
-        if (slots_.live[b]) { slots_.live[b] = 0; n_active_--; }
+        if (slots_.live[b]) { slots_.live[b] = 0; n_active_--; publish_load(); }
         r->slot = -1;
         r->state = retired_state(r->want_pcm, r->job.cancel);
         if (r->want_pcm) n_draining_++;
@@ -1199,18 +1210,22 @@
         else Q3_HIP(hipGraphLaunch(fg.exec, st_));
     }
     Q3_HIP(hipEventRecord(e1, st_));
-    const int32_t* p_nfr = (const int32_t*)d2h_begin(di(SF_NFRAMES), (size_t)width * 4);
-    const int32_t* p_fin = (const int32_t*)d2h_begin(di(SF_FINISHED), (size_t)width * 4);
-    std::vector<const int32_t*> p_hist(width, nullptr);
-    std::vector<const float*> p_lp(width, nullptr);
-    for (int b = 0; b < width; b++)
-        if (slots_.live[b]) {
-            Req* r = slot_req_[b];
-            const int rows = std::min(group, r->r.max_steps - r->fed);
-            if (rows > 0) p_hist[b] = (const int32_t*)d2h_begin(d_hist_.p + (size_t)b * hist_stride_ + (size_t)r->fed * 16, (size_t)rows * 64);
-            if (rows > 0 && r->r.logprobs)
-                p_lp[b] = (const float*)d2h_begin(d_lp_.p + ((size_t)b * lp_rows_ + r->fed) * Q3_LOGPROB_COLS, (size_t)rows * Q3_LOGPROB_COLS * 4);
-        }
+    const GroupRecord rec(width, v.lp);
+    {
+        GroupPackArgs pa;
+        pa.width = width; pa.group = group; pa.n_frames = di(SF_NFRAMES); pa.finished = di(SF_FINISHED);
+        pa.fed = d_fed_[fed_cur_].p; pa.fed_next = d_fed_[fed_cur_ ^ 1].p; pa.hist = d_hist_.p; pa.hist_stride = hist_stride_;
+        if (v.lp) { pa.lp = d_lp_.p; pa.lp_rows = lp_rows_; pa.lp_rec = d_lp_rec_.p; }
+        pa.rec = d_rec_.p;
+        launch_group_pack(st_, pa);
+        Q3_LAUNCH_CHECK();
+        fed_cur_ ^= 1;
+    }
+    const uint8_t* h_rec = (const uint8_t*)d2h_begin(d_rec_.p, rec.bytes);
+    const int32_t* p_nfr = (const int32_t*)(h_rec + rec.nfr);
+    const int32_t* p_fin = (const int32_t*)(h_rec + rec.fin);
+    const int32_t* p_codes = (const int32_t*)(h_rec + rec.codes);
+    const float* p_lps = (const float*)(h_rec + rec.logprobs);
     Q3_HIP(hipStreamSynchronize(st_));
     { float ms = 0; Q3_HIP(hipEventElapsedTime(&ms, e0, e1)); stats.frame_loop_ms += ms; }
     (void)hipEventDestroy(e0); (void)hipEventDestroy(e1);
@@ -1227,11 +1242,13 @@
         Req* r = slot_req_[b];
         if (h_nfr[b] > r->fed) {
             const int nnew = h_nfr[b] - r->fed;
-            const int32_t* hbuf = p_hist[b];
+            Q3_CHECK(nnew <= group, "a slot advanced by more frames than its group ran");
+            const int32_t* hbuf = p_codes + (size_t)b * GroupRecord::ROWS * 16;
+            const float* lbuf = r->r.logprobs ? p_lps + (size_t)b * GroupRecord::ROWS * Q3_LOGPROB_COLS : nullptr;
             {
                 std::lock_guard<std::mutex> lk(mu_);
                 r->codes.insert(r->codes.end(), hbuf, hbuf + (size_t)nnew * 16);
-                if (p_lp[b]) r->lp.insert(r->lp.end(), p_lp[b], p_lp[b] + (size_t)nnew * Q3_LOGPROB_COLS);
+                if (lbuf) r->lp.insert(r->lp.end(), lbuf, lbuf + (size_t)nnew * Q3_LOGPROB_COLS);
                 r->fed = h_nfr[b];
             }
             push_frames(*r->chunker, hbuf, nnew);
diff --git a/qwen3-tts-rust_amd/csrc/engine.h b/qwen3-tts-rust_amd/csrc/engine.h
--- a/qwen3-tts-rust_amd/csrc/engine.h
+++ b/qwen3-tts-rust_amd/csrc/engine.h
@@ -73,6 +73,9 @@
     }
     int64_t submit_decode(const int32_t* codes, int n);
     int decode_width() const { return decode_w_; }
+    void codec_pass_stats(int64_t* passes, int64_t* streams, int64_t* widest) const {
+        *passes = worker_ ? worker_->passes.load() : 0; *streams = worker_ ? worker_->pass_streams.load() : 0; *widest = worker_ ? worker_->pass_widest.load() : 0;
+    }
     void decode_stats(int64_t* requests, int64_t* chunks, int64_t* chunks_shared) const {
         *requests = dec_reqs_.load(); *chunks = worker_ ? worker_->dec_chunks.load() : 0; *chunks_shared = worker_ ? worker_->dec_shared.load() : 0;
     }
@@ -187,6 +190,7 @@
     OutSpec out_; mutable std::mutex out_mu_;
     void take_out(Req* r, int max_steps, const OutSpec* given = nullptr) const;
     void upload_slot_state();
+    void publish_load();
     void* stage_alloc(size_t bytes) { return stage_take(ar_, bytes); }
     void h2d(void* dst, const void* src, size_t bytes);
     void* d2h_begin(const void* src, size_t bytes);
@@ -213,6 +217,7 @@
     DevBuf<uint32_t> d_rngkey_, d_draws_, d_prngkey_, d_pdraws_; DevBuf<float> d_plogits_;
     DevBuf<int32_t> d_pseq_, d_pslot_, d_ppos_;
     DevBuf<float> d_tlogits_, d_thidden_, d_pin_, d_fb_;
+    DevBuf<uint8_t> d_rec_; DevBuf<int32_t> d_fed_[2]; int fed_cur_ = 0;
     int64_t kv_rows_ = 0;
     int hist_stride_ = 0, tl_stride_ = 0;
     DevBuf<float> d_text_; DevBuf<int32_t> d_trail_; int64_t text_rows_ = 0;
diff --git a/qwen3-tts-rust_amd/csrc/kernels.h b/qwen3-tts-rust_amd/csrc/kernels.h
--- a/qwen3-tts-rust_amd/csrc/kernels.h
+++ b/qwen3-tts-rust_amd/csrc/kernels.h
@@ -200,6 +200,14 @@
 };
 void launch_stall_save(hipStream_t st, const AdvanceKeysArgs& a, const StallArgs& s);
 void launch_advance_keys_gated(hipStream_t st, const AdvanceKeysArgs& a, const StallArgs& s);
+struct GroupPackArgs {
+    int width = 0, group = 0;
+    const int32_t *n_frames = nullptr, *finished = nullptr, *fed = nullptr; int32_t* fed_next = nullptr;
+    const int32_t* hist = nullptr; int hist_stride = 0;
+    const float* lp = nullptr; int lp_rows = 0; const int32_t* lp_rec = nullptr;
+    unsigned char* rec = nullptr;
+};
+void launch_group_pack(hipStream_t st, const GroupPackArgs& a);
 
 struct SampleArgs {
     const float* logits; int stride; int n;
diff --git a/qwen3-tts-rust_amd/csrc/kernels_fused.hip b/qwen3-tts-rust_amd/csrc/kernels_fused.hip
--- a/qwen3-tts-rust_amd/csrc/kernels_fused.hip
+++ b/qwen3-tts-rust_amd/csrc/kernels_fused.hip
@@ -917,4 +917,59 @@
     hipLaunchKernelGGL(k_advance_keys_gated, dim3(a.B), dim3(256), 0, st, a, s);
 }
 
-}
+__device__ __forceinline__ int pack_rows(const GroupPackArgs& a, int b) {
+    const int n = a.n_frames[b] - a.fed[b];
+    return a.fed[b] < 0 ? 0 : (n < a.group ? n : a.group);
+}
+__global__ void __launch_bounds__(256) k_group_pack(GroupPackArgs a, int n_pieces) {
+    const int p = blockIdx.x * 256 + threadIdx.x;
+    if (p >= n_pieces) return;
+    const int V = (a.width + 3) / 4;
+    int4* const dst = reinterpret_cast<int4*>(a.rec) + p;
+    if (p < 2 * V) {
+        const bool nfr = p < V;
+        const int32_t* src = nfr ? a.n_frames : a.finished;
+        const int b0 = (nfr ? p : p - V) * 4;
+        int v[4];
+#pragma unroll
+        for (int i = 0; i < 4; i++) {
+            v[i] = b0 + i < a.width ? src[b0 + i] : 0;
+            if (nfr && a.fed_next && b0 + i < a.width) a.fed_next[b0 + i] = v[i];
+        }
+        *dst = make_int4(v[0], v[1], v[2], v[3]);
+        return;
+    }
+    int q = p - 2 * V;
+    if (q < a.width * 16) {
+        const int b = q >> 4, j = (q >> 2) & 3, c = q & 3;
+        const long long row = (long long)a.fed[b] + j;
+        int4 v = make_int4(-1, -1, -1, -1);
+        if (j < pack_rows(a, b) && (row + 1) * 16 <= a.hist_stride)
+            v = *reinterpret_cast<const int4*>(a.hist + (size_t)b * a.hist_stride + (size_t)row * 16 + c * 4);
+        *dst = v;
+        return;
+    }
+    q -= a.width * 16;
+    const int b = q / Q3_LOGPROB_COLS, k = q % Q3_LOGPROB_COLS;
+    const int rows = (!a.lp_rec || a.lp_rec[b]) ? pack_rows(a, b) : 0;
+    float v[4];
+#pragma unroll
+    for (int i = 0; i < 4; i++) {
+        const int e = k * 4 + i, j = e / Q3_LOGPROB_COLS, col = e % Q3_LOGPROB_COLS;
+        const long long row = (long long)a.fed[b] + j;
+        v[i] = (j < rows && row < a.lp_rows) ? a.lp[((size_t)b * a.lp_rows + (size_t)row) * Q3_LOGPROB_COLS + col] : 0.0f;
+    }
+    *reinterpret_cast<float4*>(dst) = make_float4(v[0], v[1], v[2], v[3]);
+}
+void launch_group_pack(hipStream_t st, const GroupPackArgs& a) {
+    if (a.width < 1 || a.group < 1 || a.group > 4) throw Error("k_group_pack: width >= 1 and a group of 1..4 frames");
+    if (!a.n_frames || !a.finished || !a.fed || !a.hist || !a.rec || a.fed_next == a.fed) throw Error("k_group_pack: a buffer is missing, or fed_next is fed");
+    if (a.hist_stride < 16 || a.hist_stride % 16 != 0 || (reinterpret_cast<uintptr_t>(a.hist) & 15) != 0 || (reinterpret_cast<uintptr_t>(a.rec) & 15) != 0)
+        throw Error("k_group_pack: history rows and the record must be 16-byte aligned");
+    if (a.lp && a.lp_rows < 1) throw Error("k_group_pack: log-probability rows missing");
+    const int V = (a.width + 3) / 4;
+    const int n_pieces = 2 * V + a.width * 16 + (a.lp ? a.width * Q3_LOGPROB_COLS : 0);
+    hipLaunchKernelGGL(k_group_pack, dim3((n_pieces + 255) / 256), dim3(256), 0, st, a, n_pieces);
+}
+
+}
diff --git a/qwen3-tts-rust_amd/csrc/sched_logic.h b/qwen3-tts-rust_amd/csrc/sched_logic.h
--- a/qwen3-tts-rust_amd/csrc/sched_logic.h
+++ b/qwen3-tts-rust_amd/csrc/sched_logic.h
@@ -103,6 +103,19 @@
     }
     return v;
 }
+
+struct GroupRecord {
+    enum { ROWS = 4 };
+    int width = 0; bool lp = false;
+    size_t nfr = 0, fin = 0, codes = 0, logprobs = 0, bytes = 0;
+    GroupRecord(int width_, bool lp_) : width(width_), lp(lp_) {
+        const size_t vec = ((size_t)width * 4 + 15) & ~(size_t)15;
+        nfr = 0; fin = vec; codes = 2 * vec;
+        logprobs = codes + (size_t)width * ROWS * 16 * 4;
+        bytes = logprobs + (lp ? (size_t)width * ROWS * Q3_LOGPROB_COLS * 4 : 0);
+    }
+    size_t pieces() const { return bytes / 16; }
+};
 
 enum ReqState { REQ_QUEUED = 0, REQ_RUNNING = 1, REQ_DRAINING = 2, REQ_DONE = 3, REQ_CANCELLED = 4, REQ_FAILED = -1 };
 inline bool req_ended(int state) { return state == REQ_DONE || state == REQ_CANCELLED || state == REQ_FAILED; }
@@ -315,6 +328,18 @@
 
 inline int decode_width(int n_cs, int max_batch) { return std::max(1, (n_cs - max_batch) / 2); }
 inline int decode_admit(int queued, int free_cs, int holding, int width) { return std::max(0, std::min(queued, std::min(free_cs, width - holding))); }
+
+enum { CODEC_IDLE_GROUP = 32 };
+struct CodecCaps {
+    int busy = 1, idle = 1;
+    int pass(bool engine_idle) const { return engine_idle ? idle : busy; }
+};
+inline CodecCaps codec_caps(int max_batch, int n_cs, int group_env, int idle_env) {
+    CodecCaps c;
+    c.busy = std::max(1, std::min(max_batch, group_env > 0 ? group_env : (max_batch >= 128 ? 32 : 16)));
+    c.idle = idle_env == 0 ? c.busy : std::max(c.busy, std::min(n_cs, idle_env > 0 ? idle_env : (int)CODEC_IDLE_GROUP));
+    return c;
+}
 
 enum TaskKind { TASK_CHUNK = 0, TASK_RESET = 1, TASK_FENCE = 2 };
 enum { SEAT_DRY_MAX = 4 };
@@ -356,8 +381,14 @@
     struct Task { Job* job; TaskKind kind; std::vector<int64_t> codes; bool is_final; int64_t epoch; };
     std::deque<Task> live, low;
     int pending = 0, hold = 0, dry = 0; int64_t epoch = 0;
+    std::deque<int64_t> wide;
     void open() { if (hold++ == 0) epoch++; }
-    void close() { hold--; }
+    void close(bool engine_idle = false) { if (--hold == 0 && engine_idle) wide.push_back(epoch); }
+    bool lead_wide() {
+        if (live.empty() || live.front().kind != TASK_CHUNK) return false;
+        while (!wide.empty() && wide.front() < live.front().epoch) wide.pop_front();
+        return !wide.empty() && wide.front() == live.front().epoch;
+    }
     void push(Job* j, TaskKind kind, const int64_t* codes = nullptr, int n_codes = 0, bool is_final = false) {
         (j->decode ? low : live).push_back(Task{j, kind, std::vector<int64_t>(codes, codes + n_codes), is_final, kind == TASK_CHUNK && !j->decode ? epoch : 0});
         if (kind != TASK_RESET) pending++;
diff --git a/qwen3-tts-rust_amd/python/q3tts/__init__.py b/qwen3-tts-rust_amd/python/q3tts/__init__.py
--- a/qwen3-tts-rust_amd/python/q3tts/__init__.py
+++ b/qwen3-tts-rust_amd/python/q3tts/__init__.py
@@ -114,6 +114,7 @@
     "q3tts_loudness_tables", "q3tts_loudness_gate", "q3tts_loudness_gain_db10", "q3tts_op_loudness",
     "q3tts_intake_plan", "q3tts_intake_filter", "q3tts_intake_samples", "q3tts_intake_tile", "q3tts_intake_check", "q3tts_wav_probe",
     "q3tts_intake", "q3tts_wav_intake",
+    "q3tts_group_record_layout", "q3tts_op_group_pack", "q3tts_engine_codec_pass_stats",
 ]
 
 
@@ -289,6 +290,9 @@
         L.q3tts_op_score_inputs.argtypes = [C.c_void_p, C.POINTER(C.c_void_p), C.c_void_p, C.c_int32, C.c_void_p, C.c_int32, C.c_void_p]
         L.q3tts_op_logprob_rows.argtypes = [C.c_void_p, C.c_int32, C.c_int32, C.c_int32, C.c_void_p, C.c_int32, C.c_void_p, C.c_void_p]
         L.q3tts_op_frame_glue.argtypes = [C.c_void_p]
+        L.q3tts_group_record_layout.argtypes = [C.c_int32, C.c_int32, C.POINTER(C.c_int64)]
+        L.q3tts_op_group_pack.argtypes = [C.c_void_p]
+        L.q3tts_engine_codec_pass_stats.argtypes = [C.c_void_p, C.POINTER(C.c_int64), C.POINTER(C.c_int64), C.POINTER(C.c_int64)]
         L.q3tts_engine_set_output_format.argtypes = [C.c_void_p, C.POINTER(PcmFormat)]
         L.q3tts_request_format.argtypes = [C.c_void_p, C.c_int64, C.POINTER(PcmFormat)]
         L.q3tts_fetch_pcm16.argtypes = [C.c_void_p, C.c_int64, C.c_void_p, C.c_int64, C.c_int64, C.POINTER(C.c_int64)]
@@ -953,6 +957,11 @@
         _chk(lib().q3tts_engine_decode_stats(self.h, C.byref(a), C.byref(b), C.byref(c)))
         return dict(requests=a.value, chunks=b.value, chunks_shared=c.value)
 
+    def codec_pass_stats(self):
+        a, b, c = C.c_int64(), C.c_int64(), C.c_int64()
+        _chk(lib().q3tts_engine_codec_pass_stats(self.h, C.byref(a), C.byref(b), C.byref(c)))
+        return dict(passes=a.value, streams=b.value, widest=c.value)
+
     def candidate_stats(self):
         a, b, c = C.c_int64(), C.c_int64(), C.c_int64()
         _chk(lib().q3tts_engine_candidate_stats(self.h, C.byref(a), C.byref(b), C.byref(c)))
@@ -2126,6 +2135,38 @@
     _chk(lib().q3tts_op_frame_glue(C.byref(d)))
 
 
+class GroupPackDesc(C.Structure):
+    _fields_ = [("width", C.c_int32), ("group", C.c_int32), ("n_frames", C.c_void_p), ("finished", C.c_void_p), ("fed", C.c_void_p),
+                ("hist", C.c_void_p), ("hist_stride", C.c_int32), ("lp", C.c_void_p), ("lp_rows", C.c_int32), ("lp_rec", C.c_void_p),
+                ("rec", Guarded), ("fed_next", Guarded)]
+
+
+def group_record_layout(width, lp):
+    out = (C.c_int64 * 5)()
+    _chk(lib().q3tts_group_record_layout(int(width), int(bool(lp)), out))
+    return dict(zip(("n_frames", "finished", "codes", "logprobs", "bytes"), [int(v) for v in out]))
+
+
+def op_group_pack(width, group, n_frames, finished, fed, hist, rec, fed_next, lp=None, lp_rec=None):
+    d = GroupPackDesc()
+    d.width, d.group = int(width), int(group)
+    keep = []
+    for k, v in (("n_frames", n_frames), ("finished", finished), ("fed", fed), ("hist", hist), ("lp_rec", lp_rec)):
+        if v is not None:
+            keep.append(np.ascontiguousarray(v, np.int32))
+            setattr(d, k, keep[-1].ctypes.data)
+            if k == "hist":
+                d.hist_stride = keep[-1].shape[-1]
+    if lp is not None:
+        keep.append(np.ascontiguousarray(lp, np.float32))
+        d.lp, d.lp_rows = keep[-1].ctypes.data, keep[-1].shape[1]
+    for k, v, dt in (("rec", rec, np.uint8), ("fed_next", fed_next, np.int32)):
+        if v is not None:
+            assert isinstance(v, np.ndarray) and v.dtype == dt and v.ndim == 1 and v.flags["C_CONTIGUOUS"], k
+            setattr(d, k, Guarded(v.ctypes.data, v.size))
+    _chk(lib().q3tts_op_group_pack(C.byref(d)))
+
+
 GG_LOAD_ROWS, GG_ADD, GG_RMSNORM, GG_QUANT, GG_MATVEC, GG_LINEAR, GG_SWIGLU = range(7)
 _GG_GUARDED = {"out": np.float32, "q8": np.int8, "d8": np.uint16, "qk": np.int8, "dk": np.float32, "bs": np.int16}
 _GG_ARRAYS = {"x": np.float32, "u": np.float32, "idx": np.int32, "idx_keys": np.uint64, "w": np.uint8}
```

Measured after the change: 757.2. 0.988x the previous value.
